# Farmadupe/vid_dup_finder_lib

Measured on AMD Instinct MI355X. Metric: hash-pairs/sec all-pairs Hamming (search(), tolerance 0.35) [+ frames/sec DCT-hash in 'summary.hash_summary'], higher is better.
Workload: dtype fp4 e2m1 ({0,1}) x fp4 -> f32 accumulate (exact half-integers < 2^11)

## Files before the change

vid_dup_finder_lib_amd/csrc/api.cpp:

```cpp
#include <algorithm>
#include <chrono>
#include <cmath>
#include <cstdio>
#include <cstdlib>
#include <cstring>
#include <memory>
#include <numeric>

#include "host_sort.h"
#include "vdf_ctx.h"

namespace {
thread_local std::string g_create_error;
inline double now_ms() { return std::chrono::duration<double, std::milli>(std::chrono::steady_clock::now().time_since_epoch()).count(); }
}

vdf_ctx::~vdf_ctx()
{
    if (!subs.empty() || !workers.empty()) vdf_impl::destroy_multi(this);
    if (copy_pool) vdf_impl::destroy_copy_pool(this);
    for (auto &kv : axis_tables) {
        kv.second->start.release(); kv.second->size.release(); kv.second->w.release();
        delete kv.second;
    }
    for (auto &kv : mfma_tables) {
        kv.second->operand.release(); kv.second->bias.release(); kv.second->meta.release();
        delete kv.second;
    }
    for (auto &kv : box_tables) {
        kv.second->blob.release(); kv.second->entries.release();
        delete kv.second;
    }
    DevBuf *all[] = {&row_lo, &row_hi, &tile_lo, &tile_hi, &tile_first, &tile_count, &tile_offset, &counters,
                     &hits, &perm, &matched, &exp_cols, &exp_rows, &pop_cols, &pop_rows, &cand, &group_cmin, &group_offset, &group_blocks, &up_hashes,
                     &up_dur, &up_ref_hashes, &up_ref_dur, &small, &frames, &frames2, &out_hashes, &out_hashes2, &out_dc,
                     &out_dc2, &cos_table, &crops, &crop_desc, &crop_tables, &crop_desc2, &crop_tables2, &crop_work, &sort_scratch, &sort_scratch_pub, &hits2, &hit_bitmaps, &bitmap_gather,
                     &out_zero, &out_zero2, &up_zero, &variant_hashes, &align_plan, &align_scratch, &align_up};
    for (DevBuf *b : all) b->release();
    for (PinBuf &b : pin) b.release();
    for (PinBuf &b : pin_out) b.release();
    pin_small.release();
    pin_ctrl.release();
    pin_crops.release();
    pin_desc.release();
    host_hits.buf.release();
    if (ev0) (void)hipEventDestroy(ev0);
    if (ev1) (void)hipEventDestroy(ev1);
    if (ev_mid) (void)hipEventDestroy(ev_mid);
    if (ev_wait) (void)hipEventDestroy(ev_wait);
    for (hipEvent_t e : ev_copy) if (e) (void)hipEventDestroy(e);
    for (hipEvent_t e : ev_done) if (e) (void)hipEventDestroy(e);
    if (copy_stream) (void)hipStreamDestroy(copy_stream);
    if (stream) (void)hipStreamDestroy(stream);
}

namespace vdf_impl {

void set_create_error(const std::string &msg) { g_create_error = msg; }

int fail(vdf_ctx *ctx, int code, const std::string &msg)
{
    if (ctx) ctx->err = msg;
    return code;
}

int fail_hip(vdf_ctx *ctx, hipError_t e, const char *what)
{
    std::string msg = std::string(what) + ": " + hipGetErrorString(e);
    (void)hipGetLastError();
    return fail(ctx, e == hipErrorOutOfMemory ? VDF_E_OOM : VDF_E_HIP, msg);
}

bool is_sorted_u32(const uint32_t *d, size_t n)
{
    for (size_t i = 1; i < n; i++)
        if (d[i] < d[i - 1]) return false;
    return true;
}

constexpr size_t kPinSmallBytes = 4u << 20;
constexpr uint64_t kDeviceSortHits = 1u << 17;
constexpr uint32_t kRefsMinWorkgroups = 2048;
constexpr uint64_t kSpecSortHits = 1u << 14;
constexpr uint64_t kFilterHits = 1u << 16;

int search_core(vdf_ctx *ctx, int mode, const uint64_t *d_col_hashes, const uint32_t *d_col_dur, size_t n_cols,
                const uint64_t *d_row_hashes, const uint32_t *d_row_dur, const uint32_t *d_row_perm, size_t n_rows,
                uint32_t tol_int, uint32_t shard_index, uint32_t shard_count, uint32_t row_begin, uint32_t row_end,
                const uint32_t *d_matched, uint32_t row_index_base, vdf_hit *hits, uint64_t capacity,
                uint64_t *n_hits_out, uint32_t *overflow_row_out, hipStream_t stream, bool replay_only, vdf_ctx::HostHits *staging,
                ShardExchange *fx)
{
    *n_hits_out = 0;
    *overflow_row_out = 0xFFFFFFFFu;
    if (n_rows == 0 || n_cols == 0) return VDF_OK;
    if (n_rows >= 0xFFFFFFFFull || n_cols >= 0xFFFFFFFFull) return fail(ctx, VDF_E_INVAL, "more than 2^32-1 hashes");
    if (shard_count == 0 || shard_index >= shard_count) return fail(ctx, VDF_E_INVAL, "bad shard index/count");
    VDF_HIP(ctx, hipSetDevice(ctx->device));
    const double t_enter = now_ms();

    vdf::SearchLaunch L{};
    const bool mfma = ctx->search_backend == 1;
    L.tile_rows = mfma ? (mode == 1 ? ctx->mfma_refs_rows : ctx->mfma_self_rows) : ctx->tile_rows;
    L.chunk_cols = mfma ? ctx->mfma_chunk_cols : ctx->chunk_cols;
    L.n_row_tiles = (uint32_t)((n_rows + L.tile_rows - 1) / L.tile_rows);
    if (mfma && L.chunk_cols == 0) {
        L.chunk_cols = 65536;
        while (L.chunk_cols > 4096 && (uint64_t)L.n_row_tiles * ((n_cols + L.chunk_cols - 1) / L.chunk_cols) < ctx->mfma_min_wgs) L.chunk_cols /= 2;
    }
    while ((uint64_t)L.n_row_tiles * ((n_cols + L.chunk_cols - 1) / L.chunk_cols) >= 0x40000000ull && L.chunk_cols < (1u << 22))
        L.chunk_cols *= 2;
    const size_t padded_rows = (size_t)L.n_row_tiles * L.tile_rows;
    VDF_HIP(ctx, ctx->row_lo.reserve(padded_rows * 4));
    VDF_HIP(ctx, ctx->row_hi.reserve(padded_rows * 4));
    VDF_HIP(ctx, ctx->tile_lo.reserve((size_t)L.n_row_tiles * 4));
    VDF_HIP(ctx, ctx->tile_hi.reserve((size_t)L.n_row_tiles * 4));
    VDF_HIP(ctx, ctx->tile_first.reserve((size_t)L.n_row_tiles * 4));
    VDF_HIP(ctx, ctx->tile_count.reserve((size_t)L.n_row_tiles * 4));
    VDF_HIP(ctx, ctx->tile_offset.reserve(((size_t)L.n_row_tiles + 1) * 4));
    VDF_HIP(ctx, ctx->counters.reserve(64));
    const uint64_t dev_cap = std::max<uint64_t>(capacity, 1);
    VDF_HIP(ctx, ctx->hits.reserve(dev_cap * sizeof(vdf_hit)));

    L.row_hashes = reinterpret_cast<const uint32_t *>(d_row_hashes);
    L.row_perm = d_row_perm;
    L.n_rows = (uint32_t)n_rows;
    L.row_index_base = row_index_base;
    L.col_hashes = reinterpret_cast<const uint32_t *>(d_col_hashes);
    L.n_cols = (uint32_t)n_cols;
    L.row_lo = ctx->row_lo.as<uint32_t>();
    L.row_hi = ctx->row_hi.as<uint32_t>();
    L.tile_lo = ctx->tile_lo.as<uint32_t>();
    L.tile_hi = ctx->tile_hi.as<uint32_t>();
    L.tile_first = ctx->tile_first.as<uint32_t>();
    L.tile_count = ctx->tile_count.as<uint32_t>();
    L.tile_offset = ctx->tile_offset.as<uint32_t>();
    L.tol = tol_int;
    L.matched = d_matched;
    L.self_mode = (mode == 0);
    L.shard_index = shard_index;
    L.shard_count = shard_count;
    L.hits = ctx->hits.as<vdf_hit>();
    L.capacity = capacity;
    L.counters = ctx->counters.as<unsigned long long>();
    L.overflow_row = reinterpret_cast<uint32_t *>(ctx->counters.as<unsigned long long>() + 4);

    L.prune_step = 16;
    if (ctx->mfma_prune_step >= 0) {
        L.prune_step = ctx->mfma_prune_step;
    } else {
        for (int st = 6; st <= 14; st++) {
            const double bits = 64.0 * (st + 1);
            if (bits / 2 - 2.0 * std::sqrt(bits) >= (double)tol_int + 1) { L.prune_step = st; break; }
        }
    }
    if (mfma) L.prune_step = L.prune_step <= 6 ? 6 : L.prune_step <= 8 ? 8 : L.prune_step <= 10 ? 10 : L.prune_step <= 14 ? L.prune_step : 16;
    else L.prune_step = L.prune_step <= 6 ? 6 : L.prune_step <= 10 ? 10 : L.prune_step <= 12 ? 12 : 16;
    if (mfma) {
        L.group_size = std::min<uint32_t>(ctx->mfma_group, L.n_row_tiles);
        L.n_groups = (L.n_row_tiles + L.group_size - 1) / L.group_size;
        if (L.n_groups > 1024) return fail(ctx, VDF_E_INVAL, "too many row-tile groups");
        VDF_HIP(ctx, ctx->group_cmin.reserve((size_t)L.n_groups * 4));
        VDF_HIP(ctx, ctx->group_offset.reserve(((size_t)L.n_groups + 1) * 4));
        VDF_HIP(ctx, ctx->group_blocks.reserve((size_t)L.n_groups * 4));
        L.group_blocks = ctx->group_blocks.as<uint32_t>();
        L.group_cmin = ctx->group_cmin.as<uint32_t>();
        L.group_offset = ctx->group_offset.as<uint32_t>();
        const uint32_t k_steps = (uint32_t)(L.prune_step < 15 ? L.prune_step + 1 : 16);
        const uint32_t col_pad = (uint32_t)((n_cols + vdf::kMfmaRowPad - 1) / vdf::kMfmaRowPad * vdf::kMfmaRowPad) + vdf::kMfmaColPad;
        VDF_HIP(ctx, ctx->exp_cols.reserve((size_t)col_pad * 512));
        VDF_HIP(ctx, ctx->pop_cols.reserve((size_t)col_pad * 12));
        const ExpOwner want_owner{d_col_hashes, n_cols, k_steps, ctx->exp_cols.p};
        const bool reuse = ctx->pinned_db == d_col_hashes && ctx->pinned_n == n_cols && ctx->exp_owner == want_owner;
        if (!reuse) {
            ctx->exp_owner = ExpOwner{};
            VDF_HIP(ctx, vdf::launch_expand_fp4(L.col_hashes, (uint32_t)n_cols, col_pad, ctx->exp_cols.p, k_steps,
                                                ctx->pop_cols.as<float>(), stream));
            ctx->exp_owner = want_owner;
        }
        L.col_exp = ctx->exp_cols.p;
        L.col_pop3 = ctx->pop_cols.as<float>();
        L.col_pad = col_pad;
        if (d_row_hashes == d_col_hashes) {
            L.row_exp = ctx->exp_cols.p;
            L.row_pop3 = L.col_pop3;
            L.row_pad = col_pad;
        } else {
            const uint32_t row_pad = (uint32_t)((padded_rows + 127) / 128 * 128);
            VDF_HIP(ctx, ctx->exp_rows.reserve((size_t)row_pad * 512));
            VDF_HIP(ctx, ctx->pop_rows.reserve((size_t)row_pad * 12));
            VDF_HIP(ctx, vdf::launch_expand_fp4(L.row_hashes, (uint32_t)n_rows, row_pad, ctx->exp_rows.p, k_steps,
                                                ctx->pop_rows.as<float>(), stream));
            L.row_exp = ctx->exp_rows.p;
            L.row_pop3 = ctx->pop_rows.as<float>();
            L.row_pad = row_pad;
        }
    }
    const unsigned long long init[8] = {0, 0, 0, 0, 0xFFFFFFFFull, 0, 0, 0};
    const bool pin_ok = ctx->pin_small.reserve(kPinSmallBytes) && ctx->pin_small.pinned;
    uint64_t spec = std::min<uint64_t>(capacity, std::max<uint64_t>(ctx->hits_guess + ctx->hits_guess / 4 + 1024, 8192));
    if (!pin_ok || spec * sizeof(vdf_hit) > kPinSmallBytes) spec = 0;
    const bool spec_sort = spec && ctx->hits_guess >= kSpecSortHits;
    if (spec_sort) VDF_HIP(ctx, hipMemsetAsync(ctx->hits.p, 0xFF, (size_t)spec * sizeof(vdf_hit), stream));
    const bool adapt_refs = mode == 1 && mfma && ctx->mfma_chunk_cols == 0;
    if (adapt_refs && ctx->refs_hint_cols == n_cols && ctx->refs_hint_rows == n_rows && ctx->refs_hint_chunk) L.chunk_cols = ctx->refs_hint_chunk;
    if (!ctx->pin_ctrl.reserve(256)) return fail(ctx, VDF_E_OOM, "pinned staging");
    unsigned long long *pre = ctx->pin_ctrl.as<unsigned long long>() + 8;
    uint32_t total_tiles = 0;
    unsigned long long unsorted = 0, admitted = 0;
    for (int pass = 0;; pass++) {
        VDF_HIP(ctx, hipMemcpyAsync(ctx->counters.p, init, sizeof init, hipMemcpyHostToDevice, stream));
        VDF_HIP(ctx, vdf::launch_windows_tiles(mode, d_col_dur, (uint32_t)n_cols, d_row_dur, d_row_perm, (uint32_t)n_rows,
                                               row_begin, row_end, shard_index, shard_count, L, stream));
        VDF_HIP(ctx, hipMemcpyAsync(pre, L.counters, 64, hipMemcpyDeviceToHost, stream));
        VDF_HIP(ctx, hipMemcpyAsync(pre + 8, mfma ? L.group_offset + L.n_groups : L.tile_offset + L.n_row_tiles, 4,
                                    hipMemcpyDeviceToHost, stream));
        VDF_HIP(ctx, hipMemcpyAsync(pre + 9, L.tile_offset + L.n_row_tiles, 4, hipMemcpyDeviceToHost, stream));
        VDF_HIP(ctx, hipStreamSynchronize(stream));
        total_tiles = *reinterpret_cast<const uint32_t *>(pre + 8);
        const uint32_t busy_tiles = *reinterpret_cast<const uint32_t *>(pre + 9);
        unsorted = pre[5];
        admitted = pre[2];
        if (!adapt_refs || pass > 0 || unsorted || busy_tiles == 0 || busy_tiles >= kRefsMinWorkgroups || L.chunk_cols <= 4096) break;
        uint64_t est = busy_tiles;
        while (L.chunk_cols > 4096 && est < kRefsMinWorkgroups) { L.chunk_cols /= 2; est *= 2; }
    }
    if (adapt_refs) { ctx->refs_hint_cols = n_cols; ctx->refs_hint_rows = n_rows; ctx->refs_hint_chunk = L.chunk_cols; }
    if (unsorted) return fail(ctx, VDF_E_INVAL, "durations are not ascending: pass the arrays in Search::sort order");
    if (total_tiles >= 0x7FFFFFFFu) return fail(ctx, VDF_E_INVAL, "tile count exceeds the grid limit");
    if (mfma) {
        const uint64_t want = ((uint64_t)((double)admitted * 6e-6) + (uint64_t)total_tiles * 8 * 8 + std::max<uint64_t>(capacity, 1ull << 20)) * ctx->cand_scale;
        L.cand_capacity = (uint32_t)std::min<uint64_t>(want, 0x40000000ull);
        if (ctx->cand_capacity_override)
            L.cand_capacity = (uint32_t)std::min<uint64_t>((uint64_t)ctx->cand_capacity_override * ctx->cand_scale, 0x40000000ull);
        const void *before = ctx->cand.p;
        VDF_HIP(ctx, ctx->cand.reserve((size_t)L.cand_capacity * 16));
        if (ctx->cand.p != before) ctx->cand_dirty = SIZE_MAX;
        const size_t slots = ctx->cand.cap / 16;
        const size_t fill = (ctx->cand_dirty == SIZE_MAX ? slots : std::min<size_t>(slots, ctx->cand_dirty)) * 16;
        if (fill) VDF_HIP(ctx, hipMemsetAsync(ctx->cand.p, 0xFF, fill, stream));
        ctx->cand_dirty = L.cand_capacity;
        L.cand = ctx->cand.p;
        L.cand_head = ctx->counters.as<unsigned long long>() + 6;
    }

    ctx->timing.prep_ms += (float)(now_ms() - t_enter);
    VDF_HIP(ctx, hipEventRecord(ctx->ev0, stream));
    if (mfma) {
        VDF_HIP(ctx, vdf::launch_hamming_tiles_mfma2(L, total_tiles, stream));
        VDF_HIP(ctx, hipEventRecord(ctx->ev_mid, stream));
        if (total_tiles) VDF_HIP(ctx, vdf::launch_resolve_candidates(L, stream));
    } else {
        VDF_HIP(ctx, vdf::launch_hamming_tiles(L, total_tiles, stream));
        VDF_HIP(ctx, hipEventRecord(ctx->ev_mid, stream));
    }
    VDF_HIP(ctx, hipEventRecord(ctx->ev1, stream));
    if (!ctx->pin_ctrl.reserve(256)) return fail(ctx, VDF_E_OOM, "pinned staging");
    unsigned long long *fin = ctx->pin_ctrl.as<unsigned long long>();
    VDF_HIP(ctx, hipMemcpyAsync(fin, ctx->counters.p, 64, hipMemcpyDeviceToHost, stream));
    unsigned row_bits = 1;
    while (row_bits < 32 && ((uint64_t)row_index_base + n_rows) >> row_bits) row_bits++;
    unsigned col_bits = 1;
    while (col_bits < 32 && ((uint64_t)n_cols >> col_bits)) col_bits++;
    if (spec_sort) {
        VDF_HIP(ctx, ctx->sort_scratch.reserve(vdf::sort_hits_scratch_bytes((size_t)spec)));
        VDF_HIP(ctx, vdf::launch_sort_hits(ctx->hits.as<vdf_hit>(), (size_t)spec, row_bits, ctx->sort_scratch.p, ctx->sort_scratch.cap, stream, col_bits));
    }
    if (spec) VDF_HIP(ctx, hipMemcpyAsync(ctx->pin_small.p, ctx->hits.p, (size_t)spec * sizeof(vdf_hit), hipMemcpyDeviceToHost, stream));
    VDF_HIP(ctx, hipStreamSynchronize(stream));
    const double t_synced = now_ms();
    float ms = 0.f, ms_stream = 0.f;
    VDF_HIP(ctx, hipEventElapsedTime(&ms, ctx->ev0, ctx->ev1));
    VDF_HIP(ctx, hipEventElapsedTime(&ms_stream, ctx->ev0, ctx->ev_mid));
    ctx->timing.stream_ms += ms_stream;
    ctx->timing.resolve_ms += ms - ms_stream;
    if (mfma) { ctx->timing.suspects += fin[6]; ctx->timing.suspect_capacity = L.cand_capacity; }

    if (mfma) ctx->cand_dirty = (size_t)std::min<uint64_t>(fin[6], L.cand_capacity);
    const uint64_t produced = fin[0];
    uint64_t stored = std::min<uint64_t>(produced, capacity);
    ctx->hits_guess = stored;
    uint64_t n_out = produced;
    vdf_hit *d_list = ctx->hits.as<vdf_hit>();
    uint64_t have = std::min(stored, spec);
    bool filter = false;
    if (replay_only && mode == 0 && !ctx->no_hit_filter) {
        bool complete = produced <= capacity && (uint32_t)fin[4] == 0xFFFFFFFFu;
        uint64_t total = produced;
        if (fx) {
            const int r = fx->agree(shard_index, ctx, &complete, &total);
            if (r) return r;
        } else if (shard_count != 1) {
            complete = false;
        }
        filter = complete && total >= kFilterHits;
    }
    if (filter) {
        const size_t words = ((size_t)n_cols + 31) / 32;
        VDF_HIP(ctx, ctx->hits2.reserve((size_t)std::max<uint64_t>(stored, 1) * sizeof(vdf_hit)));
        VDF_HIP(ctx, ctx->hit_bitmaps.reserve(2 * words * 4 + 16));
        uint32_t *bm = ctx->hit_bitmaps.as<uint32_t>();
        VDF_HIP(ctx, vdf::launch_filter_mark_incoming(d_list, stored, (uint32_t)n_cols, bm, stream));
        if (fx) { const int r = fx->or_bitmap(shard_index, ctx, bm, words, stream); if (r < 0) return r; if (r == vdf_impl::kExchangeOff) filter = false; }
        if (filter) {
            VDF_HIP(ctx, vdf::launch_filter_mark_covered(d_list, stored, (uint32_t)n_cols, bm, stream));
            if (fx) { const int r = fx->or_bitmap(shard_index, ctx, bm + words, words, stream); if (r < 0) return r; if (r == vdf_impl::kExchangeOff) filter = false; }
        }
    }
    if (filter) {
        uint32_t *bm = ctx->hit_bitmaps.as<uint32_t>();
        VDF_HIP(ctx, vdf::launch_filter_compact(d_list, stored, (uint32_t)n_cols, bm, ctx->hits2.as<vdf_hit>(), L.counters + 7, stream));
        VDF_HIP(ctx, hipMemcpyAsync(fin + 7, L.counters + 7, 8, hipMemcpyDeviceToHost, stream));
        VDF_HIP(ctx, hipStreamSynchronize(stream));
        d_list = ctx->hits2.as<vdf_hit>();
        stored = fin[7];
        n_out = stored;
        have = 0;
        ctx->timing.hits_filtered += produced - stored;
    }
    if (stored) {
        if (staging) {
            const size_t need = std::max<size_t>((size_t)stored, 1u << 16);
            if (staging->size() < need && !staging->resize(need + need / 4)) return fail(ctx, VDF_E_OOM, "hit staging");
            hits = staging->data();
        }
        if (have) std::memcpy(hits, ctx->pin_small.p, (size_t)have * sizeof(vdf_hit));
        if (stored > have) {
            const bool dev_sort = stored >= (d_list == ctx->hits.as<vdf_hit>() ? kDeviceSortHits : kDeviceSortHits / 16);
            if (dev_sort) {
                VDF_HIP(ctx, ctx->sort_scratch.reserve(vdf::sort_hits_scratch_bytes((size_t)stored)));
                VDF_HIP(ctx, vdf::launch_sort_hits(d_list, (size_t)stored, row_bits, ctx->sort_scratch.p, ctx->sort_scratch.cap, stream, col_bits));
                VDF_HIP(ctx, hipMemcpyAsync(hits, d_list, (size_t)stored * sizeof(vdf_hit), hipMemcpyDeviceToHost, stream));
            } else {
                VDF_HIP(ctx, hipMemcpyAsync(hits + have, d_list + have, (size_t)(stored - have) * sizeof(vdf_hit), hipMemcpyDeviceToHost, stream));
            }
            VDF_HIP(ctx, hipStreamSynchronize(stream));
            if (!dev_sort) sort_hits(hits, (size_t)stored);
        } else if (!spec_sort) {
            sort_hits(hits, (size_t)stored);
        }
    }
    ctx->timing.download_ms += (float)(now_ms() - t_synced);
    *n_hits_out = n_out;
    *overflow_row_out = (uint32_t)fin[4];
    ctx->stats.pairs += fin[2];
    ctx->stats.pairs_computed += fin[1];
    ctx->stats.n_hits += produced;
    ctx->stats.n_tiles += total_tiles;
    ctx->stats.n_launches += 1;
    ctx->stats.kernel_ms += ms;
    ctx->stats.pairs_early_exit += fin[3];
    ctx->stats.early_exit_bits = L.prune_step < 15 ? 64u * (uint32_t)(L.prune_step + 1) : 0u;
    return VDF_OK;
}

int upload(vdf_ctx *ctx, DevBuf &buf, const void *src, size_t bytes, hipStream_t stream)
{
    VDF_HIP(ctx, buf.reserve(std::max<size_t>(bytes, 16)));
    if (bytes) VDF_HIP(ctx, hipMemcpyAsync(buf.p, src, bytes, hipMemcpyHostToDevice, stream));
    return VDF_OK;
}

std::mutex &link_mutex(int device)
{
    static std::mutex m[64];
    return m[(unsigned)device % 64u];
}

int wait_event(vdf_ctx *ctx, hipEvent_t ev)
{
    if (!ctx->spin_wait) {
        const auto until = std::chrono::steady_clock::now() + std::chrono::microseconds(50);
        do {
            const hipError_t q = hipEventQuery(ev);
            if (q == hipSuccess) return VDF_OK;
            if (q != hipErrorNotReady) return fail_hip(ctx, q, "hipEventQuery");
        } while (std::chrono::steady_clock::now() < until);
    }
    VDF_HIP(ctx, hipEventSynchronize(ev));
    return VDF_OK;
}

DeviceAxisTable *axis_table(vdf_ctx *ctx, uint32_t in_size, hipStream_t stream, int *rc)
{
    auto it = ctx->axis_tables.find(in_size);
    if (it != ctx->axis_tables.end()) { *rc = VDF_OK; return it->second; }
    DeviceAxisTable *t = new DeviceAxisTable();
    if (!vdf::build_axis_table(in_size, VDF_DCT_SIZE, t->host)) {
        delete t;
        *rc = fail(ctx, VDF_E_BAD_DIMS, "cannot build resize table");
        return nullptr;
    }
    int r = upload(ctx, t->start, t->host.start.data(), t->host.start.size() * 4, stream);
    if (r == VDF_OK) r = upload(ctx, t->size, t->host.size.data(), t->host.size.size() * 4, stream);
    if (r == VDF_OK) r = upload(ctx, t->w, t->host.w.data(), t->host.w.size() * 2, stream);
    if (r == VDF_OK && hipStreamSynchronize(stream) != hipSuccess) r = fail(ctx, VDF_E_HIP, "table upload failed");
    if (r != VDF_OK) {
        t->start.release(); t->size.release(); t->w.release();
        delete t;
        *rc = r;
        return nullptr;
    }
    ctx->axis_tables[in_size] = t;
    *rc = VDF_OK;
    return t;
}

DeviceMfmaTable *mfma_table(vdf_ctx *ctx, uint32_t in_size, int layout, hipStream_t stream, int *rc)
{
    const uint64_t key = (uint64_t)in_size * 4 + (uint64_t)layout;
    auto it = ctx->mfma_tables.find(key);
    if (it != ctx->mfma_tables.end()) { *rc = VDF_OK; return it->second; }
    DeviceMfmaTable *t = new DeviceMfmaTable();
    if (!vdf::build_mfma_axis_table(in_size, layout, t->host)) {
        delete t;
        *rc = fail(ctx, VDF_E_BAD_DIMS, "cannot build resize table");
        return nullptr;
    }
    int r = VDF_OK;
    if (t->host.ok) {
        r = upload(ctx, t->operand, t->host.operand.data(), t->host.operand.size(), stream);
        if (r == VDF_OK) r = upload(ctx, t->bias, t->host.bias.data(), t->host.bias.size() * 4, stream);
        if (r == VDF_OK && !t->host.band_meta.empty())
            r = upload(ctx, t->meta, t->host.band_meta.data(), t->host.band_meta.size() * 4, stream);
        if (r == VDF_OK && hipStreamSynchronize(stream) != hipSuccess) r = fail(ctx, VDF_E_HIP, "table upload failed");
    }
    if (r != VDF_OK) {
        t->operand.release(); t->bias.release(); t->meta.release();
        delete t;
        *rc = r;
        return nullptr;
    }
    ctx->mfma_tables[key] = t;
    *rc = VDF_OK;
    return t;
}

BoxTableSet *box_table_set(vdf_ctx *ctx, uint32_t w, uint32_t h, hipStream_t stream, int *rc)
{
    const uint64_t key = ((uint64_t)w << 32) | h;
    auto it = ctx->box_tables.find(key);
    if (it != ctx->box_tables.end()) { *rc = VDF_OK; return it->second; }
    BoxTableSet *set = new BoxTableSet();
    set->one_tile = w <= 64 && h <= 64;
    const size_t n_idx = (size_t)w + h + 2;
    std::vector<vdf::CropTableEntry> entries(n_idx, vdf::CropTableEntry{nullptr, nullptr, 0, 0});
    std::vector<size_t> offset(n_idx, 0);
    std::vector<uint8_t> blob;
    bool usable = true;
    for (size_t idx = 0; idx < n_idx && usable; idx++) {
        const bool vertical = idx > w;
        const uint32_t size = (uint32_t)(vertical ? idx - w - 1 : idx);
        offset[idx] = blob.size();
        if (size == 0) {
            if (set->one_tile) blob.resize(blob.size() + vdf::kSmallBoxTableStride, 0);
            continue;
        }
        vdf::MfmaAxisTable t;
        if (!vdf::build_mfma_axis_table(size, vertical ? vdf::kMfmaLayoutVertical : vdf::kMfmaLayoutHorizontal, t) || !t.ok) { usable = false; break; }
        const size_t at = blob.size();
        blob.resize(at + t.operand.size() + 128, 0);
        std::memcpy(blob.data() + at, t.operand.data(), t.operand.size());
        std::memcpy(blob.data() + at + t.operand.size(), t.bias.data(), 64);
        const int32_t tail[2] = {t.precision, t.n_tiles};
        std::memcpy(blob.data() + at + t.operand.size() + 64, tail, sizeof tail);
        entries[idx].n_tiles = t.n_tiles;
        entries[idx].precision = t.precision;
        if (set->one_tile && blob.size() - at != vdf::kSmallBoxTableStride) usable = false;
    }
    int r = VDF_OK;
    if (usable) {
        r = upload(ctx, set->blob, blob.data(), blob.size(), stream);
        if (r == VDF_OK) {
            for (size_t idx = 0; idx < n_idx; idx++) {
                if (!entries[idx].n_tiles) continue;
                entries[idx].operand = set->blob.as<uint8_t>() + offset[idx];
                entries[idx].bias = reinterpret_cast<const int32_t *>(set->blob.as<uint8_t>() + offset[idx] + (size_t)entries[idx].n_tiles * 2048);
            }
            r = upload(ctx, set->entries, entries.data(), entries.size() * sizeof(vdf::CropTableEntry), stream);
        }
        if (r == VDF_OK && hipStreamSynchronize(stream) != hipSuccess) r = fail(ctx, VDF_E_HIP, "table upload failed");
    }
    if (r != VDF_OK) {
        set->blob.release(); set->entries.release();
        delete set;
        *rc = r;
        return nullptr;
    }
    set->usable = usable;
    ctx->box_tables[key] = set;
    *rc = VDF_OK;
    return set;
}

vdf::ResizeAxisTable dev_view(const DeviceAxisTable *t)
{
    vdf::ResizeAxisTable v{};
    if (t) {
        v.start = t->start.as<int32_t>();
        v.size = t->size.as<int32_t>();
        v.w = t->w.as<int16_t>();
        v.window = t->host.window;
        v.precision = t->host.precision;
    }
    return v;
}

int ensure_cos_table(vdf_ctx *ctx, hipStream_t stream)
{
    if (ctx->cos_table.p) return VDF_OK;
    double tab[16 * 16 + 17];
    for (int k = 0; k < 16; k++)
        for (int n = 0; n < 16; n++) tab[k * 16 + n] = std::cos(M_PI * (double)k * ((double)n + 0.5) / 16.0);
    int at = 256;
    auto twiddle = [&](int i, int fft_len) {
        const double angle_constant = M_PI * -2.0 / (double)fft_len;
        const double angle = angle_constant * (double)i;
        tab[at++] = std::cos(angle);
        tab[at++] = -std::sin(angle);
    };
    for (int i = 0; i < 4; i++) twiddle(2 * i + 1, 64);
    for (int i = 0; i < 2; i++) twiddle(2 * i + 1, 32);
    twiddle(1, 16);
    tab[at++] = M_SQRT1_2;
    tab[at++] = 0.0; tab[at++] = 0.0;
    int rc = upload(ctx, ctx->cos_table, tab, sizeof tab, stream);
    if (rc) return rc;
    VDF_HIP(ctx, hipStreamSynchronize(stream));
    return VDF_OK;
}

using vdf::kMaxClipsPerLaunch;

struct HashJob {
    const uint8_t *d_frames;
    size_t n_clips;
    uint32_t w, h;
    size_t frame_stride, clip_stride;
    uint64_t *d_out;
    uint32_t *d_dc;
    hipStream_t stream;
    uint64_t *d_zero = nullptr;
    vdf::HashCall call() const { return vdf::HashCall{d_frames, w, h, frame_stride, clip_stride, n_clips}; }
    const uint8_t *buf_end() const { return d_frames + (n_clips - 1) * clip_stride + (VDF_DCT_SIZE - 1) * frame_stride + (size_t)w * h; }
    HashJob clips(size_t c0, size_t n) const
    {
        return HashJob{d_frames + c0 * clip_stride, n, w, h, frame_stride, clip_stride, d_out + c0 * VDF_HASH_WORDS, d_dc ? d_dc + c0 : nullptr, stream,
                       d_zero ? d_zero + c0 * VDF_HASH_WORDS : nullptr};
    }
};

template <class One> int checked_launches(vdf_ctx *ctx, const HashJob &j, uint32_t frames_per_clip, One one)
// ... 433 lines not shown
                      uint64_t *d_zero)
{
    VDF_HIP(ctx, hipSetDevice(ctx->device));
    int rc = ensure_cos_table(ctx, stream);
    if (rc) return rc;
    const size_t n = plan.descs.size(), nd = n * sizeof(vdf::MixedClipDesc), off = (nd + 63) & ~size_t(63);
    const size_t max_entries = 2 * ((size_t)plan.max_w + plan.max_h + 2);
    if (!ctx->pin_desc.reserve(off + max_entries * sizeof(vdf::CropTableEntry))) return fail(ctx, VDF_E_OOM, "host staging for the clip descriptors");
    vdf::MixedClipDesc *dsc = ctx->pin_desc.as<vdf::MixedClipDesc>();
    vdf::CropTableEntry *ent = reinterpret_cast<vdf::CropTableEntry *>(ctx->pin_desc.as<char>() + off);
    LaunchTables plain(plan.max_w, plan.max_h, vdf::kMfmaLayoutHorizontal, vdf::kMfmaLayoutVertical), wide(plan.max_w, plan.max_h, vdf::kMfmaLayoutHorizontal, vdf::kMfmaLayoutVerticalWide);
    for (const vdf::MixedLaunch &l : plan.launches) {
        LaunchTables &tabs = l.part == vdf::MixedPart::kWideLines ? wide : plain;
        for (size_t i = l.first; i < l.first + l.count; i++) {
            vdf::MixedClipDesc d = plan.descs[i];
            const int32_t ih = tabs.entry(ctx, d.bw, false, stream, &rc), iv = ih < 0 ? -1 : tabs.entry(ctx, d.bh, true, stream, &rc);
            if (iv < 0) return rc ? rc : fail(ctx, VDF_E_BAD_DIMS, "box size whose coefficients do not fit the i8 split (clip " + std::to_string(d.out_index) + ")");
            d.h_table = (uint32_t)ih; d.v_table = (uint32_t)iv;
            dsc[i] = d;
        }
    }
    const size_t n_plain = plain.used.size(), n_entries = n_plain + wide.used.size();
    if (n_entries > max_entries) return fail(ctx, VDF_E_INVAL, "table index of a mixed call outgrew its staging");
    for (size_t i = 0; i < n_plain; i++) ent[i] = plain.crop_entry(i);
    for (size_t i = n_plain; i < n_entries; i++) ent[i] = wide.crop_entry(i - n_plain);
    for (const vdf::MixedLaunch &l : plan.launches)
        for (size_t i = l.first; i < l.first + l.count; i++) {
            if (l.part == vdf::MixedPart::kWideLines) { dsc[i].h_table += (uint32_t)n_plain; dsc[i].v_table += (uint32_t)n_plain; }
            if (dsc[i].h_table >= n_entries || dsc[i].v_table >= n_entries || dsc[i].out_index >= n) return fail(ctx, VDF_E_INVAL, "descriptor names a table or an output that is not there");
        }
    const size_t n_frames_part = n - plan.n_small;
    VDF_HIP(ctx, ctx->small.reserve(std::max<size_t>(n_frames_part, 1) * 4096));
    if ((rc = upload(ctx, ctx->crop_desc2, dsc, nd, stream))) return rc;
    if ((rc = upload(ctx, ctx->crop_tables2, ent, n_entries * sizeof(vdf::CropTableEntry), stream))) return rc;
    VDF_HIP(ctx, hipEventRecord(ctx->ev_mid, stream));
    const vdf::MixedClipDesc *d_desc = ctx->crop_desc2.as<vdf::MixedClipDesc>();
    const vdf::CropTableEntry *d_tab = ctx->crop_tables2.as<vdf::CropTableEntry>();
    const uint8_t *buf_end = d_buf + buf_bytes;
    uint8_t *small = ctx->small.as<uint8_t>();
    hipError_t e = hipSuccess;
    for (const vdf::MixedLaunch &l : plan.launches) {
        if (e != hipSuccess) break;
        if (l.part == vdf::MixedPart::kSmall) {
            e = vdf::launch_mixed_small(d_buf, buf_end, d_desc + l.first, l.count, d_tab, ctx->cos_table.as<double>(), d_out, d_dc, stream, d_zero);
        } else {
            uint8_t *slot0 = small + (l.first - plan.n_small) * 4096;
            e = vdf::launch_mixed_frames(d_buf, buf_end, d_desc + l.first, l.count, d_tab, l.part == vdf::MixedPart::kWideLines, slot0, stream);
            if (e == hipSuccess) e = vdf::launch_dct_hash_indexed(slot0, d_desc + l.first, l.count, ctx->cos_table.as<double>(), d_out, d_dc, stream, d_zero);
        }
    }
    const hipError_t ew = hipEventSynchronize(ctx->ev_mid);
    if (e != hipSuccess) return fail_hip(ctx, e, "mixed hash launch");
    VDF_HIP(ctx, ew);
    return VDF_OK;
}

int hash_clips_locked(vdf_ctx *ctx, const uint8_t *d_buf, size_t buf_bytes, const vdf_clip *clips, size_t n_clips, uint32_t frames_per_clip,
                      uint64_t *d_out, uint32_t *d_dc, hipStream_t stream, uint64_t *d_zero)
{
    if (n_clips && !clips) return fail(ctx, VDF_E_INVAL, "null pointer");
    if (n_clips > 0xFFFFFFFFull) return fail(ctx, VDF_E_INVAL, "more than 2^32 - 1 clips in one call");
    const vdf::MixedClip *mc = reinterpret_cast<const vdf::MixedClip *>(clips);
    const vdf::MixedCheck chk = vdf::check_mixed(mc, n_clips, frames_per_clip, buf_bytes);
    if (chk.error != vdf::MixedError::kNone) return mixed_check_failed(ctx, chk);
    if (n_clips == 0) return VDF_OK;
    if (!d_buf || !d_out) return fail(ctx, VDF_E_INVAL, "null pointer");
    const vdf::MixedPlan plan = vdf::plan_mixed(mc, n_clips, hash_knobs(ctx));
    if (plan.kind == vdf::MixedPlan::kUniform) {
        std::vector<uint32_t> crops;
        if (plan.cropped) {
            crops.resize(n_clips * 4);
            for (size_t i = 0; i < n_clips; i++) std::memcpy(&crops[4 * i], mc[i].crop, 16);
        }
        const HashJob all{d_buf + plan.offset0, n_clips, mc[0].w, mc[0].h, (size_t)mc[0].frame_stride, (size_t)plan.clip_stride, d_out, d_dc, stream, d_zero};
        return checked_launches(ctx, all, frames_per_clip,
                                [&](size_t c0, size_t n) { return hash_cropped_launch(ctx, all.clips(c0, n), plan.cropped ? crops.data() + 4 * c0 : nullptr); });
    }
    return hash_mixed_launch(ctx, d_buf, buf_bytes, plan, d_out, d_dc, stream, d_zero);
}

int letterbox_small(vdf_ctx *ctx, const HashJob &j, uint32_t frames_per_clip, const vdf::LetterboxPlan &plan, const BoxTableSet *set, uint32_t *out_crops,
                    uint32_t *d_crops)
{
    const size_t n_fused = j.n_clips - plan.n_tail;
    if (n_fused)
        VDF_HIP(ctx, vdf::launch_letterbox_hash_small(j.d_frames, n_fused, j.w, j.h, j.frame_stride, j.clip_stride, set->blob.p, ctx->cos_table.as<double>(),
                                                      j.d_out, j.d_dc, d_crops, ctx->hash_wgs_per_cu_set ? ctx->hash_wgs_per_cu : 0, j.stream));
    if (plan.n_tail) {
        const HashJob tail = j.clips(n_fused, plan.n_tail);
        VDF_HIP(ctx, ctx->crop_work.reserve(vdf::letterbox_work_bytes(tail.n_clips, frames_per_clip)));
        VDF_HIP(ctx, vdf::launch_letterbox(tail.d_frames, tail.n_clips, frames_per_clip, j.w, j.h, j.frame_stride, j.clip_stride, d_crops + 4 * n_fused,
                                           ctx->crop_work.as<uint32_t>(), j.stream, ctx->lb_side_strips));
        VDF_HIP(ctx, vdf::launch_resize_dct_cropped_small_boxes(tail.d_frames, tail.n_clips, j.w, j.h, j.frame_stride, j.clip_stride, j.buf_end(), d_crops + 4 * n_fused,
                                                                set->entries.as<vdf::CropTableEntry>(), ctx->cos_table.as<double>(), tail.d_out, tail.d_dc, j.stream));
    }
    if (out_crops) {
        if (!ctx->pin_crops.reserve(j.n_clips * 16)) return fail(ctx, VDF_E_OOM, "host staging for the crop boxes");
        VDF_HIP(ctx, hipMemcpyAsync(ctx->pin_crops.p, d_crops, j.n_clips * 16, hipMemcpyDeviceToHost, j.stream));
        VDF_HIP(ctx, hipEventRecord(ctx->ev_mid, j.stream));
        VDF_HIP(ctx, hipEventSynchronize(ctx->ev_mid));
        std::memcpy(out_crops, ctx->pin_crops.p, j.n_clips * 16);
    }
    return VDF_OK;
}

int letterbox_launch(vdf_ctx *ctx, const HashJob &j, uint32_t frames_per_clip, uint32_t *out_crops, uint32_t *d_out_crops)
{
    VDF_HIP(ctx, hipSetDevice(ctx->device));
    uint32_t *d_crops = d_out_crops;
    if (!d_crops) {
        VDF_HIP(ctx, ctx->crops.reserve(j.n_clips * 16));
        d_crops = ctx->crops.as<uint32_t>();
    }
    const vdf::LetterboxPlan plan = vdf::plan_letterbox(j.call(), hash_knobs(ctx));
    if (plan.small_frames) {
        int rc = ensure_cos_table(ctx, j.stream);
        if (rc) return rc;
        const BoxTableSet *set = box_table_set(ctx, j.w, j.h, j.stream, &rc);
        if (rc) return rc;
        if (set->usable) return letterbox_small(ctx, j, frames_per_clip, plan, set, out_crops, d_crops);
    }
    VDF_HIP(ctx, ctx->crop_work.reserve(vdf::letterbox_work_bytes(j.n_clips, frames_per_clip)));
    VDF_HIP(ctx, vdf::launch_letterbox(j.d_frames, j.n_clips, frames_per_clip, j.w, j.h, j.frame_stride, j.clip_stride, d_crops, ctx->crop_work.as<uint32_t>(),
                                       j.stream, ctx->lb_side_strips));
    if (!ctx->pin_crops.reserve(j.n_clips * 16)) return fail(ctx, VDF_E_OOM, "host staging for the crop boxes");
    uint32_t *crops = ctx->pin_crops.as<uint32_t>();
    VDF_HIP(ctx, hipMemcpyAsync(crops, d_crops, j.n_clips * 16, hipMemcpyDeviceToHost, j.stream));
    VDF_HIP(ctx, hipEventRecord(ctx->ev_wait, j.stream));
    if (int rcw = wait_event(ctx, ctx->ev_wait)) return rcw;
    if (out_crops) std::memcpy(out_crops, crops, j.n_clips * 16);
    return hash_cropped_launch(ctx, j, crops);
}

int letterbox_hash_device_locked(vdf_ctx *ctx, const uint8_t *d_frames, size_t n_clips, uint32_t frames_per_clip,
                                 uint32_t w, uint32_t h, size_t frame_stride, size_t clip_stride, uint64_t *d_out,
                                 uint32_t *d_dc, uint32_t *out_crops, hipStream_t stream, uint32_t *d_out_crops)
{
    const HashJob all{d_frames, n_clips, w, h, frame_stride, clip_stride, d_out, d_dc, stream};
    return checked_launches(ctx, all, frames_per_clip, [&](size_t c0, size_t n) {
        return letterbox_launch(ctx, all.clips(c0, n), frames_per_clip, out_crops ? out_crops + 4 * c0 : nullptr, d_out_crops ? d_out_crops + 4 * c0 : nullptr);
    });
}

static int letterbox_clips_plan(vdf_ctx *ctx, const void *d_buf, size_t buf_bytes, const vdf_clip *clips, size_t n_clips, uint32_t frames_per_clip, const void *out,
                                vdf::LetterboxMixedPlan *plan)
{
    if (n_clips && !clips) return fail(ctx, VDF_E_INVAL, "null pointer");
    if (n_clips > 0xFFFFFFFFull) return fail(ctx, VDF_E_INVAL, "more than 2^32 - 1 clips in one call");
    const vdf::MixedClip *mc = reinterpret_cast<const vdf::MixedClip *>(clips);
    const vdf::MixedCheck chk = vdf::check_mixed(mc, n_clips, frames_per_clip, buf_bytes);
    if (chk.error != vdf::MixedError::kNone) return mixed_check_failed(ctx, chk);
    *plan = vdf::plan_letterbox_mixed(mc, n_clips, hash_knobs(ctx));
    if (plan->kind == vdf::LetterboxMixedPlan::kCropGiven) return mixed_check_failed(ctx, vdf::MixedCheck{vdf::MixedError::kCropGiven, plan->bad_clip});
    if (n_clips && (!d_buf || !out)) return fail(ctx, VDF_E_INVAL, "null pointer");
    return VDF_OK;
}

static int letterbox_clips_detect(vdf_ctx *ctx, const uint8_t *d_buf, const vdf::LetterboxMixedPlan &plan, size_t n_clips, uint32_t *d_crops, hipStream_t stream)
{
    VDF_HIP(ctx, hipSetDevice(ctx->device));
    const size_t nd = plan.descs.size() * sizeof(vdf::LetterboxProbeDesc);
    if (plan.descs.size() != n_clips) return fail(ctx, VDF_E_INVAL, "letterbox plan does not cover the call");
    if (!ctx->pin_desc.reserve(nd)) return fail(ctx, VDF_E_OOM, "host staging for the clip descriptors");
    std::memcpy(ctx->pin_desc.p, plan.descs.data(), nd);
    if (int rc = upload(ctx, ctx->crop_desc, ctx->pin_desc.p, nd, stream)) return rc;
    VDF_HIP(ctx, hipEventRecord(ctx->ev_mid, stream));
    VDF_HIP(ctx, ctx->crop_work.reserve(plan.work_bytes));
    const hipError_t e = vdf::launch_letterbox_mixed(d_buf, ctx->crop_desc.as<vdf::LetterboxProbeDesc>(), plan.launches.data(), plan.launches.size(), n_clips, d_crops,
                                                     ctx->crop_work.as<uint32_t>(), stream);
    const hipError_t ew = hipEventSynchronize(ctx->ev_mid);
    if (e != hipSuccess) return fail_hip(ctx, e, "mixed letterbox launch");
    VDF_HIP(ctx, ew);
    return VDF_OK;
}

int cropdetect_clips_locked(vdf_ctx *ctx, const uint8_t *d_buf, size_t buf_bytes, const vdf_clip *clips, size_t n_clips, uint32_t frames_per_clip,
                            uint32_t *d_crops, hipStream_t stream)
{
    vdf::LetterboxMixedPlan plan;
    if (int rc = letterbox_clips_plan(ctx, d_buf, buf_bytes, clips, n_clips, frames_per_clip, d_crops, &plan)) return rc;
    if (n_clips == 0) return VDF_OK;
    if (plan.kind == vdf::LetterboxMixedPlan::kUniform) {
        VDF_HIP(ctx, hipSetDevice(ctx->device));
        const uint8_t *base = d_buf + plan.offset0;
        VDF_HIP(ctx, ctx->crop_work.reserve(vdf::letterbox_work_bytes(std::min(kMaxClipsPerLaunch, n_clips), frames_per_clip)));
        for (size_t c0 = 0; c0 < n_clips; c0 += kMaxClipsPerLaunch)
            VDF_HIP(ctx, vdf::launch_letterbox(base + c0 * plan.clip_stride, std::min(kMaxClipsPerLaunch, n_clips - c0), frames_per_clip, clips[0].w, clips[0].h,
                                               (size_t)clips[0].frame_stride, (size_t)plan.clip_stride, d_crops + 4 * c0, ctx->crop_work.as<uint32_t>(), stream,
                                               ctx->lb_side_strips));
        return VDF_OK;
    }
    return letterbox_clips_detect(ctx, d_buf, plan, n_clips, d_crops, stream);
}

int letterbox_clips_locked(vdf_ctx *ctx, const uint8_t *d_buf, size_t buf_bytes, const vdf_clip *clips, size_t n_clips, uint32_t frames_per_clip,
                           uint64_t *d_out, uint32_t *d_dc, uint32_t *out_crops, hipStream_t stream)
{
    vdf::LetterboxMixedPlan plan;
    if (int rc = letterbox_clips_plan(ctx, d_buf, buf_bytes, clips, n_clips, frames_per_clip, d_out, &plan)) return rc;
    if (n_clips == 0) return VDF_OK;
    if (plan.kind == vdf::LetterboxMixedPlan::kUniform)
        return letterbox_hash_device_locked(ctx, d_buf + plan.offset0, n_clips, frames_per_clip, clips[0].w, clips[0].h, (size_t)clips[0].frame_stride,
                                            (size_t)plan.clip_stride, d_out, d_dc, out_crops, stream);
    VDF_HIP(ctx, hipSetDevice(ctx->device));
    VDF_HIP(ctx, ctx->crops.reserve(n_clips * 16));
    uint32_t *d_crops = ctx->crops.as<uint32_t>();
    if (int rc = letterbox_clips_detect(ctx, d_buf, plan, n_clips, d_crops, stream)) return rc;
    if (!ctx->pin_crops.reserve(n_clips * 16)) return fail(ctx, VDF_E_OOM, "host staging for the crop boxes");
    const uint32_t *crops = ctx->pin_crops.as<uint32_t>();
    VDF_HIP(ctx, hipMemcpyAsync(ctx->pin_crops.p, d_crops, n_clips * 16, hipMemcpyDeviceToHost, stream));
    VDF_HIP(ctx, hipEventRecord(ctx->ev_wait, stream));
    if (int rcw = wait_event(ctx, ctx->ev_wait)) return rcw;
    if (out_crops) std::memcpy(out_crops, crops, n_clips * 16);
    std::vector<vdf_clip> boxed(clips, clips + n_clips);
    for (size_t i = 0; i < n_clips; i++) {
        boxed[i].crop_left = crops[4 * i]; boxed[i].crop_right = crops[4 * i + 1];
        boxed[i].crop_top = crops[4 * i + 2]; boxed[i].crop_bottom = crops[4 * i + 3];
    }
    return hash_clips_locked(ctx, d_buf, buf_bytes, boxed.data(), n_clips, frames_per_clip, d_out, d_dc, stream);
}


int search_refs_device_locked(vdf_ctx *ctx, const uint64_t *d_cand_hashes, const uint32_t *d_cand_durations,
                                     size_t n_cand, const uint64_t *d_ref_hashes, const uint32_t *d_ref_durations,
                                     size_t n_ref, uint32_t tol_int, uint32_t ref_index_base, vdf_hit *hits,
                                     uint64_t capacity, uint64_t *n_hits, hipStream_t s, vdf_ctx::HostHits *staging)
{
    ctx->stats = vdf_search_stats{};
    ctx->timing = vdf_search_timing{};
    *n_hits = 0;
    if (n_ref == 0 || n_cand == 0) return VDF_OK;
    VDF_HIP(ctx, hipSetDevice(ctx->device));
    const size_t sbytes = vdf::sort_order_scratch_bytes((uint32_t)n_ref, false);
    VDF_HIP(ctx, ctx->sort_scratch.reserve(sbytes));
    VDF_HIP(ctx, ctx->perm.reserve(std::max<size_t>(n_ref * 4, 16)));
    VDF_HIP(ctx, vdf::launch_sort_order(d_ref_durations, nullptr, (uint32_t)n_ref, ctx->perm.as<uint32_t>(), ctx->sort_scratch.p,
                                        ctx->sort_scratch.cap, s));
    int rc = VDF_OK;
    for (int attempt = 0;; attempt++) {
        uint32_t overflow_row = 0;
        ctx->stats = vdf_search_stats{};
        rc = search_core(ctx, 1, d_cand_hashes, d_cand_durations, n_cand, d_ref_hashes, d_ref_durations,
                         ctx->perm.as<uint32_t>(), n_ref, tol_int, 0, 1, 0, 0xFFFFFFFFu, nullptr, ref_index_base, hits,
                         capacity, n_hits, &overflow_row, s, false, staging);
        if (rc) { ctx->cand_scale = 1; return rc; }
        if (*n_hits > capacity) { ctx->cand_scale = 1; return fail(ctx, VDF_E_OVERFLOW, "hit buffer too small; *n_hits holds the required size"); }
        if (overflow_row == 0xFFFFFFFFu) break;
        if (attempt >= 12) { ctx->cand_scale = 1; return fail(ctx, VDF_E_OVERFLOW, "suspect queue overflow"); }
        ctx->cand_scale *= 4;
    }
    ctx->cand_scale = 1;
    return VDF_OK;
}

int create_single(int device_id, vdf_ctx **out, std::string *err)
{
    *out = nullptr;
    int count = 0;
    hipError_t e = hipGetDeviceCount(&count);
    if (e != hipSuccess || count <= 0) {
        *err = std::string("no usable HIP device: ") + (e != hipSuccess ? hipGetErrorString(e) : "count = 0");
        (void)hipGetLastError();
        return VDF_E_HIP;
    }
    if (device_id < 0 || device_id >= count) { *err = "device id out of range"; return VDF_E_INVAL; }
    vdf_ctx *ctx = new (std::nothrow) vdf_ctx();
    if (!ctx) return VDF_E_OOM;
    ctx->device = device_id;
    ctx->spin_wait = std::getenv("VDF_SPIN_WAIT") != nullptr;
    ctx->no_link_turns = std::getenv("VDF_NO_LINK_TURNS") != nullptr;
    const unsigned wait_flags = hipEventDisableTiming | (ctx->spin_wait ? 0u : (unsigned)hipEventBlockingSync);
    bool ok = hipSetDevice(device_id) == hipSuccess &&
              hipStreamCreateWithFlags(&ctx->stream, hipStreamNonBlocking) == hipSuccess &&
              hipEventCreate(&ctx->ev0) == hipSuccess && hipEventCreate(&ctx->ev1) == hipSuccess &&
              hipEventCreate(&ctx->ev_mid) == hipSuccess && hipEventCreateWithFlags(&ctx->ev_wait, wait_flags) == hipSuccess;
    for (int i = 0; ok && i < 2; i++)
        ok = hipEventCreateWithFlags(&ctx->ev_copy[i], wait_flags) == hipSuccess &&
             hipEventCreateWithFlags(&ctx->ev_done[i], wait_flags) == hipSuccess;
    if (!ok) {
        *err = std::string("context setup failed: ") + hipGetErrorString(hipGetLastError());
        delete ctx;
        return VDF_E_HIP;
    }
    if (const char *s = std::getenv("VDF_ROWS_PER_LANE")) {
        int r = std::atoi(s);
        if (r == 1 || r == 2 || r == 4) ctx->tile_rows = 256u * (uint32_t)r;
    }
    if (const char *s = std::getenv("VDF_RESIZE_MODE")) {
        int m = std::atoi(s);
        if (m >= 0 && m <= 6 && m != 2) ctx->resize_mode = m;
    }
    if (const char *s = std::getenv("VDF_SEARCH_BACKEND")) {
        if (!std::strcmp(s, "valu")) ctx->search_backend = 0;
        else if (!std::strcmp(s, "mfma")) ctx->search_backend = 1;
    }
    if (const char *s = std::getenv("VDF_MFMA_CHUNK_COLS")) {
        long c = std::atol(s);
        if (c >= 32 && c <= (1 << 22)) ctx->mfma_chunk_cols = (uint32_t)c;
    }
    if (const char *s = std::getenv("VDF_CAND_CAPACITY")) { const long v = std::atol(s); if (v >= 8 && v <= 0x40000000l) ctx->cand_capacity_override = (uint32_t)v; }
    if (const char *s = std::getenv("VDF_MFMA_SELF_ROWS")) { const int v = std::atoi(s); if (v == 256 || v == 512) ctx->mfma_self_rows = (uint32_t)v; }
    if (const char *s = std::getenv("VDF_MFMA_REFS_ROWS")) { const int v = std::atoi(s); if (v == 256 || v == 512) ctx->mfma_refs_rows = (uint32_t)v; }
    if (const char *s = std::getenv("VDF_MFMA_PRUNE_STEP")) ctx->mfma_prune_step = std::atoi(s);
    if (const char *s = std::getenv("VDF_MFMA_MIN_WGS")) { const long v = std::atol(s); if (v >= 1 && v <= (1 << 24)) ctx->mfma_min_wgs = (uint32_t)v; }
    if (const char *s = std::getenv("VDF_MFMA_GROUP")) {
        long c = std::atol(s);
        if (c >= 1 && c <= (1 << 20)) ctx->mfma_group = (uint32_t)c;
    }
    if (const char *s = std::getenv("VDF_NO_HIT_FILTER")) ctx->no_hit_filter = std::atoi(s) != 0;
    if (std::getenv("VDF_NO_WAVESTREAM")) ctx->wavestream_knob = -1;
    else if (const char *s = std::getenv("VDF_WAVESTREAM_NW")) { const int v = std::atoi(s); if (v >= 3 && v <= 8) ctx->wavestream_knob = v; }
    ctx->no_rowcrop = std::getenv("VDF_NO_ROWCROP") != nullptr;
    ctx->rowcrop_all = std::getenv("VDF_ROWCROP_ALL") != nullptr;
    ctx->no_boxstream = std::getenv("VDF_NO_BOXSTREAM") != nullptr;
    ctx->no_smallcrop = std::getenv("VDF_NO_SMALLCROP") != nullptr;
    ctx->no_device_path_order = std::getenv("VDF_NO_DEVICE_PATH_ORDER") != nullptr;
    ctx->lb_host_plan = std::getenv("VDF_LB_HOST_PLAN") != nullptr;
    ctx->no_lb_fused = std::getenv("VDF_NO_LB_FUSED") != nullptr;
    if (std::getenv("VDF_LB_NC16")) ctx->lb_side_strips = 16;
    if (const char *s = std::getenv("VDF_COPY_THREADS")) { const int v = std::atoi(s); if (v >= 1 && v <= 64) ctx->copy_threads = v; }
    if (const char *s = std::getenv("VDF_HOST_CHUNK_MB")) { const long v = std::atol(s); if (v >= 1 && v <= 1024) ctx->host_chunk_bytes = (size_t)v << 20; }
    if (const char *s = std::getenv("VDF_HOST_DIRECT")) ctx->host_direct = std::atoi(s) != 0;
    if (const char *s = std::getenv("VDF_HASH_NO_PERSISTENT")) ctx->hash_no_persistent = std::atoi(s) != 0;
    if (const char *s = std::getenv("VDF_HASH_WGS_PER_CU")) {
        int v = std::atoi(s);
        if (v >= 1 && v <= 8) { ctx->hash_wgs_per_cu = v; ctx->hash_wgs_per_cu_set = true; }
    }
    if (const char *s = std::getenv("VDF_CHUNK_COLS")) {
        long c = std::atol(s);
        if (c >= 64 && c <= (1 << 20)) ctx->chunk_cols = (uint32_t)c;
    }
    *out = ctx;
    return VDF_OK;
}

int search_self_resident(vdf_ctx *ctx, size_t n, uint32_t tol_int, vdf_groups *out)
{
    const int G = device_count(ctx);
    uint64_t capacity = ctx->hit_capacity;
    std::vector<uint8_t> matched(n, 0);
    std::vector<uint32_t> bitmap;
    bool use_bitmap = false;
    std::vector<vdf_hit> merged;
    uint32_t row_begin = 0;
    uint64_t span = n;
    ctx->stats = vdf_search_stats{};
    const double t_call = now_ms();
    double replay_ms = 0.0;
    for (int k = 0; k < G; k++) { device_ctx(ctx, k)->stats = vdf_search_stats{}; device_ctx(ctx, k)->timing = vdf_search_timing{}; }
    while (row_begin < n) {
        const uint32_t row_end = (uint32_t)std::min<uint64_t>((uint64_t)row_begin + span, n);
        std::unique_ptr<ShardExchange> fx(make_local_exchange(ctx));
        int rc = for_each_device(ctx, [&](int k, vdf_ctx *d) {
            const int r = search_core(d, 0, d->up_hashes.as<uint64_t>(), d->up_dur.as<uint32_t>(), n, d->up_hashes.as<uint64_t>(),
                                      d->up_dur.as<uint32_t>(), nullptr, n, tol_int, (uint32_t)k, (uint32_t)G, row_begin, row_end,
                                      use_bitmap ? d->matched.as<uint32_t>() : nullptr, 0, nullptr, capacity,
                                      &d->r_n_hits, &d->r_overflow, d->stream, true, &d->host_hits, fx.get());
            if (r && fx && !d->err_secondary) fx->abort(r, "device " + std::to_string(d->device) + ": " + d->err);
            return r;
        });
        if (rc) { vdf_groups_free(out); return rc; }
        uint32_t overflow_row = 0xFFFFFFFFu;
        for (int k = 0; k < G; k++) overflow_row = std::min(overflow_row, device_ctx(ctx, k)->r_overflow);
        const uint32_t complete_end = std::min(overflow_row, row_end);
        const vdf_hit *hp;
        uint64_t nh;
        if (G == 1) {
            hp = device_ctx(ctx, 0)->host_hits.data();
            nh = std::min(device_ctx(ctx, 0)->r_n_hits, capacity);
        } else {
            merged.clear();
            for (int k = 0; k < G; k++) {
                const vdf_ctx *d = device_ctx(ctx, k);
                const vdf_hit *b = d->host_hits.data(), *e = b + std::min(d->r_n_hits, capacity);
                e = std::lower_bound(b, e, vdf_hit{complete_end, 0u}, hit_less);
                const size_t mid = merged.size();
                merged.insert(merged.end(), b, e);
                std::inplace_merge(merged.begin(), merged.begin() + (ptrdiff_t)mid, merged.end(), hit_less);
            }
            hp = merged.data();
            nh = merged.size();
        }
        const uint64_t old_members = out->n_groups ? out->offsets[out->n_groups] : 0;
        const double t_replay = now_ms();
        rc = vdf_replay_self(n, hp, nh, row_begin, complete_end, matched.data(), out);
        replay_ms += now_ms() - t_replay;
        if (rc) { vdf_groups_free(out); return fail(ctx, rc, "replay failed"); }
        if (overflow_row == 0xFFFFFFFFu) {
            row_begin = row_end;
            span = std::min<uint64_t>(n, span * 4);
        } else {
            const uint64_t progress = complete_end - row_begin;
            if (progress == 0) {
                span = 1;
                if (capacity < n) capacity = n;
                for (int k = 0; k < G; k++) device_ctx(ctx, k)->cand_scale = std::min<uint64_t>(device_ctx(ctx, k)->cand_scale * 4, 1ull << 24);
            } else {
                span = std::max<uint64_t>(progress * 2, device_ctx(ctx, 0)->tile_rows);
            }
            row_begin = complete_end;
        }
        if (row_begin < n) {
            if (!use_bitmap) {
                bitmap.assign((n + 31) / 32, 0u);
                for (size_t i = 0; i < n; i++)
                    if (matched[i]) bitmap[i >> 5] |= 1u << (i & 31);
                use_bitmap = true;
            } else {
                const uint64_t new_members = out->n_groups ? out->offsets[out->n_groups] : 0;
                for (uint64_t q = old_members; q < new_members; q++) {
                    const uint64_t i = out->members[q];
                    bitmap[i >> 5] |= 1u << (i & 31);
                }
            }
            rc = for_each_device(ctx, [&](int, vdf_ctx *d) {
                int r = upload(d, d->matched, bitmap.data(), bitmap.size() * 4, d->stream);
                if (r) return r;
                VDF_HIP(d, hipStreamSynchronize(d->stream));
                return (int)VDF_OK;
            });
            if (rc) { vdf_groups_free(out); return rc; }
        }
    }
    ctx->dev_stats.assign((size_t)G, vdf_search_stats{});
    vdf_search_stats agg{};
    for (int k = 0; k < G; k++) {
        device_ctx(ctx, k)->cand_scale = 1;
        const vdf_search_stats &st = device_ctx(ctx, k)->stats;
        ctx->dev_stats[(size_t)k] = st;
        agg.pairs += st.pairs; agg.pairs_computed += st.pairs_computed; agg.n_hits += st.n_hits; agg.n_tiles += st.n_tiles;
        agg.pairs_early_exit += st.pairs_early_exit;
        agg.n_launches = std::max(agg.n_launches, st.n_launches);
        agg.kernel_ms = std::max(agg.kernel_ms, st.kernel_ms);
        agg.early_exit_bits = st.early_exit_bits;
    }
    ctx->stats = agg;
    const double t_fin = now_ms();
    const int rc_fin = vdf_groups_finish_self(out);
    vdf_search_timing tm{};
    for (int k = 0; k < G; k++) {
        const vdf_search_timing &q = device_ctx(ctx, k)->timing;
        tm.prep_ms = std::max(tm.prep_ms, q.prep_ms); tm.stream_ms = std::max(tm.stream_ms, q.stream_ms);
        tm.resolve_ms = std::max(tm.resolve_ms, q.resolve_ms); tm.download_ms = std::max(tm.download_ms, q.download_ms);
        tm.suspects += q.suspects; tm.suspect_capacity = std::max(tm.suspect_capacity, q.suspect_capacity);
        tm.hits_filtered += q.hits_filtered;
    }
    tm.replay_ms = (float)(replay_ms + now_ms() - t_fin);
    tm.total_ms = (float)(now_ms() - t_call);
    ctx->timing = tm;
    ctx->dev_timing.assign((size_t)G, vdf_search_timing{});
    for (int k = 0; k < G; k++) ctx->dev_timing[(size_t)k] = device_ctx(ctx, k)->timing;
    return rc_fin;
}

int search_refs_resident(vdf_ctx *ctx, size_t n_cand, const std::vector<size_t> &ref_cnt, const std::vector<size_t> &ref_base,
                         uint32_t tol_int, vdf_groups *out)
{
    const int G = device_count(ctx);
    const uint64_t capacity0 = ctx->hit_capacity;
    const double t_call = now_ms();
    int rc = for_each_device(ctx, [&](int k, vdf_ctx *d) {
        d->r_n_hits = 0;
        d->stats = vdf_search_stats{};
        d->timing = vdf_search_timing{};
        if (ref_cnt[(size_t)k] == 0) return (int)VDF_OK;
        uint64_t capacity = capacity0;
        for (int attempt = 0; attempt < 6; attempt++) {
            int r = search_refs_device_locked(d, d->up_hashes.as<uint64_t>(), d->up_dur.as<uint32_t>(), n_cand,
                                              d->up_ref_hashes.as<uint64_t>(), d->up_ref_dur.as<uint32_t>(),
                                              ref_cnt[(size_t)k], tol_int, (uint32_t)ref_base[(size_t)k], nullptr,
                                              capacity, &d->r_n_hits, d->stream, &d->host_hits);
            if (r == VDF_E_OVERFLOW && d->r_n_hits > capacity) { capacity = d->r_n_hits; continue; }
            return r;
        }
        return (int)VDF_E_OVERFLOW;
    });
    if (rc) return rc;
    ctx->dev_stats.assign((size_t)G, vdf_search_stats{});
    vdf_search_stats agg{};
    for (int k = 0; k < G; k++) {
        const vdf_search_stats &st = device_ctx(ctx, k)->stats;
        ctx->dev_stats[(size_t)k] = st;
        agg.pairs += st.pairs; agg.pairs_computed += st.pairs_computed; agg.n_hits += st.n_hits; agg.n_tiles += st.n_tiles;
        agg.pairs_early_exit += st.pairs_early_exit;
        agg.n_launches = std::max(agg.n_launches, st.n_launches);
        agg.kernel_ms = std::max(agg.kernel_ms, st.kernel_ms);
        agg.early_exit_bits = st.early_exit_bits;
    }
    ctx->stats = agg;
    vdf_search_timing tm{};
    for (int k = 0; k < G; k++) {
        const vdf_search_timing &q = device_ctx(ctx, k)->timing;
        tm.prep_ms = std::max(tm.prep_ms, q.prep_ms); tm.stream_ms = std::max(tm.stream_ms, q.stream_ms);
        tm.resolve_ms = std::max(tm.resolve_ms, q.resolve_ms); tm.download_ms = std::max(tm.download_ms, q.download_ms);
        tm.suspects += q.suspects; tm.suspect_capacity = std::max(tm.suspect_capacity, q.suspect_capacity);
        tm.hits_filtered += q.hits_filtered;
    }
    ctx->dev_timing.assign((size_t)G, vdf_search_timing{});
    for (int k = 0; k < G; k++) ctx->dev_timing[(size_t)k] = device_ctx(ctx, k)->timing;
    const double t_group = now_ms();
    int rcg;
    if (G == 1) {
        rcg = vdf_groups_from_ref_hits(device_ctx(ctx, 0)->host_hits.data(), device_ctx(ctx, 0)->r_n_hits, out);
    } else {
        std::vector<vdf_hit> all;
        for (int k = 0; k < G; k++) {
            const vdf_ctx *d = device_ctx(ctx, k);
            all.insert(all.end(), d->host_hits.data(), d->host_hits.data() + d->r_n_hits);
        }
        rcg = vdf_groups_from_ref_hits(all.data(), all.size(), out);
    }
    tm.replay_ms = (float)(now_ms() - t_group);
    tm.total_ms = (float)(now_ms() - t_call);
    ctx->timing = tm;
    return rcg;
}

int align_checks(vdf_ctx *ctx, const void *a_hashes, const uint32_t *a_first, size_t n_a, const void *b_hashes, const uint32_t *b_first, size_t n_b,
                 const void *a_first_ptr, const void *b_first_ptr, uint32_t min_run, const void *out, size_t capacity, const size_t *n_out)
{
    const bool self = b_hashes == nullptr;
    if (!n_out || (n_a && (!a_hashes || !a_first_ptr)) || (!self && n_b && !b_first_ptr) || (capacity && !out)) return fail(ctx, VDF_E_INVAL, "null pointer");
    if (min_run == 0) return fail(ctx, VDF_E_INVAL, "min_run of zero");
    const uint32_t *firsts[2] = {a_first, self ? nullptr : b_first};
    const size_t counts[2] = {n_a, n_b};
    for (int side = 0; side < 2; side++)
        for (size_t v = 0; firsts[side] && v < counts[side]; v++)
            if (firsts[side][v + 1] >= firsts[side][v] && firsts[side][v + 1] - firsts[side][v] > vdf::kAlignMaxWindows)
                return fail(ctx, VDF_E_INVAL, std::string("video ") + std::to_string(v) + (side ? " of B" : " of A") + " has more than 2^20 windows");
    for (int side = 0; side < 2; side++)
        for (size_t v = 0; firsts[side] && v < counts[side]; v++)
            if (firsts[side][v + 1] < firsts[side][v])
                return fail(ctx, VDF_E_INVAL, std::string("the first array") + (side ? " of B" : " of A") + " decreases at video " + std::to_string(v));
    if (n_a > 0xFFFFFFFFull || n_b > 0xFFFFFFFFull || vdf::align_pair_count(n_a, self ? n_a : n_b, self) > vdf::kAlignMaxPairs)
        return fail(ctx, VDF_E_INVAL, "more than 2^24 pairs of videos in one call");
    return VDF_OK;
}

void align_pair_host(const uint64_t *A, uint32_t Na, const uint8_t *skip_a, const uint64_t *B, uint32_t Nb, const uint8_t *skip_b, uint32_t tol,
                     uint32_t min_run, vdf_alignment *best)
{
    uint32_t best_score = 0;
    best->offset = 0; best->start_a = 0; best->n_windows = 0; best->dist_sum = 0;
    for (int64_t d = -((int64_t)Na - 1); d <= (int64_t)Nb - 1; d++) {
        const int64_t ka0 = std::max<int64_t>(0, -d), ka1 = std::min<int64_t>(Na, (int64_t)Nb - d);
        uint32_t len = 0, sum = 0;
        for (int64_t ka = ka0; ka <= ka1; ka++) {
            bool match = false;
            uint32_t dist = 0;
            if (ka < ka1 && !(skip_a && skip_a[ka]) && !(skip_b && skip_b[ka + d])) {
                const uint64_t *x = A + 16 * ka, *y = B + 16 * (ka + d);
                for (int w = 0; w < VDF_HASH_WORDS; w++) dist += (uint32_t)__builtin_popcountll(x[w] ^ y[w]);
                match = dist <= tol;
            }
            if (match) { len++; sum += dist; continue; }
            if (len >= min_run) {
                const uint32_t score = len * (tol + 1) - sum, start = (uint32_t)(ka - len);
                if (vdf::align_better(score, (int32_t)d, start, best_score, best->offset, best->start_a)) {
                    best_score = score; best->offset = (int32_t)d; best->start_a = start; best->n_windows = len; best->dist_sum = sum;
                }
            }
            len = 0; sum = 0;
        }
    }
}

int align_locked(vdf_ctx *ctx, const uint64_t *d_a_hashes, const uint32_t *d_a_first, const uint32_t *h_first_a, size_t n_a, const uint8_t *d_a_skip,
                 const uint64_t *d_b_hashes, const uint32_t *d_b_first, const uint32_t *h_first_b, size_t n_b, const uint8_t *d_b_skip, bool self,
                 uint32_t tol_int, uint32_t min_run, vdf_alignment *out, size_t capacity, size_t *n_out, hipStream_t s)
{
    vdf::AlignCursor cur;
    vdf::AlignChunk ch;
    size_t found = 0;
    while (vdf::align_next_chunk(h_first_a, n_a, h_first_b, n_b, self, cur, ch)) {
        const size_t n_pairs = ch.pairs.size(), n_units = ch.n_units();
        const size_t pair_bytes = n_pairs * sizeof(vdf::AlignPair), off_bytes = (n_pairs + 1) * sizeof(uint32_t);
        VDF_HIP(ctx, ctx->align_plan.reserve(pair_bytes + off_bytes));
        VDF_HIP(ctx, ctx->align_scratch.reserve(vdf::align_scratch_bytes(n_pairs, n_units)));
        char *plan = ctx->align_plan.as<char>();
        VDF_HIP(ctx, hipMemcpyAsync(plan, ch.pairs.data(), pair_bytes, hipMemcpyHostToDevice, s));
        VDF_HIP(ctx, hipMemcpyAsync(plan + pair_bytes, ch.unit_offset.data(), off_bytes, hipMemcpyHostToDevice, s));
        vdf_alignment *d_dense = nullptr;
        uint32_t *d_total = nullptr;
        vdf::AlignLaunch L{};
        L.a_hashes = reinterpret_cast<const uint32_t *>(d_a_hashes); L.a_first = d_a_first; L.a_skip = d_a_skip;
        L.b_hashes = reinterpret_cast<const uint32_t *>(d_b_hashes); L.b_first = d_b_first; L.b_skip = d_b_skip;
        L.pairs = reinterpret_cast<const vdf::AlignPair *>(plan);
        L.unit_offset = reinterpret_cast<const uint32_t *>(plan + pair_bytes);
        L.n_pairs = (uint32_t)n_pairs; L.n_units = (uint32_t)n_units;
        L.tol = std::min<uint32_t>(tol_int, 1024u); L.min_run = min_run;
        L.scratch = ctx->align_scratch.p; L.dense_out = &d_dense; L.total_out = &d_total;
        VDF_HIP(ctx, vdf::launch_align_chunk(L, s));
        uint32_t total = 0;
        VDF_HIP(ctx, hipMemcpyAsync(&total, d_total, sizeof(total), hipMemcpyDeviceToHost, s));
        VDF_HIP(ctx, hipStreamSynchronize(s));
        const size_t room = capacity > found ? capacity - found : 0, take = std::min<size_t>(total, room);
        if (take) {
            VDF_HIP(ctx, hipMemcpyAsync(out + found, d_dense, take * sizeof(vdf_alignment), hipMemcpyDeviceToHost, s));
            VDF_HIP(ctx, hipStreamSynchronize(s));
        }
        found += total;
    }
    *n_out = found;
    return VDF_OK;
}

}

using namespace vdf_impl;

extern "C" {
// ... 739 lines not shown
```

vid_dup_finder_lib_amd/csrc/hamming.hip:

```cpp
#include <algorithm>

#include "vdf_internal.h"

namespace vdf {

constexpr uint32_t kMaxBlocksPerLaunch = 4u << 20;

typedef const __attribute__((address_space(4))) uint32_t *const_u32_ptr;

__device__ __forceinline__ uint32_t sat_u32(double x)
{
    if (!(x == x)) return 0u;
    if (x <= 0.0) return 0u;
    if (x >= 4294967295.0) return 0xFFFFFFFFu;
    return (uint32_t)x;
}

__device__ __forceinline__ uint32_t partition_point_lt(const uint32_t *__restrict__ d, uint32_t n, uint32_t v)
{
    uint32_t lo = 0, hi = n;
    while (lo < hi) {
        uint32_t mid = lo + ((hi - lo) >> 1);
        if (d[mid] < v) lo = mid + 1; else hi = mid;
    }
    return lo;
}
__device__ __forceinline__ uint32_t partition_point_le(const uint32_t *__restrict__ d, uint32_t n, uint32_t v)
{
    uint32_t lo = 0, hi = n;
    while (lo < hi) {
        uint32_t mid = lo + ((hi - lo) >> 1);
        if (d[mid] <= v) lo = mid + 1; else hi = mid;
    }
    return lo;
}

__device__ __forceinline__ uint32_t wave_min(uint32_t v)
{
#pragma unroll
    for (int o = 32; o > 0; o >>= 1) v = min(v, (uint32_t)__shfl_xor((int)v, o, 64));
    return v;
}
__device__ __forceinline__ uint32_t wave_max(uint32_t v)
{
#pragma unroll
    for (int o = 32; o > 0; o >>= 1) v = max(v, (uint32_t)__shfl_xor((int)v, o, 64));
    return v;
}

__device__ __forceinline__ void wave_append_hits(bool hit, uint32_t row, uint32_t col, vdf_hit *__restrict__ hits,
                                                 unsigned long long capacity, unsigned long long *__restrict__ counters,
                                                 uint32_t *__restrict__ overflow_row)
{
    const unsigned long long bal = __builtin_amdgcn_ballot_w64(hit);
    if (bal == 0ull) return;
    const int leader = __builtin_ctzll(bal);
    unsigned long long base = 0;
    if ((int)(threadIdx.x & 63) == leader) base = atomicAdd(&counters[0], (unsigned long long)__builtin_popcountll(bal));
    base = ((unsigned long long)(uint32_t)__shfl((int)(base >> 32), leader, 64) << 32) | (uint32_t)__shfl((int)(uint32_t)base, leader, 64);
    if (hit) {
        const unsigned long long at = base + __builtin_amdgcn_mbcnt_hi((uint32_t)(bal >> 32), __builtin_amdgcn_mbcnt_lo((uint32_t)bal, 0u));
        if (at < capacity) {
            vdf_hit hp; hp.row = row; hp.col = col;
            hits[at] = hp;
        } else {
            atomicMin(overflow_row, row);
        }
    }
}

__global__ __launch_bounds__(256) void windows_tiles_kernel(
    int mode, const uint32_t *__restrict__ col_dur, uint32_t n_cols, const uint32_t *__restrict__ row_dur,
    const uint32_t *__restrict__ row_perm, uint32_t n_rows, uint32_t row_begin, uint32_t row_end, uint32_t shard_index,
    uint32_t shard_count, uint32_t tile_rows, uint32_t chunk_cols, uint32_t *__restrict__ row_lo,
    uint32_t *__restrict__ row_hi, uint32_t *__restrict__ tile_lo, uint32_t *__restrict__ tile_hi,
    uint32_t *__restrict__ tile_first, uint32_t *__restrict__ tile_count, unsigned long long *__restrict__ counters)
{
    __shared__ uint32_t s_min[4], s_max[4];
    __shared__ unsigned long long s_pairs[4];
    const uint32_t t = blockIdx.x;
    const bool mine = (t % shard_count) == shard_index;
    uint32_t mn = 0xFFFFFFFFu, mx = 0u;
    unsigned long long pairs = 0;
    for (uint32_t q = threadIdx.x; q < tile_rows; q += 256) {
        const uint32_t p = t * tile_rows + q;
        uint32_t lo = 0, hi = 0;
        if (mine && p < n_rows && p >= row_begin && p < row_end) {
            const uint32_t r = row_perm ? row_perm[p] : p;
            const double d = (double)row_dur[r];
            if (mode == 0) {
                lo = p + 1;
                hi = partition_point_le(col_dur, n_cols, sat_u32(d * 1.1));
            } else {
                lo = partition_point_lt(col_dur, n_cols, sat_u32(d * 0.95));
                hi = partition_point_le(col_dur, n_cols, sat_u32(d * 1.05));
            }
            if (hi <= lo) { lo = 0; hi = 0; }
        }
        row_lo[p] = lo;
        row_hi[p] = hi;
        if (hi > lo) {
            mn = min(mn, lo);
            mx = max(mx, hi);
            pairs += hi - lo;
        }
    }
    mn = wave_min(mn);
    mx = wave_max(mx);
#pragma unroll
    for (int o = 32; o > 0; o >>= 1) pairs += __shfl_xor(pairs, o, 64);
    const int wave = threadIdx.x >> 6;
    if ((threadIdx.x & 63) == 0) { s_min[wave] = mn; s_max[wave] = mx; s_pairs[wave] = pairs; }
    __syncthreads();
    if (threadIdx.x == 0) {
        mn = min(min(s_min[0], s_min[1]), min(s_min[2], s_min[3]));
        mx = max(max(s_max[0], s_max[1]), max(s_max[2], s_max[3]));
        pairs = s_pairs[0] + s_pairs[1] + s_pairs[2] + s_pairs[3];
        uint32_t cnt = 0, first = 0;
        if (mx > mn) {
            first = mn / chunk_cols;
            cnt = (mx + chunk_cols - 1) / chunk_cols - first;
        } else {
            mn = 0; mx = 0;
        }
        tile_lo[t] = mn;
        tile_hi[t] = mx;
        tile_first[t] = first;
        tile_count[t] = cnt;
        if (pairs) atomicAdd(&counters[2], pairs);
    }
}

__global__ __launch_bounds__(256) void check_sorted_kernel(const uint32_t *__restrict__ d, uint32_t n,
                                                           unsigned long long *__restrict__ counters)
{
    bool bad = false;
    for (size_t i = (size_t)blockIdx.x * 256 + threadIdx.x; i + 1 < n; i += (size_t)gridDim.x * 256) bad |= d[i] > d[i + 1];
    if (__builtin_amdgcn_ballot_w64(bad) != 0ull && (threadIdx.x & 63) == 0) counters[5] = 1ull;
}

__global__ __launch_bounds__(1024) void scan_tiles_kernel(const uint32_t *__restrict__ tile_count, uint32_t n,
                                                          uint32_t *__restrict__ tile_offset)
{
    __shared__ uint32_t s_part[1024];
    const uint32_t tid = threadIdx.x;
    const uint32_t per = (n + 1023) / 1024;
    const uint32_t b = min(tid * per, n), e = min(b + per, n);
    uint32_t sum = 0;
    for (uint32_t i = b; i < e; i++) sum += tile_count[i];
    s_part[tid] = sum;
    __syncthreads();
    for (uint32_t o = 1; o < 1024; o <<= 1) {
        uint32_t v = (tid >= o) ? s_part[tid - o] : 0u;
        __syncthreads();
        s_part[tid] += v;
        __syncthreads();
    }
    uint32_t run = s_part[tid] - sum;
    for (uint32_t i = b; i < e; i++) { tile_offset[i] = run; run += tile_count[i]; }
    if (tid == 1023) tile_offset[n] = s_part[1023];
}

__global__ __launch_bounds__(256) void group_tiles_kernel(const uint32_t *__restrict__ tile_first,
                                                          const uint32_t *__restrict__ tile_count, uint32_t n_row_tiles,
                                                          uint32_t group_size, uint32_t shard_count,
                                                          uint32_t *__restrict__ group_cmin,
                                                          uint32_t *__restrict__ group_blocks)
{
    __shared__ uint32_t s_min[4], s_max[4];
    const uint32_t g = blockIdx.x;
    uint32_t cmin = 0xFFFFFFFFu, cmax = 0;
    const uint32_t t1 = min((g + 1) * group_size, n_row_tiles);
    for (uint32_t t = g * group_size + threadIdx.x; t < t1; t += 256) {
        if (tile_count[t]) {
            cmin = min(cmin, tile_first[t]);
            cmax = max(cmax, tile_first[t] + tile_count[t]);
        }
    }
    cmin = wave_min(cmin);
    cmax = wave_max(cmax);
    if ((threadIdx.x & 63) == 0) { s_min[threadIdx.x >> 6] = cmin; s_max[threadIdx.x >> 6] = cmax; }
    __syncthreads();
    if (threadIdx.x == 0) {
        cmin = min(min(s_min[0], s_min[1]), min(s_min[2], s_min[3]));
        cmax = max(max(s_max[0], s_max[1]), max(s_max[2], s_max[3]));
        if (cmax <= cmin) { cmin = 0; cmax = 0; }
        group_cmin[g] = cmin;
        const uint32_t n_chunks = cmax - cmin;
        group_blocks[g] = n_chunks * ((group_size + shard_count - 1) / shard_count);
    }
}

__global__ void group_scan_kernel(const uint32_t *__restrict__ group_blocks, uint32_t n_groups,
                                  uint32_t *__restrict__ group_offset)
{
    if (threadIdx.x == 0 && blockIdx.x == 0) {
        uint32_t run = 0;
        for (uint32_t g = 0; g < n_groups; g++) { group_offset[g] = run; run += group_blocks[g]; }
        group_offset[n_groups] = run;
    }
}

template <int R, int CHKW>
__global__ __launch_bounds__(256) void hamming_tile_kernel(
    const uint32_t *__restrict__ row_hashes, const uint32_t *__restrict__ row_perm, uint32_t n_rows,
    uint32_t row_index_base, const uint32_t *__restrict__ col_hashes, const uint32_t *__restrict__ row_lo,
    const uint32_t *__restrict__ row_hi, const uint32_t *__restrict__ tile_lo, const uint32_t *__restrict__ tile_hi,
    const uint32_t *__restrict__ tile_first, const uint32_t *__restrict__ tile_offset, uint32_t n_row_tiles,
    uint32_t chunk_cols, uint32_t tol, const uint32_t *__restrict__ matched, int self_mode,
    vdf_hit *__restrict__ hits, unsigned long long capacity, unsigned long long *__restrict__ counters,
    uint32_t *__restrict__ overflow_row, uint32_t block_base)
{
    constexpr uint32_t TILE_ROWS = 256 * R;
    const uint32_t lane = threadIdx.x & 63, wave = threadIdx.x >> 6;
    const uint32_t bid = blockIdx.x + block_base;

    const_u32_ptr off = (const_u32_ptr)(uintptr_t)tile_offset;
    uint32_t tl = 0, th = n_row_tiles;
    while (th - tl > 1) {
        const uint32_t mid = (tl + th) >> 1;
        if (off[mid] <= bid) tl = mid; else th = mid;
    }
    const uint32_t t = tl;
    const uint32_t chunk = ((const_u32_ptr)(uintptr_t)tile_first)[t] + (bid - off[t]);
    const uint32_t t_lo = ((const_u32_ptr)(uintptr_t)tile_lo)[t];
    const uint32_t t_hi = ((const_u32_ptr)(uintptr_t)tile_hi)[t];
    const uint32_t c_begin = max(chunk * chunk_cols, t_lo);
    const uint32_t c_end = min((chunk + 1) * chunk_cols, t_hi);
    if (c_begin >= c_end) return;

    uint32_t rw[R][32];
    uint32_t rlo[R], rhi[R], rid[R];
#pragma unroll
    for (int k = 0; k < R; k++) {
        const uint32_t p = t * TILE_ROWS + wave * (64 * R) + k * 64 + lane;
        uint32_t lo = row_lo[p], hi = row_hi[p];
        uint32_t src = p;
        if (p < n_rows) {
            if (row_perm) src = row_perm[p];
            const uint4 *rp = reinterpret_cast<const uint4 *>(row_hashes + (size_t)src * 32);
#pragma unroll
            for (int q = 0; q < 8; q++) {
                const uint4 v = rp[q];
                rw[k][4 * q + 0] = v.x; rw[k][4 * q + 1] = v.y; rw[k][4 * q + 2] = v.z; rw[k][4 * q + 3] = v.w;
            }
            if (self_mode && matched && ((matched[src >> 5] >> (src & 31)) & 1u)) { lo = 0; hi = 0; }
        } else {
#pragma unroll
            for (int q = 0; q < 32; q++) rw[k][q] = 0u;
            lo = 0; hi = 0;
        }
        rlo[k] = lo; rhi[k] = hi; rid[k] = row_index_base + src;
    }

    const_u32_ptr cols = (const_u32_ptr)(uintptr_t)col_hashes;
    uint32_t n_early = 0;
    for (uint32_t c = c_begin; c < c_end; ++c) {
        const_u32_ptr cp = cols + (size_t)c * 32;
        uint32_t d[R];
#pragma unroll
        for (int k = 0; k < R; k++) d[k] = 0u;
#pragma unroll
        for (int w = 0; w < (CHKW < 32 ? CHKW : 32); ++w) {
            const uint32_t cw = cp[w];
#pragma unroll
            for (int k = 0; k < R; k++) d[k] += __builtin_popcount(rw[k][w] ^ cw);
        }
        uint32_t m = d[0];
#pragma unroll
        for (int k = 1; k < R; k++) m = min(m, d[k]);
        if (CHKW < 32) {
            if (__builtin_amdgcn_ballot_w64(m <= tol) == 0ull) { n_early += 1; continue; }
#pragma unroll
            for (int w = CHKW; w < 32; ++w) {
                const uint32_t cw = cp[w];
#pragma unroll
                for (int k = 0; k < R; k++) d[k] += __builtin_popcount(rw[k][w] ^ cw);
            }
            m = d[0];
#pragma unroll
            for (int k = 1; k < R; k++) m = min(m, d[k]);
        }
        if (__builtin_amdgcn_ballot_w64(m <= tol) != 0ull) {
            bool col_ok = true;
            if (matched) col_ok = ((((const_u32_ptr)(uintptr_t)matched)[c >> 5] >> (c & 31)) & 1u) == 0u;
            if (col_ok) {
#pragma unroll
                for (int k = 0; k < R; k++)
                    wave_append_hits(d[k] <= tol && c >= rlo[k] && c < rhi[k], rid[k], c, hits, capacity, counters, overflow_row);
            }
        }
    }
    if (threadIdx.x == 0) atomicAdd(&counters[1], (unsigned long long)(c_end - c_begin) * TILE_ROWS);
    if (CHKW < 32 && lane == 0 && n_early) atomicAdd(&counters[3], (unsigned long long)n_early * (64u * R));
}

typedef int v8i __attribute__((ext_vector_type(8)));
typedef int v4i __attribute__((ext_vector_type(4)));
typedef float v16f __attribute__((ext_vector_type(16)));

__global__ __launch_bounds__(256) void expand_fp4_kernel(const uint32_t *__restrict__ packed, uint32_t n,
                                                        uint32_t n_pad, uint4 *__restrict__ expanded,
                                                        uint32_t k_steps, float *__restrict__ pop,
                                                        float *__restrict__ popk, float *__restrict__ popkT)
{
    for (size_t idx = (size_t)blockIdx.x * 256 + threadIdx.x; idx < (size_t)n_pad * 32;
         idx += (size_t)gridDim.x * 256) {
    const uint32_t hsh = (uint32_t)(idx >> 5), dw = (uint32_t)idx & 31u;
    uint4 out = {0u, 0u, 0u, 0u};
    uint32_t w = 0;
    if (hsh < n) {
        w = packed[idx];
        uint32_t o[4];
#pragma unroll
        for (int j = 0; j < 4; j++) {
            uint32_t x = (w >> (8 * j)) & 0xFFu;
            x = (x | (x << 12)) & 0x000F000Fu;
            x = (x | (x << 6)) & 0x03030303u;
            x = (x | (x << 3)) & 0x11111111u;
            o[j] = x << 1;
        }
        out = make_uint4(o[0], o[1], o[2], o[3]);
    }
    expanded[idx] = out;
    if (pop) {
        uint32_t pc = (uint32_t)__builtin_popcount(w), pk = (dw & 15u) < k_steps ? pc : 0u;
#pragma unroll
        for (int o = 16; o > 0; o >>= 1) { pc += (uint32_t)__shfl_xor((int)pc, o, 32); pk += (uint32_t)__shfl_xor((int)pk, o, 32); }
        if (dw == 0) {
            pop[hsh] = (float)pc;
            popk[hsh] = (float)pk;
            popkT[(size_t)(hsh >> 7) * 128 + (hsh & 31u) * 4 + ((hsh >> 5) & 3u)] = (float)pk;
        }
    }
    }
}

template <int N>
struct IntC { static constexpr int value = N; };
template <int I, int N, class F>
__device__ __forceinline__ void static_for(F &&f)
{
    if constexpr (I < N) {
        f(IntC<I>{});
        static_for<I + 1, N>(f);
    }
}

struct CandEntry {
    uint32_t row_base;
    uint32_t col;
    uint32_t mask;
    uint32_t pad;
};

__global__ __launch_bounds__(256) void resolve_candidates_kernel(
    const CandEntry *__restrict__ cand, const unsigned long long *__restrict__ cand_head, uint32_t cand_capacity,
    const uint32_t *__restrict__ row_hashes, const uint32_t *__restrict__ row_perm, uint32_t n_rows, uint32_t row_index_base,
    const uint32_t *__restrict__ col_hashes, uint32_t n_cols, const uint32_t *__restrict__ row_lo,
    const uint32_t *__restrict__ row_hi, uint32_t tol, const uint32_t *__restrict__ matched, int self_mode,
    vdf_hit *__restrict__ hits, unsigned long long capacity, unsigned long long *__restrict__ counters,
    uint32_t *__restrict__ overflow_row)
{
    const uint32_t n = (uint32_t)min(*cand_head, (unsigned long long)cand_capacity);
    const uint32_t lane = threadIdx.x & 63, wave = threadIdx.x >> 6;
    constexpr uint32_t kStage = 512;
    __shared__ vdf_hit s_stage[4][kStage];
    uint32_t staged = 0;
    auto flush = [&]() {
        if (staged == 0) return;
        __builtin_amdgcn_fence(__ATOMIC_ACQ_REL, "wavefront");
        __builtin_amdgcn_wave_barrier();
        unsigned long long base = 0;
        if (lane == 0) base = atomicAdd(&counters[0], (unsigned long long)staged);
        base = ((unsigned long long)(uint32_t)__builtin_amdgcn_readfirstlane((int)(base >> 32)) << 32) |
               (uint32_t)__builtin_amdgcn_readfirstlane((int)(uint32_t)base);
        for (uint32_t k = lane; k < staged; k += 64) {
            const vdf_hit hp = s_stage[wave][k];
            if (base + k < capacity) hits[base + k] = hp;
            else atomicMin(overflow_row, hp.row);
        }
        __builtin_amdgcn_fence(__ATOMIC_ACQ_REL, "wavefront");
        __builtin_amdgcn_wave_barrier();
        staged = 0;
    };
    for (uint32_t e0 = blockIdx.x * 256 + (threadIdx.x & ~63u); e0 < n; e0 += gridDim.x * 256) {
        const uint32_t e = e0 + lane;
        CandEntry ce;
        ce.row_base = 0xFFFFFFFFu; ce.col = 0; ce.mask = 0; ce.pad = 0;
        if (e < n) ce = cand[e];
        uint32_t m = ce.mask;
        if (ce.row_base == 0xFFFFFFFFu || ce.col >= n_cols) m = 0;
        if (m && matched && ((matched[ce.col >> 5] >> (ce.col & 31)) & 1u)) m = 0;
        uint4 cw[8];
        if (m) {
            const uint4 *cp = reinterpret_cast<const uint4 *>(col_hashes + (size_t)ce.col * 32);
#pragma unroll
            for (int q = 0; q < 8; q++) cw[q] = cp[q];
        }
        while (__builtin_amdgcn_ballot_w64(m != 0u) != 0ull) {
            bool hit = false;
            uint32_t src = 0;
            if (m) {
                const uint32_t r = (uint32_t)__builtin_ctz(m);
                m &= m - 1;
                const uint32_t p = ce.row_base + (r & 3) + 8 * (r >> 2);
                if (p < n_rows) {
                    const uint32_t lo = row_lo[p], hi = row_hi[p];
                    if (ce.col >= lo && ce.col < hi) {
                        src = row_perm ? row_perm[p] : p;
                        if (!(self_mode && matched && ((matched[src >> 5] >> (src & 31)) & 1u))) {
                            const uint4 *rp = reinterpret_cast<const uint4 *>(row_hashes + (size_t)src * 32);
                            uint32_t d = 0;
#pragma unroll
                            for (int q = 0; q < 8; q++) {
                                const uint4 v = rp[q];
                                d += __builtin_popcount(v.x ^ cw[q].x) + __builtin_popcount(v.y ^ cw[q].y) +
                                     __builtin_popcount(v.z ^ cw[q].z) + __builtin_popcount(v.w ^ cw[q].w);
                            }
                            hit = d <= tol;
                        }
                    }
                }
            }
            const unsigned long long bal = __builtin_amdgcn_ballot_w64(hit);
            if (bal == 0ull) continue;
            const uint32_t cnt = (uint32_t)__builtin_popcountll(bal);
            if (staged + cnt > kStage) flush();
            if (hit) {
                vdf_hit hp; hp.row = row_index_base + src; hp.col = ce.col;
                s_stage[wave][staged + __builtin_amdgcn_mbcnt_hi((uint32_t)(bal >> 32), __builtin_amdgcn_mbcnt_lo((uint32_t)bal, 0u))] = hp;
            }
            staged += cnt;
        }
    }
    flush();
}

template <int CHK, int WAVES>
__global__ __launch_bounds__(64 * WAVES, 2) void hamming_mfma2_kernel(
    const uint4 *__restrict__ row_exp, const uint32_t *__restrict__ row_perm, uint32_t n_rows,
    uint32_t row_index_base, const uint4 *__restrict__ col_exp, const uint32_t *__restrict__ row_lo,
    const uint32_t *__restrict__ row_hi, const uint32_t *__restrict__ tile_lo, const uint32_t *__restrict__ tile_hi,
    const uint32_t *__restrict__ tile_first, const uint32_t *__restrict__ tile_count,
    const uint32_t *__restrict__ group_offset, const uint32_t *__restrict__ group_cmin, uint32_t n_groups,
    uint32_t group_size, uint32_t shard_index, uint32_t shard_count, uint32_t n_row_tiles, uint32_t chunk_cols,
    uint32_t tol, const uint32_t *__restrict__ matched, int self_mode, vdf_hit *__restrict__ hits,
    unsigned long long capacity, unsigned long long *__restrict__ counters, uint32_t *__restrict__ overflow_row,
    uint32_t block_base, const float *__restrict__ row_pop3, uint32_t row_pad, const float *__restrict__ col_pop3,
    uint32_t col_pad, CandEntry *__restrict__ cand, uint32_t cand_capacity, unsigned long long *__restrict__ cand_head)
{
    constexpr int K = CHK < 15 ? CHK + 1 : 16;
    constexpr bool kRowcLds = K > 13;
    constexpr uint32_t kSub = WAVES >= 8 ? 4 : 2;
    constexpr uint32_t kColStep = 32 * kSub;
    constexpr int NBLK = 2 * (int)kSub;
    constexpr int NM = NBLK * K;
    constexpr int P = (K == 16 && WAVES >= 8) ? 2 : 4, NB = P + 1;
    constexpr uint32_t kTileRows = 64 * WAVES;
    constexpr int kDmaPerWave = (int)(kColStep * 32 / (64 * WAVES));
    constexpr int kDmaEvery = NM / kDmaPerWave;
    static_assert(kDmaEvery >= 2, "stage too short for its DMA pieces");
    constexpr int kTestAt = 2;
    static_assert(K >= kTestAt + 4, "block too short to hide the previous block's test");
    const uint32_t bid = blockIdx.x + block_base;
    __shared__ __attribute__((aligned(16))) uint4 s_b0[kColStep * 32];
    __shared__ __attribute__((aligned(16))) uint4 s_b1[kColStep * 32];
    const uint32_t tid = threadIdx.x, lane = tid & 63, g = lane >> 5, c31 = lane & 31;
    const uint32_t wave = (uint32_t)__builtin_amdgcn_readfirstlane((int)(tid >> 6));

    const_u32_ptr goff = (const_u32_ptr)(uintptr_t)group_offset;
    uint32_t gl = 0, gh = n_groups;
    while (gh - gl > 1) {
        const uint32_t mid = (gl + gh) >> 1;
        if (goff[mid] <= bid) gl = mid; else gh = mid;
    }
    const uint32_t idx = bid - goff[gl];
    const uint32_t per_group = (group_size + shard_count - 1) / shard_count;
    const uint32_t g0 = gl * group_size;
    const uint32_t t0 = g0 + (shard_index + shard_count - g0 % shard_count) % shard_count;
    const uint32_t t = t0 + (idx % per_group) * shard_count;
    const uint32_t chunk = ((const_u32_ptr)(uintptr_t)group_cmin)[gl] + idx / per_group;
    if (t >= n_row_tiles || t >= g0 + group_size) return;
    {
        const uint32_t f = ((const_u32_ptr)(uintptr_t)tile_first)[t], cnt = ((const_u32_ptr)(uintptr_t)tile_count)[t];
        if (chunk < f || chunk >= f + cnt) return;
    }
    const uint32_t t_lo = ((const_u32_ptr)(uintptr_t)tile_lo)[t];
    const uint32_t t_hi = ((const_u32_ptr)(uintptr_t)tile_hi)[t];
    const uint32_t c_begin = max(chunk * chunk_cols, t_lo);
    const uint32_t c_end = min((chunk + 1) * chunk_cols, t_hi);
    if (c_begin >= c_end) return;

    const float tol_f = (float)min(tol, 1024u);
    const float *row_popk = row_pop3 + row_pad;
    const float *col_popkT = col_pop3 + 2 * (size_t)col_pad;
    const uint32_t row0 = t * kTileRows + wave * 64;
    v4i a[2][K];
    const float4 *s_rc = nullptr;
    v16f rowc[2];
    uint32_t live[2];
#pragma unroll
    for (int rt = 0; rt < 2; rt++) {
        live[rt] = 0;
        const uint32_t p = row0 + 32 * rt + c31;
        uint32_t src = p;
        if (p < n_rows && row_perm) src = row_perm[p];
        const uint4 *rp = row_exp + (size_t)src * 32 + 16 * g;
#pragma unroll
        for (int s = 0; s < K; s++) {
            const uint4 v = rp[s];
            a[rt][s] = (v4i){(int)v.x, (int)v.y, (int)v.z, (int)v.w};
        }
#pragma unroll
        for (int r = 0; r < 16; r++) {
            const uint32_t pr = row0 + 32 * rt + (r & 3) + 8 * (r >> 2) + 4 * g;
            const uint32_t sr = (pr < n_rows && row_perm) ? row_perm[pr] : pr;
            rowc[rt][r] = -0.5f * row_popk[sr];
            if (row_hi[pr] > row_lo[pr]) live[rt] |= 1u << r;
        }
    }
    if constexpr (kRowcLds) {
        __shared__ __attribute__((aligned(16))) float4 s_rowc[WAVES * 2 * 2 * 4];
        float4 *mine = s_rowc + ((size_t)wave * 2 * 2 + g) * 4;
        if (c31 == 0) {
#pragma unroll
            for (int rt = 0; rt < 2; rt++)
#pragma unroll
                for (int q = 0; q < 4; q++)
                    mine[rt * 2 * 4 + q] = float4{rowc[rt][4 * q], rowc[rt][4 * q + 1], rowc[rt][4 * q + 2], rowc[rt][4 * q + 3]};
        }
        s_rc = mine;
    }
    const uint32_t cb0 = c_begin & ~(kColStep - 1);
    constexpr uint32_t kColsPerRound = 2 * WAVES;
    constexpr int kOffsets = 32 / kColsPerRound;
    static_assert(kOffsets >= 1 && (kOffsets & (kOffsets - 1)) == 0, "piece addressing");
    const uint32_t c0 = 2 * wave + g;
    uint32_t lane_off[kOffsets];
#pragma unroll
    for (int j = 0; j < kOffsets; j++) lane_off[j] = c0 * 512u + ((((lane & 31) ^ c0) << 4) ^ (16u * kColsPerRound * j));
    auto stage_rsrc = [&](uint32_t cb) __attribute__((always_inline)) {
        return __builtin_amdgcn_make_buffer_rsrc(
            const_cast<char *>(reinterpret_cast<const char *>(col_exp) + (size_t)cb * 512), 0, kColStep * 512u, 0x00020000);
    };
    auto load_piece = [&](__amdgpu_buffer_rsrc_t rs, uint4 *dst, int i) __attribute__((always_inline)) {
        auto *lds = (__attribute__((address_space(3))) void *)&dst[64 * WAVES * i + 64 * wave];
        const int voff = (int)lane_off[i & (kOffsets - 1)], soff = (int)(512u * kColsPerRound * (uint32_t)i);
        __builtin_amdgcn_raw_ptr_buffer_load_lds(rs, lds, 16, voff, soff, 0, 0);
    };
    auto load_thr = [&](uint32_t cb, float (&out)[kSub]) __attribute__((always_inline)) {
        const float *q = col_popkT + (size_t)(cb >> 7) * 128 + c31 * 4 + ((cb >> 5) & 3u);
        if constexpr (kSub == 4) {
            const float4 v = *reinterpret_cast<const float4 *>(q);
            out[0] = v.x; out[1] = v.y; out[2] = v.z; out[3] = v.w;
        } else {
            const float2 v = *reinterpret_cast<const float2 *>(q);
            out[0] = v.x; out[1] = v.y;
        }
    };

    v16f acc[2] = {v16f{}, v16f{}};
    if constexpr (kRowcLds) acc[0] = rowc[0];
    uint32_t n_early = 0;
    float thr[kSub], thr_next[kSub];

    constexpr uint32_t kCandChunk = 8, kCandChunkMax = 512;
    uint32_t q_chunk = kCandChunk, q_taken = 0;
    unsigned long long q_next = 0, q_end = 0;
    auto emit = [&](const v16f &c, float thrv, uint32_t live_rows, uint32_t rows_first, uint32_t col_first) __attribute__((always_inline)) {
        uint32_t mask = 0;
#pragma unroll
        for (int r = 0; r < 16; r++) mask |= (c[r] >= thrv) ? (1u << r) : 0u;
        mask &= live_rows;
        const uint32_t j = col_first + c31;
        if (j < c_begin || j >= c_end) mask = 0;
        const unsigned long long bal = __builtin_amdgcn_ballot_w64(mask != 0u);
        if (bal == 0ull) return;
        const uint32_t need = (uint32_t)__builtin_popcountll(bal);
        if (q_next + need > q_end) {
            if (q_taken >= 2) q_chunk = min(2u * q_chunk, kCandChunkMax);
            q_taken++;
            const uint32_t take = max((need + kCandChunk - 1) / kCandChunk * kCandChunk, q_chunk);
            unsigned long long base = 0;
            if (lane == 0) base = atomicAdd(cand_head, (unsigned long long)take);
            q_next = ((unsigned long long)(uint32_t)__builtin_amdgcn_readfirstlane((int)(base >> 32)) << 32) |
                     (uint32_t)__builtin_amdgcn_readfirstlane((int)(uint32_t)base);
            q_end = q_next + take;
        }
        const unsigned long long slot = q_next + __builtin_amdgcn_mbcnt_hi((uint32_t)(bal >> 32), __builtin_amdgcn_mbcnt_lo((uint32_t)bal, 0u));
        if (mask != 0u) {
            if (slot < cand_capacity) {
                CandEntry ce; ce.row_base = rows_first + 4 * g; ce.col = j; ce.mask = mask; ce.pad = 0;
                *reinterpret_cast<uint4 *>(&cand[slot]) = *reinterpret_cast<const uint4 *>(&ce);
            } else {
                const uint32_t p = rows_first + 4 * g + (uint32_t)(__builtin_ctz(mask) & 3) + 8 * (uint32_t)(__builtin_ctz(mask) >> 2);
                if (p < n_rows) atomicMin(overflow_row, row_index_base + (row_perm ? row_perm[p] : p));
            }
        }
        q_next += need;
    };

    auto run_stage = [&](uint32_t cb, const uint4 *cur, uint4 *nxt) __attribute__((always_inline)) {
        const uint32_t cb_next = cb + kColStep < c_end ? cb + kColStep : cb;
        const __amdgpu_buffer_rsrc_t rs_next = stage_rsrc(cb_next);
        load_thr(cb_next, thr_next);
        uint32_t flags = 0;
        uint4 fq[NB];
        auto frag = [&](int i) __attribute__((always_inline)) {
            const uint32_t sub = (uint32_t)((i / K) >> 1), s = (uint32_t)(i % K);
            return cur[((32u * sub + c31) << 5) | ((s + 16u * g) ^ c31)];
        };
#pragma unroll
        for (int i = 0; i < P; i++) fq[i] = frag(i);
        __builtin_amdgcn_sched_barrier(0);
        float m0 = 0.f, m1 = 0.f, m2 = 0.f, m3 = 0.f, m4 = 0.f, m5 = 0.f;
        static_for<0, NM>([&](auto ic) __attribute__((always_inline)) {
            constexpr int i = decltype(ic)::value;
            constexpr int blk = i / K, s = i % K, rt = blk & 1;
            const uint4 bv = fq[i % NB];
            const v8i b = {(int)bv.x, (int)bv.y, (int)bv.z, (int)bv.w, 0, 0, 0, 0};
            const v8i ar = {a[rt][s].x, a[rt][s].y, a[rt][s].z, a[rt][s].w, 0, 0, 0, 0};
            if constexpr (s == 0 && !kRowcLds) acc[rt] = __builtin_amdgcn_mfma_scale_f32_32x32x64_f8f6f4(ar, b, rowc[rt], 4, 4, 0, 0, 0, 0);
            else acc[rt] = __builtin_amdgcn_mfma_scale_f32_32x32x64_f8f6f4(ar, b, acc[rt], 4, 4, 0, 0, 0, 0);
            if constexpr (i + P < NM) fq[(i + P) % NB] = frag(i + P);
            if constexpr ((i % kDmaEvery) == 1 && (i / kDmaEvery) < kDmaPerWave) load_piece(rs_next, nxt, i / kDmaEvery);
            if constexpr (blk >= 1) {
                const v16f &c = acc[rt ^ 1];
                if constexpr (s == kTestAt) {
                    m0 = fmaxf(fmaxf(c[0], c[1]), c[2]); m1 = fmaxf(fmaxf(c[3], c[4]), c[5]); m2 = fmaxf(fmaxf(c[6], c[7]), c[8]);
                } else if constexpr (s == kTestAt + 1) {
                    m3 = fmaxf(fmaxf(c[9], c[10]), c[11]); m4 = fmaxf(fmaxf(c[12], c[13]), c[14]);
                } else if constexpr (s == kTestAt + 2) {
                    m5 = fmaxf(fmaxf(m0, m1), m2); m3 = fmaxf(fmaxf(m3, m4), c[15]);
                } else if constexpr (s == kTestAt + 3) {
                    if (__builtin_amdgcn_ballot_w64(fmaxf(m5, m3) >= thr[(blk - 1) >> 1]) != 0ull) {
                        flags |= 1u << (blk - 1);
                        emit(c, thr[(blk - 1) >> 1], live[rt ^ 1], row0 + 32u * (uint32_t)(rt ^ 1), cb + 32u * (uint32_t)((blk - 1) >> 1));
                    }
                }
            }
            if constexpr (kRowcLds && s >= kTestAt + 4 && s < kTestAt + 8) {
                constexpr int q = s - (kTestAt + 4);
                const float4 v = s_rc[((rt ^ 1) * 2) * 4 + q];
                acc[rt ^ 1][4 * q + 0] = v.x; acc[rt ^ 1][4 * q + 1] = v.y; acc[rt ^ 1][4 * q + 2] = v.z; acc[rt ^ 1][4 * q + 3] = v.w;
            }
            __builtin_amdgcn_sched_barrier(0);
        });
        {
            const v16f &c = acc[(NBLK - 1) & 1];
            m0 = fmaxf(fmaxf(c[0], c[1]), c[2]); m1 = fmaxf(fmaxf(c[3], c[4]), c[5]); m2 = fmaxf(fmaxf(c[6], c[7]), c[8]);
            m3 = fmaxf(fmaxf(c[9], c[10]), c[11]); m4 = fmaxf(fmaxf(c[12], c[13]), c[14]);
            const float pm = fmaxf(fmaxf(fmaxf(m0, m1), m2), fmaxf(fmaxf(m3, m4), c[15]));
            if (__builtin_amdgcn_ballot_w64(pm >= thr[kSub - 1]) != 0ull) {
                flags |= 1u << (NBLK - 1);
                emit(c, thr[kSub - 1], live[(NBLK - 1) & 1], row0 + 32u * (uint32_t)((NBLK - 1) & 1), cb + 32u * (kSub - 1));
            }
        }
        uint32_t valid = 0;
#pragma unroll
        for (uint32_t sub = 0; sub < kSub; sub++)
            if (cb + 32u * sub < c_end) valid |= 3u << (2 * sub);
        flags &= valid;
        n_early += (uint32_t)__builtin_popcount(valid & ~flags);
        asm volatile("s_waitcnt vmcnt(0)" ::: "memory");
        __syncthreads();
#pragma unroll
        for (uint32_t sub = 0; sub < kSub; sub++) thr[sub] = 0.5f * (thr_next[sub] - tol_f);
    };

#pragma unroll
    for (int i = 0; i < kDmaPerWave; i++) load_piece(stage_rsrc(cb0), s_b0, i);
    load_thr(cb0, thr_next);
#pragma unroll
    for (int rt = 0; rt < 2; rt++)
#pragma unroll
        for (int s = 0; s < K; s++) asm volatile("" ::"v"(a[rt][s]));
    asm volatile("s_waitcnt vmcnt(0)" ::: "memory");
    __syncthreads();
#pragma unroll
    for (uint32_t sub = 0; sub < kSub; sub++) thr[sub] = 0.5f * (thr_next[sub] - tol_f);
    for (uint32_t cb = cb0; cb < c_end; cb += 2 * kColStep) {
        run_stage(cb, s_b0, s_b1);
        if (cb + kColStep >= c_end) break;
        run_stage(cb + kColStep, s_b1, s_b0);
    }
    if (tid == 0) atomicAdd(&counters[1], (unsigned long long)(c_end - c_begin) * kTileRows);
    if (CHK < 15 && lane == 0 && n_early) atomicAdd(&counters[3], (unsigned long long)n_early * (32u * 32u));
}

__global__ __launch_bounds__(256) void hits_mark_incoming_kernel(const vdf_hit *__restrict__ hits, unsigned long long n,
                                                                 uint32_t *__restrict__ has_in)
{
    for (size_t i = (size_t)blockIdx.x * 256 + threadIdx.x; i < n; i += (size_t)gridDim.x * 256) {
        const uint32_t j = hits[i].col;
        if (!((has_in[j >> 5] >> (j & 31)) & 1u)) atomicOr(&has_in[j >> 5], 1u << (j & 31));
    }
}

__global__ __launch_bounds__(256) void hits_mark_covered_kernel(const vdf_hit *__restrict__ hits, unsigned long long n,
                                                                const uint32_t *__restrict__ has_in, uint32_t *__restrict__ covered)
{
    for (size_t i = (size_t)blockIdx.x * 256 + threadIdx.x; i < n; i += (size_t)gridDim.x * 256) {
        const vdf_hit h = hits[i];
        if (!((has_in[h.row >> 5] >> (h.row & 31)) & 1u) && !((covered[h.col >> 5] >> (h.col & 31)) & 1u))
            atomicOr(&covered[h.col >> 5], 1u << (h.col & 31));
    }
}

__global__ __launch_bounds__(256) void hits_compact_kernel(const vdf_hit *__restrict__ hits, unsigned long long n,
                                                           const uint32_t *__restrict__ covered, vdf_hit *__restrict__ out,
                                                           unsigned long long *__restrict__ counter)
{
    const size_t n_round = (n + 63) & ~(size_t)63;
    for (size_t i = (size_t)blockIdx.x * 256 + threadIdx.x; i < n_round; i += (size_t)gridDim.x * 256) {
        vdf_hit h{0u, 0u};
        bool keep = false;
        if (i < n) {
            h = hits[i];
            keep = !((covered[h.row >> 5] >> (h.row & 31)) & 1u);
        }
        const unsigned long long bal = __builtin_amdgcn_ballot_w64(keep);
        if (bal == 0ull) continue;
        const int leader = __builtin_ctzll(bal);
        unsigned long long base = 0;
        if ((int)(threadIdx.x & 63) == leader) base = atomicAdd(counter, (unsigned long long)__builtin_popcountll(bal));
        base = ((unsigned long long)(uint32_t)__shfl((int)(base >> 32), leader, 64) << 32) | (uint32_t)__shfl((int)(uint32_t)base, leader, 64);
        if (keep) out[base + __builtin_amdgcn_mbcnt_hi((uint32_t)(bal >> 32), __builtin_amdgcn_mbcnt_lo((uint32_t)bal, 0u))] = h;
    }
}

__global__ __launch_bounds__(256) void bitmap_or_kernel(uint32_t *__restrict__ dst, const uint32_t *__restrict__ srcs, size_t n_words,
                                                        uint32_t n_srcs)
{
    for (size_t w = (size_t)blockIdx.x * 256 + threadIdx.x; w < n_words; w += (size_t)gridDim.x * 256) {
        uint32_t v = dst[w];
        for (uint32_t r = 0; r < n_srcs; r++) v |= srcs[(size_t)r * n_words + w];
        dst[w] = v;
    }
}

hipError_t launch_bitmap_or(uint32_t *dst, const uint32_t *srcs, size_t n_words, uint32_t n_srcs, hipStream_t stream)
{
    if (n_words == 0 || n_srcs == 0) return hipSuccess;
    const uint32_t grid = (uint32_t)std::min<size_t>((n_words + 255) / 256, 4096);
    hipLaunchKernelGGL(bitmap_or_kernel, dim3(grid), dim3(256), 0, stream, dst, srcs, n_words, n_srcs);
    return hipGetLastError();
}

static inline uint32_t filter_grid(unsigned long long n_hits) { return (uint32_t)std::min<unsigned long long>(std::max<unsigned long long>((n_hits + 255) / 256, 1ull), 8192ull); }

hipError_t launch_filter_mark_incoming(const vdf_hit *hits, unsigned long long n_hits, uint32_t n_entries, uint32_t *bitmaps, hipStream_t stream)
{
    const size_t words = ((size_t)n_entries + 31) / 32;
    hipError_t e = hipMemsetAsync(bitmaps, 0, 2 * words * 4, stream);
    if (e != hipSuccess) return e;
    if (n_hits) hipLaunchKernelGGL(hits_mark_incoming_kernel, dim3(filter_grid(n_hits)), dim3(256), 0, stream, hits, n_hits, bitmaps);
    return hipGetLastError();
}

hipError_t launch_filter_mark_covered(const vdf_hit *hits, unsigned long long n_hits, uint32_t n_entries, uint32_t *bitmaps, hipStream_t stream)
{
    const size_t words = ((size_t)n_entries + 31) / 32;
    if (n_hits) hipLaunchKernelGGL(hits_mark_covered_kernel, dim3(filter_grid(n_hits)), dim3(256), 0, stream, hits, n_hits, bitmaps, bitmaps + words);
    return hipGetLastError();
}

hipError_t launch_filter_compact(const vdf_hit *hits, unsigned long long n_hits, uint32_t n_entries, const uint32_t *bitmaps, vdf_hit *out,
                                 unsigned long long *counter, hipStream_t stream)
{
    const size_t words = ((size_t)n_entries + 31) / 32;
    hipError_t e = hipMemsetAsync(counter, 0, 8, stream);
    if (e != hipSuccess) return e;
    if (n_hits) hipLaunchKernelGGL(hits_compact_kernel, dim3(filter_grid(n_hits)), dim3(256), 0, stream, hits, n_hits, bitmaps + words, out, counter);
    return hipGetLastError();
}

hipError_t launch_windows_tiles(int mode, const uint32_t *col_dur, uint32_t n_cols, const uint32_t *row_dur,
                                const uint32_t *row_perm, uint32_t n_rows, uint32_t row_begin, uint32_t row_end,
                                uint32_t shard_index, uint32_t shard_count, const SearchLaunch &L, hipStream_t stream)
{
    if (L.n_row_tiles == 0) return hipSuccess;
    hipLaunchKernelGGL(check_sorted_kernel, dim3(std::min<uint32_t>((n_cols + 255) / 256, 2048u)), dim3(256), 0, stream, col_dur,
                       n_cols, L.counters);
    hipLaunchKernelGGL(windows_tiles_kernel, dim3(L.n_row_tiles), dim3(256), 0, stream, mode, col_dur, n_cols, row_dur,
                       row_perm, n_rows, row_begin, row_end, shard_index, shard_count, (uint32_t)L.tile_rows,
                       L.chunk_cols, L.row_lo, L.row_hi, L.tile_lo, L.tile_hi, L.tile_first, L.tile_count, L.counters);
    hipLaunchKernelGGL(scan_tiles_kernel, dim3(1), dim3(1024), 0, stream, L.tile_count, L.n_row_tiles, L.tile_offset);
    if (L.n_groups) {
        hipLaunchKernelGGL(group_tiles_kernel, dim3(L.n_groups), dim3(256), 0, stream, L.tile_first, L.tile_count,
                           L.n_row_tiles, L.group_size, L.shard_count, L.group_cmin, L.group_blocks);
        hipLaunchKernelGGL(group_scan_kernel, dim3(1), dim3(64), 0, stream, L.group_blocks, L.n_groups, L.group_offset);
    }
    return hipGetLastError();
}

hipError_t launch_hamming_tiles(const SearchLaunch &L, uint32_t total_tiles, hipStream_t stream)
{
    if (total_tiles == 0) return hipSuccess;
#define VDF_LAUNCH(RR, CW)                                                                                          \
    hipLaunchKernelGGL((hamming_tile_kernel<RR, CW>), dim3(nb), dim3(256), 0, stream, L.row_hashes, L.row_perm,      \
                       L.n_rows, L.row_index_base, L.col_hashes, L.row_lo, L.row_hi, L.tile_lo, L.tile_hi,          \
                       L.tile_first, L.tile_offset, L.n_row_tiles, L.chunk_cols, L.tol, L.matched, L.self_mode,     \
                       L.hits, L.capacity, L.counters, L.overflow_row, base)
#define VDF_LAUNCH_R(RR)                                                                                            \
    switch (L.prune_step) {       \
    case 6: VDF_LAUNCH(RR, 14); break;                                                                              \
    case 8: case 10: VDF_LAUNCH(RR, 22); break;                                                                     \
    case 11: case 12: VDF_LAUNCH(RR, 26); break;                                                                    \
    default: VDF_LAUNCH(RR, 32); break;                                                                             \
    }
    for (uint32_t base = 0; base < total_tiles; base += kMaxBlocksPerLaunch) {
        const uint32_t nb = std::min(kMaxBlocksPerLaunch, total_tiles - base);
        switch (L.tile_rows / 256) {
        case 1: VDF_LAUNCH_R(1); break;
        case 2: VDF_LAUNCH_R(2); break;
        case 4: VDF_LAUNCH_R(4); break;
        default: return hipErrorInvalidValue;
        }
        hipError_t e = hipGetLastError();
        if (e != hipSuccess) return e;
    }
#undef VDF_LAUNCH_R
#undef VDF_LAUNCH
    return hipSuccess;
}

__global__ __launch_bounds__(256) void group_max_distance_kernel(const uint32_t *__restrict__ hashes,
                                                                 const unsigned long long *__restrict__ offsets,
                                                                 const unsigned long long *__restrict__ members,
                                                                 const uint32_t *__restrict__ ref_hashes,
                                                                 const long long *__restrict__ ref_index,
                                                                 uint32_t *__restrict__ out)
{
    __shared__ uint32_t s_max[4];
    const uint32_t g = blockIdx.x;
    const unsigned long long a = offsets[g], b = offsets[g + 1];
    const bool has_ref = ref_hashes != nullptr && ref_index != nullptr && ref_index[g] >= 0;
    const uint32_t k = (uint32_t)(b - a) + (has_ref ? 1u : 0u);
    auto member_ptr = [&](uint32_t idx) -> const uint32_t * {
        return idx < (uint32_t)(b - a) ? hashes + (size_t)members[a + idx] * 32 : ref_hashes + (size_t)ref_index[g] * 32;
    };
    uint32_t best = 0;
    for (uint32_t i = 0; i + 1 < k; i++) {
        const_u32_ptr hi = (const_u32_ptr)(uintptr_t)member_ptr(i);
        for (uint32_t j = i + 1 + threadIdx.x; j < k; j += 256) {
            const uint4 *hj = reinterpret_cast<const uint4 *>(member_ptr(j));
            uint32_t d = 0;
#pragma unroll
            for (int q = 0; q < 8; q++) {
                const uint4 v = hj[q];
                d += __builtin_popcount(v.x ^ hi[4 * q]) + __builtin_popcount(v.y ^ hi[4 * q + 1]) +
                     __builtin_popcount(v.z ^ hi[4 * q + 2]) + __builtin_popcount(v.w ^ hi[4 * q + 3]);
            }
            best = max(best, d);
        }
    }
    best = wave_max(best);
    if ((threadIdx.x & 63) == 0) s_max[threadIdx.x >> 6] = best;
    __syncthreads();
    if (threadIdx.x == 0) out[g] = max(max(s_max[0], s_max[1]), max(s_max[2], s_max[3]));
}

hipError_t launch_group_max_distance(const uint32_t *hashes, const unsigned long long *offsets,
                                     const unsigned long long *members, const uint32_t *ref_hashes,
                                     const long long *ref_index, uint32_t n_groups, uint32_t *out, hipStream_t stream)
{
    if (n_groups == 0) return hipSuccess;
    hipLaunchKernelGGL(group_max_distance_kernel, dim3(n_groups), dim3(256), 0, stream, hashes, offsets, members,
                       ref_hashes, ref_index, out);
    return hipGetLastError();
}

hipError_t launch_expand_fp4(const uint32_t *packed, uint32_t n, uint32_t n_pad, void *expanded, uint32_t k_steps,
                             float *pop3 , hipStream_t stream)
{
    if (n_pad == 0) return hipSuccess;
    if (pop3 && (n_pad % 128u)) return hipErrorInvalidValue;
    const size_t total = (size_t)n_pad * 32;
    hipLaunchKernelGGL(expand_fp4_kernel, dim3((uint32_t)std::min<size_t>((total + 255) / 256, kMaxBlocksPerLaunch)), dim3(256), 0, stream, packed, n, n_pad,
                       reinterpret_cast<uint4 *>(expanded), k_steps, pop3, pop3 ? pop3 + n_pad : nullptr,
                       pop3 ? pop3 + 2 * (size_t)n_pad : nullptr);
    return hipGetLastError();
}

hipError_t launch_hamming_tiles_mfma2(const SearchLaunch &L, uint32_t total_tiles, hipStream_t stream)
{
    if (total_tiles == 0) return hipSuccess;
    if (L.tile_rows != 512 && L.tile_rows != 256) return hipErrorInvalidValue;
    for (uint32_t base = 0; base < total_tiles; base += kMaxBlocksPerLaunch) {
        const uint32_t nb = std::min(kMaxBlocksPerLaunch, total_tiles - base);
#define VDF_MFMA2_LAUNCH(CK, WV)                                                                                    \
    hipLaunchKernelGGL((hamming_mfma2_kernel<CK, WV>), dim3(nb), dim3(64 * WV), 0, stream,                           \
                       reinterpret_cast<const uint4 *>(L.row_exp), L.row_perm, L.n_rows, L.row_index_base,           \
                       reinterpret_cast<const uint4 *>(L.col_exp), L.row_lo, L.row_hi, L.tile_lo, L.tile_hi,         \
                       L.tile_first, L.tile_count, L.group_offset, L.group_cmin, L.n_groups, L.group_size,           \
                       L.shard_index, L.shard_count, L.n_row_tiles, L.chunk_cols, L.tol, L.matched, L.self_mode,     \
                       L.hits, L.capacity, L.counters, L.overflow_row, base, L.row_pop3, L.row_pad, L.col_pop3, L.col_pad,                   \
                       reinterpret_cast<CandEntry *>(L.cand), L.cand_capacity, L.cand_head)
#define VDF_MFMA2_STEPS(WV)                                                                                         \
    switch (L.prune_step) {                                    \
    case 0: case 1: case 2: case 3: case 4: case 5: case 6: VDF_MFMA2_LAUNCH(6, WV); break;                          \
    case 7: case 8: VDF_MFMA2_LAUNCH(8, WV); break;                                                                  \
    case 9: case 10: VDF_MFMA2_LAUNCH(10, WV); break;                                                                \
    case 11: VDF_MFMA2_LAUNCH(11, WV); break;                                                                        \
    case 12: VDF_MFMA2_LAUNCH(12, WV); break;                                                                        \
    case 13: VDF_MFMA2_LAUNCH(13, WV); break;                                                                        \
    case 14: VDF_MFMA2_LAUNCH(14, WV); break;                                                                        \
    default: VDF_MFMA2_LAUNCH(16, WV); break;                                                                        \
    }
        if (L.tile_rows == 512) { VDF_MFMA2_STEPS(8) } else { VDF_MFMA2_STEPS(4) }
#undef VDF_MFMA2_STEPS
#undef VDF_MFMA2_LAUNCH
        hipError_t e = hipGetLastError();
        if (e != hipSuccess) return e;
    }
    return hipSuccess;
}

hipError_t launch_resolve_candidates(const SearchLaunch &L, hipStream_t stream)
{
    hipLaunchKernelGGL(resolve_candidates_kernel, dim3(1024), dim3(256), 0, stream, reinterpret_cast<const CandEntry *>(L.cand),
                       L.cand_head, L.cand_capacity, L.row_hashes, L.row_perm, L.n_rows, L.row_index_base, L.col_hashes, L.n_cols,
                       L.row_lo, L.row_hi, L.tol, L.matched, L.self_mode, L.hits, L.capacity, L.counters, L.overflow_row);
    return hipGetLastError();
}

}
```

vid_dup_finder_lib_amd/csrc/vdf_ctx.h:

```cpp
#pragma once
#include <condition_variable>
#include <functional>
#include <map>
#include <mutex>
#include <string>
#include <thread>
#include <vector>

#include "resize_tables.h"
#include <atomic>

#include "vdf_internal.h"

inline std::atomic<long long> g_live_device_bytes{0};
inline std::atomic<long long> g_live_pinned_bytes{0};

struct DevBuf {
    void *p = nullptr;
    size_t cap = 0;
    hipError_t reserve(size_t bytes)
    {
        if (bytes <= cap) return hipSuccess;
        release();
        size_t want = bytes + bytes / 8 + 256;
        hipError_t e = hipMalloc(&p, want);
        if (e != hipSuccess) { p = nullptr; return e; }
        cap = want;
        g_live_device_bytes += (long long)cap;
        return hipSuccess;
    }
    void release()
    {
        if (p) { (void)hipFree(p); g_live_device_bytes -= (long long)cap; }
        p = nullptr;
        cap = 0;
    }
    template <class T> T *as() const { return reinterpret_cast<T *>(p); }
};

struct PinBuf {
    void *p = nullptr;
    size_t cap = 0;
    bool pinned = false;
    bool reserve(size_t bytes)
    {
        if (bytes <= cap) return true;
        release();
        if (hipHostMalloc(&p, bytes, hipHostMallocDefault) == hipSuccess) {
            pinned = true;
            g_live_pinned_bytes += (long long)bytes;
        } else {
            (void)hipGetLastError();
            p = std::malloc(bytes);
            pinned = false;
            if (!p) return false;
        }
        cap = bytes;
        return true;
    }
    void release()
    {
        if (p) { if (pinned) { (void)hipHostFree(p); g_live_pinned_bytes -= (long long)cap; } else std::free(p); }
        p = nullptr; cap = 0; pinned = false;
    }
    template <class T> T *as() const { return reinterpret_cast<T *>(p); }
};

struct DeviceAxisTable {
    DevBuf start, size, w;
    vdf::HostAxisTable host;
};

struct DeviceMfmaTable {
    DevBuf operand, bias, meta;
    vdf::MfmaAxisTable host;
};

struct BoxTableSet {
    DevBuf blob, entries;
    bool usable = false;
    bool one_tile = false;
};

namespace vdf_impl {
struct Worker;
struct RcclState;
struct CopyPool;

struct ShardExchange {
    virtual ~ShardExchange() = default;
    virtual int agree(uint32_t shard, vdf_ctx *d, bool *all_complete, uint64_t *total_hits) = 0;
    virtual int or_bitmap(uint32_t shard, vdf_ctx *d, uint32_t *d_bitmap, size_t n_words, hipStream_t stream) = 0;
    virtual void abort(int rc, const std::string &msg) { (void)rc; (void)msg; }
};
constexpr int kExchangeOff = 1;
}

struct ExpOwner {
    const void *hashes = nullptr;
    size_t n = 0;
    uint32_t k_steps = 0;
    const void *buffer = nullptr;
    bool operator==(const ExpOwner &o) const { return hashes == o.hashes && n == o.n && k_steps == o.k_steps && buffer == o.buffer && hashes; }
};

struct vdf_ctx {
    int device = 0;
    hipStream_t stream = nullptr;
    hipStream_t copy_stream = nullptr;
    bool one_stream = false;
    hipEvent_t ev0 = nullptr, ev1 = nullptr;
    hipEvent_t ev_copy[2] = {nullptr, nullptr}, ev_done[2] = {nullptr, nullptr};
    std::mutex mu;
    std::string err;
    uint64_t hit_capacity = 1ull << 24;
    vdf_search_stats stats{};
    vdf_search_timing timing{};
    hipEvent_t ev_mid = nullptr;
    hipEvent_t ev_wait = nullptr;
    bool spin_wait = false;
    bool no_link_turns = false;
    uint32_t tile_rows = 256 * vdf::kDefaultRowsPerLane;
    uint32_t chunk_cols = vdf::kDefaultChunkCols;
    DevBuf row_lo, row_hi, tile_lo, tile_hi, tile_first, tile_count, tile_offset, counters, hits, perm, matched;
    DevBuf up_hashes, up_dur, up_ref_hashes, up_ref_dur;
    DevBuf hits2, hit_bitmaps;
    DevBuf bitmap_gather;
    DevBuf sort_scratch;
    DevBuf sort_scratch_pub;
    DevBuf align_plan, align_scratch, align_up;
    DevBuf out_zero, out_zero2, up_zero, variant_hashes;
    DevBuf small, frames, frames2, out_hashes, out_hashes2, out_dc, out_dc2, cos_table, crops, crop_desc, crop_tables, crop_desc2, crop_tables2, crop_work;
    PinBuf pin[2], pin_out[2];
    PinBuf pin_ctrl;
    PinBuf pin_crops, pin_desc;
    const void *pinned_db = nullptr;
    size_t pinned_n = 0;
    ExpOwner exp_owner;
    size_t refs_hint_cols = 0, refs_hint_rows = 0;
    uint32_t refs_hint_chunk = 0;
    bool no_hit_filter = false;
    uint64_t hits_guess = 0;
    PinBuf pin_small;
    std::map<uint32_t, DeviceAxisTable *> axis_tables;
    std::map<uint64_t, DeviceMfmaTable *> mfma_tables;
    std::map<uint64_t, BoxTableSet *> box_tables;
    std::map<uint32_t, bool> axis_symmetric;
    bool no_device_path_order = false;
    bool lb_host_plan = false;
    bool no_lb_fused = false;
    int hash_no_persistent = 0, hash_wgs_per_cu = 3;
    bool hash_wgs_per_cu_set = false;
    uint32_t mfma_chunk_cols = 0, mfma_group = 8192;
    DevBuf group_cmin, group_offset, group_blocks;
    uint32_t mfma_min_wgs = 8192;
    uint64_t cand_scale = 1;
    uint32_t cand_capacity_override = 0;
    uint32_t mfma_self_rows = 512;
    uint32_t mfma_refs_rows = 256;
    int mfma_prune_step = -1;
    int search_backend = 1;
    DevBuf exp_cols, exp_rows, pop_cols, pop_rows, cand;
    size_t cand_dirty = SIZE_MAX;
    int wavestream_knob = 0;
    bool no_rowcrop = false, rowcrop_all = false, no_boxstream = false;
    bool no_smallcrop = false;
    int lb_side_strips = 0;
    int copy_threads = 0;
    size_t host_chunk_bytes = 32u << 20;
    bool host_direct = true;
    bool force_rccl = false;
    bool test_exchange_fail = false;
    bool err_secondary = false;
    int resize_mode = 0;
    struct HostHits {
        PinBuf buf;
        size_t size() const { return buf.cap / sizeof(vdf_hit); }
        bool resize(size_t n) { return buf.reserve(n * sizeof(vdf_hit)); }
        vdf_hit *data() const { return buf.as<vdf_hit>(); }
    } host_hits;
    vdf_impl::CopyPool *copy_pool = nullptr;
    uint64_t r_n_hits = 0;
    uint32_t r_overflow = 0xFFFFFFFFu;
    int r_rc = 0;

    std::vector<vdf_ctx *> subs;
    std::vector<vdf_impl::Worker *> workers;
    vdf_impl::RcclState *rccl = nullptr;
    std::vector<vdf_search_stats> dev_stats;
    std::vector<vdf_search_timing> dev_timing;

    ~vdf_ctx();
};

namespace vdf_impl {

void set_create_error(const std::string &msg);
int fail(vdf_ctx *ctx, int code, const std::string &msg);
int fail_hip(vdf_ctx *ctx, hipError_t e, const char *what);

#define VDF_HIP(ctx, call)                                                      \
    do {                                                                        \
        hipError_t e__ = (call);                                                \
        if (e__ != hipSuccess) return vdf_impl::fail_hip((ctx), e__, #call);    \
    } while (0)

struct DeviceGuard {
    int saved = -1;
    DeviceGuard() { if (hipGetDevice(&saved) != hipSuccess) { saved = -1; (void)hipGetLastError(); } }
    ~DeviceGuard() { if (saved >= 0) (void)hipSetDevice(saved); }
    DeviceGuard(const DeviceGuard &) = delete;
    DeviceGuard &operator=(const DeviceGuard &) = delete;
};

inline bool hit_less(const vdf_hit &a, const vdf_hit &b) { return a.row != b.row ? a.row < b.row : a.col < b.col; }

int create_single(int device_id, vdf_ctx **out, std::string *err);
int upload(vdf_ctx *ctx, DevBuf &buf, const void *src, size_t bytes, hipStream_t stream);
int wait_event(vdf_ctx *ctx, hipEvent_t ev);
std::mutex &link_mutex(int device);
int search_core(vdf_ctx *ctx, int mode, const uint64_t *d_col_hashes, const uint32_t *d_col_dur, size_t n_cols,
                const uint64_t *d_row_hashes, const uint32_t *d_row_dur, const uint32_t *d_row_perm, size_t n_rows,
                uint32_t tol_int, uint32_t shard_index, uint32_t shard_count, uint32_t row_begin, uint32_t row_end,
                const uint32_t *d_matched, uint32_t row_index_base, vdf_hit *hits, uint64_t capacity,
                uint64_t *n_hits_out, uint32_t *overflow_row_out, hipStream_t stream, bool replay_only = false,
                vdf_ctx::HostHits *staging = nullptr,
                ShardExchange *fx = nullptr);
int search_refs_device_locked(vdf_ctx *ctx, const uint64_t *d_cand_hashes, const uint32_t *d_cand_durations,
                              size_t n_cand, const uint64_t *d_ref_hashes, const uint32_t *d_ref_durations, size_t n_ref,
                              uint32_t tol_int, uint32_t ref_index_base, vdf_hit *hits, uint64_t capacity,
                              uint64_t *n_hits, hipStream_t s, vdf_ctx::HostHits *staging = nullptr);
int hash_device_locked(vdf_ctx *ctx, const uint8_t *d_frames, size_t n_clips, uint32_t frames_per_clip, uint32_t w,
                       uint32_t h, size_t frame_stride, size_t clip_stride, uint64_t *d_out, uint32_t *d_dc,
                       hipStream_t stream, uint64_t *d_zero = nullptr);
int hash_host_locked(vdf_ctx *ctx, const uint8_t *frames, size_t n_clips, uint32_t w, uint32_t h, size_t frame_stride,
                     size_t clip_stride, int letterbox, uint64_t *out_hashes, uint32_t *out_crops, uint32_t *out_dontcare,
                     uint64_t *out_zero = nullptr);
int search_self_resident(vdf_ctx *ctx, size_t n, uint32_t tol_int, vdf_groups *out);
int search_refs_resident(vdf_ctx *ctx, size_t n_cand, const std::vector<size_t> &ref_cnt, const std::vector<size_t> &ref_base,
                         uint32_t tol_int, vdf_groups *out);
int letterbox_hash_device_locked(vdf_ctx *ctx, const uint8_t *d_frames, size_t n_clips, uint32_t frames_per_clip,
                                 uint32_t w, uint32_t h, size_t frame_stride, size_t clip_stride, uint64_t *d_out,
                                 uint32_t *d_dc, uint32_t *out_crops, hipStream_t stream, uint32_t *d_out_crops = nullptr);
int hash_clips_locked(vdf_ctx *ctx, const uint8_t *d_buf, size_t buf_bytes, const vdf_clip *clips, size_t n_clips, uint32_t frames_per_clip,
                      uint64_t *d_out, uint32_t *d_dc, hipStream_t stream, uint64_t *d_zero = nullptr);
int hash_clips_host_locked(vdf_ctx *ctx, const uint8_t *buf, size_t buf_bytes, const vdf_clip *clips, size_t n_clips, uint32_t frames_per_clip,
                           uint64_t *out_hashes, uint32_t *out_dontcare, int letterbox = 0, uint32_t *out_crops = nullptr,
                           uint64_t *out_zero = nullptr);
int letterbox_clips_locked(vdf_ctx *ctx, const uint8_t *d_buf, size_t buf_bytes, const vdf_clip *clips, size_t n_clips, uint32_t frames_per_clip,
                           uint64_t *d_out, uint32_t *d_dc, uint32_t *out_crops, hipStream_t stream);
int mixed_check_failed(vdf_ctx *ctx, const vdf::MixedCheck &c);
void destroy_copy_pool(vdf_ctx *ctx);
bool is_sorted_u32(const uint32_t *d, size_t n);

int for_each_device(vdf_ctx *ctx, const std::function<int(int, vdf_ctx *)> &f);
inline int device_count(const vdf_ctx *ctx) { return ctx->subs.empty() ? 1 : (int)ctx->subs.size(); }
inline vdf_ctx *device_ctx(vdf_ctx *ctx, int k) { return ctx->subs.empty() ? ctx : ctx->subs[k]; }
void destroy_multi(vdf_ctx *ctx);
ShardExchange *make_local_exchange(vdf_ctx *ctx);

}
```

vid_dup_finder_lib_amd/csrc/vdf_internal.h:

```cpp
#pragma once
#include <hip/hip_runtime.h>
#include <stdint.h>

#include "../../include/vdf.h"
#include "hash_variant.h"
#include "resize_dispatch.h"
#include "windows_plan.h"
#include "align_plan.h"

namespace vdf {

constexpr int kDefaultRowsPerLane = 2;
constexpr uint32_t kDefaultChunkCols = 2048;

struct SearchLaunch {
    const uint32_t *row_hashes;
    const uint32_t *row_perm;
    uint32_t n_rows;
    uint32_t row_index_base;
    const uint32_t *col_hashes;
    uint32_t n_cols;
    const void *row_exp, *col_exp;
    const float *row_pop3 = nullptr, *col_pop3 = nullptr;
    uint32_t row_pad = 0, col_pad = 0;
    void *cand = nullptr;
    uint32_t cand_capacity = 0;
    unsigned long long *cand_head = nullptr;
    uint32_t *row_lo, *row_hi;
    uint32_t *tile_lo, *tile_hi, *tile_first, *tile_count, *tile_offset;
    uint32_t *group_cmin, *group_offset, *group_blocks;
    int prune_step = 16;
    uint32_t shard_index = 0, shard_count = 1;
    uint32_t n_groups, group_size;
    uint32_t n_row_tiles;
    uint32_t tile_rows;
    uint32_t chunk_cols;
    uint32_t tol;
    const uint32_t *matched;
    int self_mode;
    vdf_hit *hits;
    unsigned long long capacity;
    unsigned long long *counters;
    uint32_t *overflow_row;
};

hipError_t launch_windows_tiles(int mode, const uint32_t *col_dur, uint32_t n_cols, const uint32_t *row_dur,
                                const uint32_t *row_perm, uint32_t n_rows, uint32_t row_begin, uint32_t row_end,
                                uint32_t shard_index, uint32_t shard_count, const SearchLaunch &L,
                                hipStream_t stream);
hipError_t launch_hamming_tiles(const SearchLaunch &L, uint32_t total_tiles, hipStream_t stream);
constexpr uint32_t kMfmaRowPad = 512, kMfmaColPad = 128;
hipError_t launch_expand_fp4(const uint32_t *packed, uint32_t n, uint32_t n_pad, void *expanded, uint32_t k_steps,
                             float *pop3, hipStream_t stream);
hipError_t launch_hamming_tiles_mfma2(const SearchLaunch &L, uint32_t total_tiles, hipStream_t stream);
hipError_t launch_resolve_candidates(const SearchLaunch &L, hipStream_t stream);
hipError_t launch_filter_mark_incoming(const vdf_hit *hits, unsigned long long n_hits, uint32_t n_entries, uint32_t *bitmaps, hipStream_t stream);
hipError_t launch_filter_mark_covered(const vdf_hit *hits, unsigned long long n_hits, uint32_t n_entries, uint32_t *bitmaps, hipStream_t stream);
hipError_t launch_filter_compact(const vdf_hit *hits, unsigned long long n_hits, uint32_t n_entries, const uint32_t *bitmaps, vdf_hit *out,
                                 unsigned long long *counter, hipStream_t stream);
hipError_t launch_bitmap_or(uint32_t *dst, const uint32_t *srcs, size_t n_words, uint32_t n_srcs, hipStream_t stream);
hipError_t launch_group_max_distance(const uint32_t *hashes, const unsigned long long *offsets,
                                     const unsigned long long *members, const uint32_t *ref_hashes,
                                     const long long *ref_index, uint32_t n_groups, uint32_t *out, hipStream_t stream);

struct ResizeAxisTable {
    const int32_t *start;
    const int32_t *size;
    const int16_t *w;
    int32_t window;
    int32_t precision;
};

hipError_t launch_resize_generic(const uint8_t *frames, size_t n_clips, uint32_t w, uint32_t h, size_t frame_stride,
                                 size_t clip_stride, ResizeAxisTable th, ResizeAxisTable tv, int need_h, int need_v,
                                 int32_t y_first, int32_t tmp_rows, uint8_t *small, hipStream_t stream);
struct MfmaResizeArgs {
    const void *bh, *av;
    const int32_t *bias_h, *bias_v;
    int32_t prec_h, prec_v, n_kt, n_rg;
    const int32_t *band_meta = nullptr;
    int32_t band_stride = 0;
    int32_t persistent_wgs_per_cu = 3;
};
hipError_t launch_resize_dct_fused(const uint8_t *frames, size_t n_clips, uint32_t w, uint32_t h, size_t frame_stride,
                                   size_t clip_stride, const uint8_t *buf_end, const MfmaResizeArgs &a, const HashPlan &plan,
                                   const double *cos_table, uint64_t *out_hashes, uint32_t *out_dontcare,
                                   hipStream_t stream, uint64_t *out_zero = nullptr);
hipError_t launch_resize_mfma_frames(const uint8_t *frames, size_t n_clips, uint32_t w, uint32_t h,
                                     size_t frame_stride, size_t clip_stride, const uint8_t *buf_end,
                                     const MfmaResizeArgs &a, uint8_t *small, hipStream_t stream);
struct CropStreamClip;
struct CropStreamTable;
hipError_t launch_resize_mfma_frames_stream(const uint8_t *frames, size_t n_clips, uint32_t w, uint32_t h,
                                            size_t frame_stride, size_t clip_stride, const MfmaResizeArgs &a, const HashPlan &plan,
                                            uint8_t *small, hipStream_t stream, const CropStreamClip *clips = nullptr,
                                            const CropStreamTable *tables = nullptr);
hipError_t launch_resize_mfma_frames_ksplit(const uint8_t *frames, size_t n_clips, uint32_t w, uint32_t h,
                                            size_t frame_stride, size_t clip_stride, const MfmaResizeArgs &a, const HashPlan &plan,
                                            uint8_t *small, hipStream_t stream, const CropStreamClip *clips = nullptr,
                                            const CropStreamTable *tables = nullptr);
struct CropClipDesc {
    uint32_t x0, y0, w, h;
    uint32_t h_table, v_table;
    uint32_t src_clip, pad;
};
struct CropTableEntry {
    const void *operand;
    const int32_t *bias;
    int32_t n_tiles, precision;
};
struct CropStreamClip {
    uint32_t x0, y0, w, h;
    uint32_t wp, nb, n_chunks, src_clip;
    uint32_t h_table, v_table, step_rows, step_x;
};
struct CropStreamTable {
    const void *operand;
    const int32_t *bias;
    const int32_t *meta;
    int32_t n_tiles, precision, band_stride, pad;
};
hipError_t launch_resize_mfma_cropped_stream(const uint8_t *frames, size_t n_clips, uint32_t pitch, uint32_t frame_rows,
                                             size_t frame_stride, size_t clip_stride, const CropStreamClip *clips,
                                             const CropStreamTable *tables, int cls, bool shift, uint8_t *small,
                                             hipStream_t stream);
hipError_t launch_resize_mfma_box_wavestream(const uint8_t *frames, size_t n_clips, uint32_t w, uint32_t h, size_t frame_stride,
                                             size_t clip_stride, const MfmaResizeArgs &a, uint32_t x0, uint32_t box_w, int waves,
                                             const CropStreamClip *clips, const CropStreamTable *tables, uint8_t *small, hipStream_t stream);
size_t letterbox_work_bytes(size_t n_clips, uint32_t frames_per_clip);
hipError_t launch_letterbox(const uint8_t *frames, size_t n_clips, uint32_t frames_per_clip, uint32_t w, uint32_t h,
                            size_t frame_stride, size_t clip_stride, uint32_t *crops, uint32_t *work, hipStream_t stream, int side_strips = 0);
hipError_t launch_resize_dct_cropped_small(const uint8_t *frames, size_t n_clips, uint32_t pitch, size_t frame_stride,
                                           size_t clip_stride, const uint8_t *buf_end, const CropClipDesc *desc,
                                           const CropTableEntry *tables, const double *cos_table, uint64_t *out_hashes,
                                           uint32_t *out_dontcare, hipStream_t stream, uint64_t *out_zero = nullptr);
hipError_t launch_resize_dct_cropped_small_boxes(const uint8_t *frames, size_t n_clips, uint32_t w, uint32_t h, size_t frame_stride,
                                                 size_t clip_stride, const uint8_t *buf_end, const uint32_t *boxes,
                                                 const CropTableEntry *tables, const double *cos_table, uint64_t *out_hashes,
                                                 uint32_t *out_dontcare, hipStream_t stream);
hipError_t launch_letterbox_mixed(const uint8_t *buf, const LetterboxProbeDesc *d_desc, const LetterboxMixedLaunch *launches, size_t n_launches, size_t n_clips,
                                  uint32_t *crops, uint32_t *work, hipStream_t stream);
constexpr uint32_t kSmallBoxTableStride = 2176;
hipError_t launch_letterbox_hash_small(const uint8_t *frames, size_t n_clips, uint32_t w, uint32_t h, size_t frame_stride, size_t clip_stride,
                                       const void *box_tables, const double *cos_table, uint64_t *out_hashes, uint32_t *out_dontcare,
                                       uint32_t *out_crops, int wgs_per_cu, hipStream_t stream);
hipError_t launch_resize_mfma_cropped(const uint8_t *frames, size_t n_clips, uint32_t pitch, size_t frame_stride,
                                      size_t clip_stride, const uint8_t *buf_end, const CropClipDesc *desc,
                                      const CropTableEntry *tables, uint8_t *small, bool wide, hipStream_t stream);
hipError_t launch_mixed_small(const uint8_t *buf, const uint8_t *buf_end, const MixedClipDesc *desc, size_t n_clips, const CropTableEntry *tables,
                              const double *cos_table, uint64_t *out_hashes, uint32_t *out_dontcare, hipStream_t stream, uint64_t *out_zero = nullptr);
hipError_t launch_mixed_frames(const uint8_t *buf, const uint8_t *buf_end, const MixedClipDesc *desc, size_t n_clips, const CropTableEntry *tables,
                               bool wide, uint8_t *small, hipStream_t stream);
hipError_t launch_dct_hash_indexed(const uint8_t *small, const MixedClipDesc *desc, size_t n_clips, const double *cos_table, uint64_t *out_hashes,
                                   uint32_t *out_dontcare, hipStream_t stream, uint64_t *out_zero = nullptr);
size_t sort_order_scratch_bytes(uint32_t n, bool with_rank);
hipError_t launch_sort_order(const uint32_t *dur, const uint32_t *rank, uint32_t n, uint32_t *perm_out, void *scratch,
                             size_t scratch_bytes, hipStream_t stream);
hipError_t launch_path_facts(const char *d_blob, const unsigned long long *d_off, const uint32_t *d_sel, uint32_t n, void *d_facts16, hipStream_t stream);
size_t path_order_scratch_bytes(uint32_t n);
hipError_t launch_path_duration_order(const char *d_blob, const unsigned long long *d_off, const uint32_t *d_sel, const uint32_t *d_dur, uint32_t n,
                                      uint32_t first_word, uint32_t n_words, uint32_t *order_out, void *scratch, size_t scratch_bytes,
                                      hipStream_t stream);
size_t sort_hits_scratch_bytes(size_t n);
hipError_t launch_sort_hits(vdf_hit *hits, size_t n, unsigned row_bits, void *scratch, size_t scratch_bytes, hipStream_t stream,
                            unsigned col_bits = 32);
hipError_t launch_gather_hashes(const uint64_t *hashes, const uint32_t *dur, const uint32_t *perm, uint32_t n, uint64_t *hashes_out,
                                uint32_t *dur_out, hipStream_t stream);
hipError_t launch_dct_hash(const uint8_t *small, size_t small_clip_stride, size_t small_frame_stride, size_t n_clips,
                           const double *cos_table, uint64_t *out_hashes, uint32_t *out_dontcare, hipStream_t stream, uint64_t *out_zero = nullptr);
hipError_t launch_hash_variants(const uint64_t *hashes, const uint64_t *zero, size_t n, const uint32_t *variants, uint32_t n_variants, uint64_t *out,
                                hipStream_t stream);
struct WindowsFrames {
    const uint8_t *base, *tail;
    size_t clip_stride, chunk_stride, frame_stride, tail_clip_stride;
    uint32_t main_frames, tail_first;
    bool dwords;
};
hipError_t launch_dct_hash_windows(const WindowsFrames &f, size_t n_clips, const WindowsPlan &plan, const double *cos_table, uint64_t *out_hashes,
                                   uint32_t *out_dontcare, hipStream_t stream);
struct AlignLaunch {
    const uint32_t *a_hashes, *a_first;
    const uint8_t *a_skip;
    const uint32_t *b_hashes, *b_first;
    const uint8_t *b_skip;
    const AlignPair *pairs;
    const uint32_t *unit_offset;
    uint32_t n_pairs, n_units;
    uint32_t tol, min_run;
    void *scratch;
    vdf_alignment **dense_out;
    uint32_t **total_out;
};
size_t align_scratch_bytes(size_t n_pairs, size_t n_units);
hipError_t launch_align_chunk(const AlignLaunch &L, hipStream_t stream);

}
```

Before: 4712 billion.

## Replace row-tile groups with balanced work items and a persistent ticketed MFMA kernel

Replaces the group-based grid (groups of row tiles times column chunks) with an explicit list of search items, each a row tile and a column span. Span size is capped from the total column work divided by resident workgroups times items per workgroup. The MFMA kernel now launches with as many workgroups as can be resident, queried through occupancy, and they pull items through an atomic ticket. This is meant to remove idle blocks and load imbalance from uneven duration windows, and it drops the two-pass adaptive chunk search for refs mode. The cost is extra count, scan and fill kernels plus the added item buffer.

```diff
diff --git a/vid_dup_finder_lib_amd/csrc/api.cpp b/vid_dup_finder_lib_amd/csrc/api.cpp
--- a/vid_dup_finder_lib_amd/csrc/api.cpp
+++ b/vid_dup_finder_lib_amd/csrc/api.cpp
@@ -32,7 +32,7 @@
         delete kv.second;
     }
     DevBuf *all[] = {&row_lo, &row_hi, &tile_lo, &tile_hi, &tile_first, &tile_count, &tile_offset, &counters,
-                     &hits, &perm, &matched, &exp_cols, &exp_rows, &pop_cols, &pop_rows, &cand, &group_cmin, &group_offset, &group_blocks, &up_hashes,
+                     &hits, &perm, &matched, &exp_cols, &exp_rows, &pop_cols, &pop_rows, &cand, &chunk_items, &chunk_offset, &items, &up_hashes,
                      &up_dur, &up_ref_hashes, &up_ref_dur, &small, &frames, &frames2, &out_hashes, &out_hashes2, &out_dc,
                      &out_dc2, &cos_table, &crops, &crop_desc, &crop_tables, &crop_desc2, &crop_tables2, &crop_work, &sort_scratch, &sort_scratch_pub, &hits2, &hit_bitmaps, &bitmap_gather,
                      &out_zero, &out_zero2, &up_zero, &variant_hashes, &align_plan, &align_scratch, &align_up};
@@ -80,7 +80,6 @@
 
 constexpr size_t kPinSmallBytes = 4u << 20;
 constexpr uint64_t kDeviceSortHits = 1u << 17;
-constexpr uint32_t kRefsMinWorkgroups = 2048;
 constexpr uint64_t kSpecSortHits = 1u << 14;
 constexpr uint64_t kFilterHits = 1u << 16;
 
@@ -104,12 +103,10 @@
     L.tile_rows = mfma ? (mode == 1 ? ctx->mfma_refs_rows : ctx->mfma_self_rows) : ctx->tile_rows;
     L.chunk_cols = mfma ? ctx->mfma_chunk_cols : ctx->chunk_cols;
     L.n_row_tiles = (uint32_t)((n_rows + L.tile_rows - 1) / L.tile_rows);
-    if (mfma && L.chunk_cols == 0) {
-        L.chunk_cols = 65536;
-        while (L.chunk_cols > 4096 && (uint64_t)L.n_row_tiles * ((n_cols + L.chunk_cols - 1) / L.chunk_cols) < ctx->mfma_min_wgs) L.chunk_cols /= 2;
-    }
-    while ((uint64_t)L.n_row_tiles * ((n_cols + L.chunk_cols - 1) / L.chunk_cols) >= 0x40000000ull && L.chunk_cols < (1u << 22))
+    if (mfma && L.chunk_cols == 0) L.chunk_cols = vdf::kItemMaxSpan;
+    while (!mfma && (uint64_t)L.n_row_tiles * ((n_cols + L.chunk_cols - 1) / L.chunk_cols) >= 0x40000000ull && L.chunk_cols < (1u << 22))
         L.chunk_cols *= 2;
+    while (mfma && (n_cols + L.chunk_cols - 1) / L.chunk_cols > (1u << 20) && L.chunk_cols < (1u << 22)) L.chunk_cols *= 2;
     const size_t padded_rows = (size_t)L.n_row_tiles * L.tile_rows;
     VDF_HIP(ctx, ctx->row_lo.reserve(padded_rows * 4));
     VDF_HIP(ctx, ctx->row_hi.reserve(padded_rows * 4));
@@ -118,7 +115,7 @@
     VDF_HIP(ctx, ctx->tile_first.reserve((size_t)L.n_row_tiles * 4));
     VDF_HIP(ctx, ctx->tile_count.reserve((size_t)L.n_row_tiles * 4));
     VDF_HIP(ctx, ctx->tile_offset.reserve(((size_t)L.n_row_tiles + 1) * 4));
-    VDF_HIP(ctx, ctx->counters.reserve(64));
+    VDF_HIP(ctx, ctx->counters.reserve(128));
     const uint64_t dev_cap = std::max<uint64_t>(capacity, 1);
     VDF_HIP(ctx, ctx->hits.reserve(dev_cap * sizeof(vdf_hit)));
 
@@ -157,15 +154,23 @@
     if (mfma) L.prune_step = L.prune_step <= 6 ? 6 : L.prune_step <= 8 ? 8 : L.prune_step <= 10 ? 10 : L.prune_step <= 14 ? L.prune_step : 16;
     else L.prune_step = L.prune_step <= 6 ? 6 : L.prune_step <= 10 ? 10 : L.prune_step <= 12 ? 12 : 16;
     if (mfma) {
-        L.group_size = std::min<uint32_t>(ctx->mfma_group, L.n_row_tiles);
-        L.n_groups = (L.n_row_tiles + L.group_size - 1) / L.group_size;
-        if (L.n_groups > 1024) return fail(ctx, VDF_E_INVAL, "too many row-tile groups");
-        VDF_HIP(ctx, ctx->group_cmin.reserve((size_t)L.n_groups * 4));
-        VDF_HIP(ctx, ctx->group_offset.reserve(((size_t)L.n_groups + 1) * 4));
-        VDF_HIP(ctx, ctx->group_blocks.reserve((size_t)L.n_groups * 4));
-        L.group_blocks = ctx->group_blocks.as<uint32_t>();
-        L.group_cmin = ctx->group_cmin.as<uint32_t>();
-        L.group_offset = ctx->group_offset.as<uint32_t>();
+        L.n_chunks = (uint32_t)((n_cols + L.chunk_cols - 1) / L.chunk_cols);
+        VDF_HIP(ctx, ctx->chunk_items.reserve((size_t)L.n_chunks * 4));
+        VDF_HIP(ctx, ctx->chunk_offset.reserve(((size_t)L.n_chunks + 1) * 4));
+        L.chunk_items = ctx->chunk_items.as<uint32_t>();
+        L.chunk_offset = ctx->chunk_offset.as<uint32_t>();
+        L.ticket = reinterpret_cast<uint32_t *>(ctx->counters.as<unsigned long long>() + 8);
+        L.items_per_wg = ctx->mfma_items_per_wg;
+        uint32_t &resident = ctx->mfma_resident[L.tile_rows * 32u + (uint32_t)L.prune_step];
+        if (resident == 0) {
+            int per_cu = 0, cus = 0;
+            VDF_HIP(ctx, vdf::mfma2_resident_per_cu(L.tile_rows, L.prune_step, &per_cu));
+            VDF_HIP(ctx, hipDeviceGetAttribute(&cus, hipDeviceAttributeMultiprocessorCount, ctx->device));
+            if (cus < 1) return fail(ctx, VDF_E_HIP, "no compute units");
+            resident = (uint32_t)per_cu * (uint32_t)cus;
+        }
+        L.resident_wgs = resident;
+        L.max_wgs = ctx->mfma_max_wgs;
         const uint32_t k_steps = (uint32_t)(L.prune_step < 15 ? L.prune_step + 1 : 16);
         const uint32_t col_pad = (uint32_t)((n_cols + vdf::kMfmaRowPad - 1) / vdf::kMfmaRowPad * vdf::kMfmaRowPad) + vdf::kMfmaColPad;
         VDF_HIP(ctx, ctx->exp_cols.reserve((size_t)col_pad * 512));
@@ -196,39 +201,31 @@
             L.row_pad = row_pad;
         }
     }
-    const unsigned long long init[8] = {0, 0, 0, 0, 0xFFFFFFFFull, 0, 0, 0};
+    const unsigned long long init[16] = {0, 0, 0, 0, 0xFFFFFFFFull, 0, 0, 0, 0, 0, 0, 0, 0, 0, 0, 0};
     const bool pin_ok = ctx->pin_small.reserve(kPinSmallBytes) && ctx->pin_small.pinned;
     uint64_t spec = std::min<uint64_t>(capacity, std::max<uint64_t>(ctx->hits_guess + ctx->hits_guess / 4 + 1024, 8192));
     if (!pin_ok || spec * sizeof(vdf_hit) > kPinSmallBytes) spec = 0;
     const bool spec_sort = spec && ctx->hits_guess >= kSpecSortHits;
     if (spec_sort) VDF_HIP(ctx, hipMemsetAsync(ctx->hits.p, 0xFF, (size_t)spec * sizeof(vdf_hit), stream));
-    const bool adapt_refs = mode == 1 && mfma && ctx->mfma_chunk_cols == 0;
-    if (adapt_refs && ctx->refs_hint_cols == n_cols && ctx->refs_hint_rows == n_rows && ctx->refs_hint_chunk) L.chunk_cols = ctx->refs_hint_chunk;
-    if (!ctx->pin_ctrl.reserve(256)) return fail(ctx, VDF_E_OOM, "pinned staging");
+    if (!ctx->pin_ctrl.reserve(512)) return fail(ctx, VDF_E_OOM, "pinned staging");
     unsigned long long *pre = ctx->pin_ctrl.as<unsigned long long>() + 8;
-    uint32_t total_tiles = 0;
-    unsigned long long unsorted = 0, admitted = 0;
-    for (int pass = 0;; pass++) {
-        VDF_HIP(ctx, hipMemcpyAsync(ctx->counters.p, init, sizeof init, hipMemcpyHostToDevice, stream));
-        VDF_HIP(ctx, vdf::launch_windows_tiles(mode, d_col_dur, (uint32_t)n_cols, d_row_dur, d_row_perm, (uint32_t)n_rows,
-                                               row_begin, row_end, shard_index, shard_count, L, stream));
-        VDF_HIP(ctx, hipMemcpyAsync(pre, L.counters, 64, hipMemcpyDeviceToHost, stream));
-        VDF_HIP(ctx, hipMemcpyAsync(pre + 8, mfma ? L.group_offset + L.n_groups : L.tile_offset + L.n_row_tiles, 4,
-                                    hipMemcpyDeviceToHost, stream));
-        VDF_HIP(ctx, hipMemcpyAsync(pre + 9, L.tile_offset + L.n_row_tiles, 4, hipMemcpyDeviceToHost, stream));
-        VDF_HIP(ctx, hipStreamSynchronize(stream));
-        total_tiles = *reinterpret_cast<const uint32_t *>(pre + 8);
-        const uint32_t busy_tiles = *reinterpret_cast<const uint32_t *>(pre + 9);
-        unsorted = pre[5];
-        admitted = pre[2];
-        if (!adapt_refs || pass > 0 || unsorted || busy_tiles == 0 || busy_tiles >= kRefsMinWorkgroups || L.chunk_cols <= 4096) break;
-        uint64_t est = busy_tiles;
-        while (L.chunk_cols > 4096 && est < kRefsMinWorkgroups) { L.chunk_cols /= 2; est *= 2; }
-    }
-    if (adapt_refs) { ctx->refs_hint_cols = n_cols; ctx->refs_hint_rows = n_rows; ctx->refs_hint_chunk = L.chunk_cols; }
+    VDF_HIP(ctx, hipMemcpyAsync(ctx->counters.p, init, sizeof init, hipMemcpyHostToDevice, stream));
+    VDF_HIP(ctx, vdf::launch_windows_tiles(mode, d_col_dur, (uint32_t)n_cols, d_row_dur, d_row_perm, (uint32_t)n_rows,
+                                           row_begin, row_end, shard_index, shard_count, L, stream));
+    VDF_HIP(ctx, hipMemcpyAsync(pre, L.counters, 128, hipMemcpyDeviceToHost, stream));
+    VDF_HIP(ctx, hipMemcpyAsync(pre + 16, mfma ? L.chunk_offset + L.n_chunks : L.tile_offset + L.n_row_tiles, 4,
+                                hipMemcpyDeviceToHost, stream));
+    VDF_HIP(ctx, hipStreamSynchronize(stream));
+    const uint32_t total_tiles = *reinterpret_cast<const uint32_t *>(pre + 16);
+    const unsigned long long unsorted = pre[5], admitted = pre[2];
     if (unsorted) return fail(ctx, VDF_E_INVAL, "durations are not ascending: pass the arrays in Search::sort order");
     if (total_tiles >= 0x7FFFFFFFu) return fail(ctx, VDF_E_INVAL, "tile count exceeds the grid limit");
     if (mfma) {
+        L.n_items = total_tiles;
+        VDF_HIP(ctx, ctx->items.reserve((size_t)std::max<uint32_t>(L.n_items, 1) * sizeof(vdf::SearchItem)));
+        L.items = ctx->items.as<vdf::SearchItem>();
+        VDF_HIP(ctx, vdf::launch_search_items_fill(L, stream));
+        L.span_cap = (uint32_t)pre[9];
         const uint64_t want = ((uint64_t)((double)admitted * 6e-6) + (uint64_t)total_tiles * 8 * 8 + std::max<uint64_t>(capacity, 1ull << 20)) * ctx->cand_scale;
         L.cand_capacity = (uint32_t)std::min<uint64_t>(want, 0x40000000ull);
         if (ctx->cand_capacity_override)
@@ -247,7 +244,7 @@
     ctx->timing.prep_ms += (float)(now_ms() - t_enter);
     VDF_HIP(ctx, hipEventRecord(ctx->ev0, stream));
     if (mfma) {
-        VDF_HIP(ctx, vdf::launch_hamming_tiles_mfma2(L, total_tiles, stream));
+        VDF_HIP(ctx, vdf::launch_hamming_tiles_mfma2(L, stream));
         VDF_HIP(ctx, hipEventRecord(ctx->ev_mid, stream));
         if (total_tiles) VDF_HIP(ctx, vdf::launch_resolve_candidates(L, stream));
     } else {
@@ -1287,11 +1284,8 @@
     if (const char *s = std::getenv("VDF_MFMA_SELF_ROWS")) { const int v = std::atoi(s); if (v == 256 || v == 512) ctx->mfma_self_rows = (uint32_t)v; }
     if (const char *s = std::getenv("VDF_MFMA_REFS_ROWS")) { const int v = std::atoi(s); if (v == 256 || v == 512) ctx->mfma_refs_rows = (uint32_t)v; }
     if (const char *s = std::getenv("VDF_MFMA_PRUNE_STEP")) ctx->mfma_prune_step = std::atoi(s);
-    if (const char *s = std::getenv("VDF_MFMA_MIN_WGS")) { const long v = std::atol(s); if (v >= 1 && v <= (1 << 24)) ctx->mfma_min_wgs = (uint32_t)v; }
-    if (const char *s = std::getenv("VDF_MFMA_GROUP")) {
-        long c = std::atol(s);
-        if (c >= 1 && c <= (1 << 20)) ctx->mfma_group = (uint32_t)c;
-    }
+    if (const char *s = std::getenv("VDF_MFMA_MAX_WGS")) { const long v = std::atol(s); if (v >= 1 && v <= (1 << 20)) ctx->mfma_max_wgs = (uint32_t)v; }
+    if (const char *s = std::getenv("VDF_MFMA_ITEMS_PER_WG")) { const long v = std::atol(s); if (v >= 1 && v <= (1 << 16)) ctx->mfma_items_per_wg = (uint32_t)v; }
     if (const char *s = std::getenv("VDF_NO_HIT_FILTER")) ctx->no_hit_filter = std::atoi(s) != 0;
     if (std::getenv("VDF_NO_WAVESTREAM")) ctx->wavestream_knob = -1;
     else if (const char *s = std::getenv("VDF_WAVESTREAM_NW")) { const int v = std::atoi(s); if (v >= 3 && v <= 8) ctx->wavestream_knob = v; }
diff --git a/vid_dup_finder_lib_amd/csrc/hamming.hip b/vid_dup_finder_lib_amd/csrc/hamming.hip
--- a/vid_dup_finder_lib_amd/csrc/hamming.hip
+++ b/vid_dup_finder_lib_amd/csrc/hamming.hip
@@ -161,43 +161,63 @@
     if (tid == 1023) tile_offset[n] = s_part[1023];
 }
 
-__global__ __launch_bounds__(256) void group_tiles_kernel(const uint32_t *__restrict__ tile_first,
-                                                          const uint32_t *__restrict__ tile_count, uint32_t n_row_tiles,
-                                                          uint32_t group_size, uint32_t shard_count,
-                                                          uint32_t *__restrict__ group_cmin,
-                                                          uint32_t *__restrict__ group_blocks)
-{
-    __shared__ uint32_t s_min[4], s_max[4];
-    const uint32_t g = blockIdx.x;
-    uint32_t cmin = 0xFFFFFFFFu, cmax = 0;
-    const uint32_t t1 = min((g + 1) * group_size, n_row_tiles);
-    for (uint32_t t = g * group_size + threadIdx.x; t < t1; t += 256) {
-        if (tile_count[t]) {
-            cmin = min(cmin, tile_first[t]);
-            cmax = max(cmax, tile_first[t] + tile_count[t]);
-        }
-    }
-    cmin = wave_min(cmin);
-    cmax = wave_max(cmax);
-    if ((threadIdx.x & 63) == 0) { s_min[threadIdx.x >> 6] = cmin; s_max[threadIdx.x >> 6] = cmax; }
+__global__ __launch_bounds__(256) void items_count_kernel(const uint32_t *__restrict__ tile_lo, const uint32_t *__restrict__ tile_hi,
+                                                          uint32_t n_row_tiles, uint32_t shard_index, uint32_t shard_count,
+                                                          uint32_t chunk_cols, uint32_t resident_wgs, uint32_t per_wg,
+                                                          uint32_t *__restrict__ chunk_items, unsigned long long *__restrict__ counters)
+{
+    __shared__ unsigned long long s_cols[4];
+    __shared__ uint32_t s_n[4];
+    const uint32_t c = blockIdx.x, wave = threadIdx.x >> 6;
+    unsigned long long cols = 0;
+    for (uint32_t t = shard_index + threadIdx.x * shard_count; t < n_row_tiles; t += 256 * shard_count) cols += tile_hi[t] - tile_lo[t];
+#pragma unroll
+    for (int o = 32; o > 0; o >>= 1) cols += __shfl_xor(cols, o, 64);
+    if ((threadIdx.x & 63) == 0) s_cols[wave] = cols;
+    __syncthreads();
+    const uint32_t cap = item_span_cap(s_cols[0] + s_cols[1] + s_cols[2] + s_cols[3], resident_wgs, per_wg);
+    uint32_t n = 0;
+    for (uint32_t t = shard_index + threadIdx.x * shard_count; t < n_row_tiles; t += 256 * shard_count)
+        n += items_in_chunk(tile_lo[t], tile_hi[t], chunk_cols, cap, c);
+#pragma unroll
+    for (int o = 32; o > 0; o >>= 1) n += (uint32_t)__shfl_xor((int)n, o, 64);
+    if ((threadIdx.x & 63) == 0) s_n[wave] = n;
     __syncthreads();
     if (threadIdx.x == 0) {
-        cmin = min(min(s_min[0], s_min[1]), min(s_min[2], s_min[3]));
-        cmax = max(max(s_max[0], s_max[1]), max(s_max[2], s_max[3]));
-        if (cmax <= cmin) { cmin = 0; cmax = 0; }
-        group_cmin[g] = cmin;
-        const uint32_t n_chunks = cmax - cmin;
-        group_blocks[g] = n_chunks * ((group_size + shard_count - 1) / shard_count);
-    }
-}
-
-__global__ void group_scan_kernel(const uint32_t *__restrict__ group_blocks, uint32_t n_groups,
-                                  uint32_t *__restrict__ group_offset)
-{
-    if (threadIdx.x == 0 && blockIdx.x == 0) {
-        uint32_t run = 0;
-        for (uint32_t g = 0; g < n_groups; g++) { group_offset[g] = run; run += group_blocks[g]; }
-        group_offset[n_groups] = run;
+        chunk_items[c] = s_n[0] + s_n[1] + s_n[2] + s_n[3];
+        if (c == 0) counters[9] = cap;
+    }
+}
+
+__global__ __launch_bounds__(256) void items_fill_kernel(const uint32_t *__restrict__ tile_lo, const uint32_t *__restrict__ tile_hi,
+                                                         uint32_t n_row_tiles, uint32_t shard_index, uint32_t shard_count,
+                                                         uint32_t chunk_cols, const uint32_t *__restrict__ chunk_offset,
+                                                         const unsigned long long *__restrict__ counters, uint32_t n_items,
+                                                         SearchItem *__restrict__ items)
+{
+    __shared__ uint32_t s_scan[256];
+    const uint32_t c = blockIdx.x, tid = threadIdx.x;
+    const uint32_t cap = (uint32_t)counters[9];
+    uint32_t run = chunk_offset[c];
+    if (chunk_offset[c + 1] == run) return;
+    for (uint32_t t0 = shard_index; t0 < n_row_tiles; t0 += 256 * shard_count) {
+        const uint32_t t = t0 + tid * shard_count;
+        uint32_t lo = 0, hi = 0;
+        if (t < n_row_tiles) { lo = tile_lo[t]; hi = tile_hi[t]; }
+        const uint32_t n = items_in_chunk(lo, hi, chunk_cols, cap, c);
+        s_scan[tid] = n;
+        __syncthreads();
+        for (uint32_t o = 1; o < 256; o <<= 1) {
+            const uint32_t v = tid >= o ? s_scan[tid - o] : 0u;
+            __syncthreads();
+            s_scan[tid] += v;
+            __syncthreads();
+        }
+        const uint32_t at = run + s_scan[tid] - n;
+        for (uint32_t k = 0; k < n; k++)
+            if (at + k < n_items) items[at + k] = item_in_chunk(t, lo, hi, chunk_cols, cap, c, k);
+        run += s_scan[255];
+        __syncthreads();
     }
 }
 
@@ -437,19 +457,33 @@
     flush();
 }
 
+struct Mfma2Args {
+    const uint4 *row_exp;
+    const uint32_t *row_perm;
+    const uint4 *col_exp;
+    const uint32_t *row_lo, *row_hi;
+    const SearchItem *items;
+    uint32_t *ticket;
+    unsigned long long *counters;
+    uint32_t *overflow_row;
+    const float *row_pop3, *col_pop3;
+    CandEntry *cand;
+    unsigned long long *cand_head;
+    uint32_t n_rows, row_index_base, n_items, tol, row_pad, col_pad, cand_capacity;
+};
+
 template <int CHK, int WAVES>
-__global__ __launch_bounds__(64 * WAVES, 2) void hamming_mfma2_kernel(
-    const uint4 *__restrict__ row_exp, const uint32_t *__restrict__ row_perm, uint32_t n_rows,
-    uint32_t row_index_base, const uint4 *__restrict__ col_exp, const uint32_t *__restrict__ row_lo,
-    const uint32_t *__restrict__ row_hi, const uint32_t *__restrict__ tile_lo, const uint32_t *__restrict__ tile_hi,
-    const uint32_t *__restrict__ tile_first, const uint32_t *__restrict__ tile_count,
-    const uint32_t *__restrict__ group_offset, const uint32_t *__restrict__ group_cmin, uint32_t n_groups,
-    uint32_t group_size, uint32_t shard_index, uint32_t shard_count, uint32_t n_row_tiles, uint32_t chunk_cols,
-    uint32_t tol, const uint32_t *__restrict__ matched, int self_mode, vdf_hit *__restrict__ hits,
-    unsigned long long capacity, unsigned long long *__restrict__ counters, uint32_t *__restrict__ overflow_row,
-    uint32_t block_base, const float *__restrict__ row_pop3, uint32_t row_pad, const float *__restrict__ col_pop3,
-    uint32_t col_pad, CandEntry *__restrict__ cand, uint32_t cand_capacity, unsigned long long *__restrict__ cand_head)
-{
+__global__ __launch_bounds__(64 * WAVES, 2) void hamming_mfma2_kernel(const Mfma2Args A)
+{
+    const uint4 *__restrict__ col_exp = A.col_exp;
+    CandEntry *__restrict__ cand = A.cand;
+    unsigned long long *__restrict__ cand_head = A.cand_head;
+    const uint32_t cand_capacity = A.cand_capacity, tol = A.tol;
+    auto cold = [&]() __attribute__((always_inline)) {
+        const Mfma2Args *p = (const Mfma2Args *)__builtin_amdgcn_kernarg_segment_ptr();
+        asm volatile("" : "+s"(p));
+        return (const __attribute__((address_space(4))) Mfma2Args *)(uintptr_t)p;
+    };
     constexpr int K = CHK < 15 ? CHK + 1 : 16;
     constexpr bool kRowcLds = K > 13;
     constexpr uint32_t kSub = WAVES >= 8 ? 4 : 2;
@@ -463,43 +497,40 @@
     static_assert(kDmaEvery >= 2, "stage too short for its DMA pieces");
     constexpr int kTestAt = 2;
     static_assert(K >= kTestAt + 4, "block too short to hide the previous block's test");
-    const uint32_t bid = blockIdx.x + block_base;
     __shared__ __attribute__((aligned(16))) uint4 s_b0[kColStep * 32];
     __shared__ __attribute__((aligned(16))) uint4 s_b1[kColStep * 32];
     const uint32_t tid = threadIdx.x, lane = tid & 63, g = lane >> 5, c31 = lane & 31;
     const uint32_t wave = (uint32_t)__builtin_amdgcn_readfirstlane((int)(tid >> 6));
 
-    const_u32_ptr goff = (const_u32_ptr)(uintptr_t)group_offset;
-    uint32_t gl = 0, gh = n_groups;
-    while (gh - gl > 1) {
-        const uint32_t mid = (gl + gh) >> 1;
-        if (goff[mid] <= bid) gl = mid; else gh = mid;
-    }
-    const uint32_t idx = bid - goff[gl];
-    const uint32_t per_group = (group_size + shard_count - 1) / shard_count;
-    const uint32_t g0 = gl * group_size;
-    const uint32_t t0 = g0 + (shard_index + shard_count - g0 % shard_count) % shard_count;
-    const uint32_t t = t0 + (idx % per_group) * shard_count;
-    const uint32_t chunk = ((const_u32_ptr)(uintptr_t)group_cmin)[gl] + idx / per_group;
-    if (t >= n_row_tiles || t >= g0 + group_size) return;
+    __shared__ uint32_t s_next_item;
+    if (blockIdx.x >= A.n_items) return;
+    uint32_t t, c_begin, c_end;
     {
-        const uint32_t f = ((const_u32_ptr)(uintptr_t)tile_first)[t], cnt = ((const_u32_ptr)(uintptr_t)tile_count)[t];
-        if (chunk < f || chunk >= f + cnt) return;
-    }
-    const uint32_t t_lo = ((const_u32_ptr)(uintptr_t)tile_lo)[t];
-    const uint32_t t_hi = ((const_u32_ptr)(uintptr_t)tile_hi)[t];
-    const uint32_t c_begin = max(chunk * chunk_cols, t_lo);
-    const uint32_t c_end = min((chunk + 1) * chunk_cols, t_hi);
-    if (c_begin >= c_end) return;
+        const_u32_ptr w = (const_u32_ptr)(uintptr_t)A.items + 4 * (size_t)blockIdx.x;
+        t = w[0]; c_begin = w[1]; c_end = w[2];
+    }
+    uint32_t n_t = t, n_begin = c_begin, n_end = c_end;
+    bool have_next = false;
 
     const float tol_f = (float)min(tol, 1024u);
-    const float *row_popk = row_pop3 + row_pad;
-    const float *col_popkT = col_pop3 + 2 * (size_t)col_pad;
-    const uint32_t row0 = t * kTileRows + wave * 64;
+    const float *col_popkT = A.col_pop3 + 2 * (size_t)A.col_pad;
+    uint32_t row0 = t * kTileRows + wave * 64;
     v4i a[2][K];
-    const float4 *s_rc = nullptr;
+    float4 *s_rc = nullptr;
+    if constexpr (kRowcLds) {
+        __shared__ __attribute__((aligned(16))) float4 s_rowc[WAVES * 2 * 2 * 4];
+        s_rc = s_rowc + ((size_t)wave * 2 * 2 + g) * 4;
+    }
     v16f rowc[2];
     uint32_t live[2];
+    v16f acc[2] = {v16f{}, v16f{}};
+    auto load_targets = [&]() __attribute__((always_inline)) {
+    const auto ka = cold();
+    const uint4 *row_exp = ka->row_exp;
+    const uint32_t *row_perm = ka->row_perm, *row_lo = ka->row_lo, *row_hi = ka->row_hi;
+    const float *row_popk = ka->row_pop3 + ka->row_pad;
+    const uint32_t n_rows = ka->n_rows;
+    row0 = t * kTileRows + wave * 64;
 #pragma unroll
     for (int rt = 0; rt < 2; rt++) {
         live[rt] = 0;
@@ -512,27 +543,38 @@
             const uint4 v = rp[s];
             a[rt][s] = (v4i){(int)v.x, (int)v.y, (int)v.z, (int)v.w};
         }
-#pragma unroll
-        for (int r = 0; r < 16; r++) {
-            const uint32_t pr = row0 + 32 * rt + (r & 3) + 8 * (r >> 2) + 4 * g;
-            const uint32_t sr = (pr < n_rows && row_perm) ? row_perm[pr] : pr;
-            rowc[rt][r] = -0.5f * row_popk[sr];
-            if (row_hi[pr] > row_lo[pr]) live[rt] |= 1u << r;
+        if constexpr (!kRowcLds) {
+#pragma unroll
+            for (int r = 0; r < 16; r++) {
+                const uint32_t pr = row0 + 32 * rt + (r & 3) + 8 * (r >> 2) + 4 * g;
+                const uint32_t sr = (pr < n_rows && row_perm) ? row_perm[pr] : pr;
+                rowc[rt][r] = -0.5f * row_popk[sr];
+                if (row_hi[pr] > row_lo[pr]) live[rt] |= 1u << r;
+            }
         }
     }
     if constexpr (kRowcLds) {
-        __shared__ __attribute__((aligned(16))) float4 s_rowc[WAVES * 2 * 2 * 4];
-        float4 *mine = s_rowc + ((size_t)wave * 2 * 2 + g) * 4;
-        if (c31 == 0) {
-#pragma unroll
-            for (int rt = 0; rt < 2; rt++)
-#pragma unroll
-                for (int q = 0; q < 4; q++)
-                    mine[rt * 2 * 4 + q] = float4{rowc[rt][4 * q], rowc[rt][4 * q + 1], rowc[rt][4 * q + 2], rowc[rt][4 * q + 3]};
-        }
-        s_rc = mine;
-    }
-    const uint32_t cb0 = c_begin & ~(kColStep - 1);
+        const uint32_t rt = c31 >> 4, r = c31 & 15;
+        const uint32_t pr = row0 + 32 * rt + (r & 3) + 8 * (r >> 2) + 4 * g;
+        const uint32_t sr = (pr < n_rows && row_perm) ? row_perm[pr] : pr;
+        reinterpret_cast<float *>(s_rc)[rt * 32 + r] = -0.5f * row_popk[sr];
+        const unsigned long long lv = __builtin_amdgcn_ballot_w64(row_hi[pr] > row_lo[pr]);
+        const uint32_t mine = g ? (uint32_t)(lv >> 32) : (uint32_t)lv;
+        live[0] = mine & 0xFFFFu;
+        live[1] = mine >> 16;
+        __builtin_amdgcn_fence(__ATOMIC_ACQ_REL, "wavefront");
+        __builtin_amdgcn_wave_barrier();
+#pragma unroll
+        for (int q = 0; q < 4; q++) {
+            const float4 v = s_rc[q];
+            acc[0][4 * q + 0] = v.x; acc[0][4 * q + 1] = v.y; acc[0][4 * q + 2] = v.z; acc[0][4 * q + 3] = v.w;
+        }
+    }
+#pragma unroll
+    for (int rt = 0; rt < 2; rt++)
+#pragma unroll
+        for (int s = 0; s < K; s++) asm volatile("" ::"v"(a[rt][s]));
+    };
     constexpr uint32_t kColsPerRound = 2 * WAVES;
     constexpr int kOffsets = 32 / kColsPerRound;
     static_assert(kOffsets >= 1 && (kOffsets & (kOffsets - 1)) == 0, "piece addressing");
@@ -560,8 +602,6 @@
         }
     };
 
-    v16f acc[2] = {v16f{}, v16f{}};
-    if constexpr (kRowcLds) acc[0] = rowc[0];
     uint32_t n_early = 0;
     float thr[kSub], thr_next[kSub];
 
@@ -595,14 +635,16 @@
                 *reinterpret_cast<uint4 *>(&cand[slot]) = *reinterpret_cast<const uint4 *>(&ce);
             } else {
                 const uint32_t p = rows_first + 4 * g + (uint32_t)(__builtin_ctz(mask) & 3) + 8 * (uint32_t)(__builtin_ctz(mask) >> 2);
-                if (p < n_rows) atomicMin(overflow_row, row_index_base + (row_perm ? row_perm[p] : p));
+                const auto ka = cold();
+                const uint32_t *row_perm = ka->row_perm;
+                if (p < ka->n_rows) atomicMin(ka->overflow_row, ka->row_index_base + (row_perm ? row_perm[p] : p));
             }
         }
         q_next += need;
     };
 
     auto run_stage = [&](uint32_t cb, const uint4 *cur, uint4 *nxt) __attribute__((always_inline)) {
-        const uint32_t cb_next = cb + kColStep < c_end ? cb + kColStep : cb;
+        const uint32_t cb_next = cb + kColStep < c_end ? cb + kColStep : (n_begin & ~(kColStep - 1));
         const __amdgpu_buffer_rsrc_t rs_next = stage_rsrc(cb_next);
         load_thr(cb_next, thr_next);
         uint32_t flags = 0;
@@ -669,24 +711,51 @@
         for (uint32_t sub = 0; sub < kSub; sub++) thr[sub] = 0.5f * (thr_next[sub] - tol_f);
     };
 
-#pragma unroll
-    for (int i = 0; i < kDmaPerWave; i++) load_piece(stage_rsrc(cb0), s_b0, i);
-    load_thr(cb0, thr_next);
-#pragma unroll
-    for (int rt = 0; rt < 2; rt++)
-#pragma unroll
-        for (int s = 0; s < K; s++) asm volatile("" ::"v"(a[rt][s]));
-    asm volatile("s_waitcnt vmcnt(0)" ::: "memory");
-    __syncthreads();
+    auto begin_item = [&](bool reload) __attribute__((always_inline)) {
+        const auto ka = cold();
+        uint32_t drawn = 0;
+        if (tid == 0) drawn = gridDim.x + atomicAdd(ka->ticket, 1u);
+        if (reload) load_targets();
+        asm volatile("s_waitcnt vmcnt(0)" ::: "memory");
+        if (tid == 0) s_next_item = drawn;
+        __syncthreads();
+        const uint32_t next_item = (uint32_t)__builtin_amdgcn_readfirstlane((int)s_next_item);
+        have_next = next_item < ka->n_items;
+        if (have_next) {
+            const_u32_ptr w = (const_u32_ptr)(uintptr_t)ka->items + 4 * (size_t)next_item;
+            n_t = w[0]; n_begin = w[1]; n_end = w[2];
+        } else {
+            n_t = t; n_begin = c_begin; n_end = c_end;
+        }
+    };
+    unsigned long long cols_done = 0;
+    uint32_t cb = c_begin & ~(kColStep - 1);
+    auto advance = [&]() __attribute__((always_inline)) {
+        cb += kColStep;
+        if (cb < c_end) return true;
+        cols_done += c_end - c_begin;
+        if (!have_next) return false;
+        const bool reload = n_t != t;
+        t = n_t; c_begin = n_begin; c_end = n_end;
+        cb = c_begin & ~(kColStep - 1);
+        begin_item(reload);
+        return true;
+    };
+
+#pragma unroll
+    for (int i = 0; i < kDmaPerWave; i++) load_piece(stage_rsrc(cb), s_b0, i);
+    load_thr(cb, thr_next);
+    begin_item(true);
 #pragma unroll
     for (uint32_t sub = 0; sub < kSub; sub++) thr[sub] = 0.5f * (thr_next[sub] - tol_f);
-    for (uint32_t cb = cb0; cb < c_end; cb += 2 * kColStep) {
+    for (;;) {
         run_stage(cb, s_b0, s_b1);
-        if (cb + kColStep >= c_end) break;
-        run_stage(cb + kColStep, s_b1, s_b0);
-    }
-    if (tid == 0) atomicAdd(&counters[1], (unsigned long long)(c_end - c_begin) * kTileRows);
-    if (CHK < 15 && lane == 0 && n_early) atomicAdd(&counters[3], (unsigned long long)n_early * (32u * 32u));
+        if (!advance()) break;
+        run_stage(cb, s_b1, s_b0);
+        if (!advance()) break;
+    }
+    if (tid == 0) atomicAdd(&A.counters[1], cols_done * kTileRows);
+    if (CHK < 15 && lane == 0 && n_early) atomicAdd(&A.counters[3], (unsigned long long)n_early * (32u * 32u));
 }
 
 __global__ __launch_bounds__(256) void hits_mark_incoming_kernel(const vdf_hit *__restrict__ hits, unsigned long long n,
@@ -786,11 +855,13 @@
     hipLaunchKernelGGL(windows_tiles_kernel, dim3(L.n_row_tiles), dim3(256), 0, stream, mode, col_dur, n_cols, row_dur,
                        row_perm, n_rows, row_begin, row_end, shard_index, shard_count, (uint32_t)L.tile_rows,
                        L.chunk_cols, L.row_lo, L.row_hi, L.tile_lo, L.tile_hi, L.tile_first, L.tile_count, L.counters);
-    hipLaunchKernelGGL(scan_tiles_kernel, dim3(1), dim3(1024), 0, stream, L.tile_count, L.n_row_tiles, L.tile_offset);
-    if (L.n_groups) {
-        hipLaunchKernelGGL(group_tiles_kernel, dim3(L.n_groups), dim3(256), 0, stream, L.tile_first, L.tile_count,
-                           L.n_row_tiles, L.group_size, L.shard_count, L.group_cmin, L.group_blocks);
-        hipLaunchKernelGGL(group_scan_kernel, dim3(1), dim3(64), 0, stream, L.group_blocks, L.n_groups, L.group_offset);
+    if (L.n_chunks) {
+        if (L.n_chunks > kMaxBlocksPerLaunch) return hipErrorInvalidValue;
+        hipLaunchKernelGGL(items_count_kernel, dim3(L.n_chunks), dim3(256), 0, stream, L.tile_lo, L.tile_hi, L.n_row_tiles, L.shard_index,
+                           L.shard_count, L.chunk_cols, L.resident_wgs, L.items_per_wg, L.chunk_items, L.counters);
+        hipLaunchKernelGGL(scan_tiles_kernel, dim3(1), dim3(1024), 0, stream, L.chunk_items, L.n_chunks, L.chunk_offset);
+    } else {
+        hipLaunchKernelGGL(scan_tiles_kernel, dim3(1), dim3(1024), 0, stream, L.tile_count, L.n_row_tiles, L.tile_offset);
     }
     return hipGetLastError();
 }
@@ -884,39 +955,62 @@
     return hipGetLastError();
 }
 
-hipError_t launch_hamming_tiles_mfma2(const SearchLaunch &L, uint32_t total_tiles, hipStream_t stream)
-{
-    if (total_tiles == 0) return hipSuccess;
+#define VDF_MFMA2_STEPS(WV, DO)                                                                                     \
+    switch (prune_step) {                                                                                           \
+    case 0: case 1: case 2: case 3: case 4: case 5: case 6: DO(6, WV); break;                                        \
+    case 7: case 8: DO(8, WV); break;                                                                                \
+    case 9: case 10: DO(10, WV); break;                                                                              \
+    case 11: DO(11, WV); break;                                                                                      \
+    case 12: DO(12, WV); break;                                                                                      \
+    case 13: DO(13, WV); break;                                                                                      \
+    case 14: DO(14, WV); break;                                                                                      \
+    default: DO(16, WV); break;                                                                                      \
+    }
+
+hipError_t mfma2_resident_per_cu(uint32_t tile_rows, int prune_step, int *out)
+{
+    if (tile_rows != 512 && tile_rows != 256) return hipErrorInvalidValue;
+    int n = 0;
+    hipError_t e = hipSuccess;
+#define VDF_MFMA2_OCC(CK, WV) e = hipOccupancyMaxActiveBlocksPerMultiprocessor(&n, hamming_mfma2_kernel<CK, WV>, 64 * WV, 0)
+    if (tile_rows == 512) { VDF_MFMA2_STEPS(8, VDF_MFMA2_OCC) } else { VDF_MFMA2_STEPS(4, VDF_MFMA2_OCC) }
+#undef VDF_MFMA2_OCC
+    if (e != hipSuccess) return e;
+    if (n < 1) return hipErrorLaunchOutOfResources;
+    *out = n;
+    return hipSuccess;
+}
+
+hipError_t launch_search_items_fill(const SearchLaunch &L, hipStream_t stream)
+{
+    if (L.n_items == 0) return hipSuccess;
+    hipLaunchKernelGGL(items_fill_kernel, dim3(L.n_chunks), dim3(256), 0, stream, L.tile_lo, L.tile_hi, L.n_row_tiles, L.shard_index,
+                       L.shard_count, L.chunk_cols, L.chunk_offset, L.counters, L.n_items, L.items);
+    return hipGetLastError();
+}
+
+hipError_t launch_hamming_tiles_mfma2(const SearchLaunch &L, hipStream_t stream)
+{
+    if (L.n_items == 0) return hipSuccess;
     if (L.tile_rows != 512 && L.tile_rows != 256) return hipErrorInvalidValue;
-    for (uint32_t base = 0; base < total_tiles; base += kMaxBlocksPerLaunch) {
-        const uint32_t nb = std::min(kMaxBlocksPerLaunch, total_tiles - base);
+    if (L.resident_wgs == 0) return hipErrorInvalidValue;
+    uint32_t nb = std::min(L.resident_wgs, L.n_items);
+    if (L.max_wgs) nb = std::min(nb, L.max_wgs);
+    else if (L.span_cap >= kItemMaxSpan && L.n_items <= kMaxBlocksPerLaunch) nb = L.n_items;
+    const int prune_step = L.prune_step;
+    Mfma2Args A;
+    A.row_exp = reinterpret_cast<const uint4 *>(L.row_exp); A.row_perm = L.row_perm; A.col_exp = reinterpret_cast<const uint4 *>(L.col_exp);
+    A.row_lo = L.row_lo; A.row_hi = L.row_hi; A.items = L.items; A.ticket = L.ticket; A.counters = L.counters; A.overflow_row = L.overflow_row;
+    A.row_pop3 = L.row_pop3; A.col_pop3 = L.col_pop3; A.cand = reinterpret_cast<CandEntry *>(L.cand); A.cand_head = L.cand_head;
+    A.n_rows = L.n_rows; A.row_index_base = L.row_index_base; A.n_items = L.n_items; A.tol = L.tol; A.row_pad = L.row_pad; A.col_pad = L.col_pad;
+    A.cand_capacity = L.cand_capacity;
 #define VDF_MFMA2_LAUNCH(CK, WV)                                                                                    \
-    hipLaunchKernelGGL((hamming_mfma2_kernel<CK, WV>), dim3(nb), dim3(64 * WV), 0, stream,                           \
-                       reinterpret_cast<const uint4 *>(L.row_exp), L.row_perm, L.n_rows, L.row_index_base,           \
-                       reinterpret_cast<const uint4 *>(L.col_exp), L.row_lo, L.row_hi, L.tile_lo, L.tile_hi,         \
-                       L.tile_first, L.tile_count, L.group_offset, L.group_cmin, L.n_groups, L.group_size,           \
-                       L.shard_index, L.shard_count, L.n_row_tiles, L.chunk_cols, L.tol, L.matched, L.self_mode,     \
-                       L.hits, L.capacity, L.counters, L.overflow_row, base, L.row_pop3, L.row_pad, L.col_pop3, L.col_pad,                   \
-                       reinterpret_cast<CandEntry *>(L.cand), L.cand_capacity, L.cand_head)
-#define VDF_MFMA2_STEPS(WV)                                                                                         \
-    switch (L.prune_step) {                                    \
-    case 0: case 1: case 2: case 3: case 4: case 5: case 6: VDF_MFMA2_LAUNCH(6, WV); break;                          \
-    case 7: case 8: VDF_MFMA2_LAUNCH(8, WV); break;                                                                  \
-    case 9: case 10: VDF_MFMA2_LAUNCH(10, WV); break;                                                                \
-    case 11: VDF_MFMA2_LAUNCH(11, WV); break;                                                                        \
-    case 12: VDF_MFMA2_LAUNCH(12, WV); break;                                                                        \
-    case 13: VDF_MFMA2_LAUNCH(13, WV); break;                                                                        \
-    case 14: VDF_MFMA2_LAUNCH(14, WV); break;                                                                        \
-    default: VDF_MFMA2_LAUNCH(16, WV); break;                                                                        \
-    }
-        if (L.tile_rows == 512) { VDF_MFMA2_STEPS(8) } else { VDF_MFMA2_STEPS(4) }
+    hipLaunchKernelGGL((hamming_mfma2_kernel<CK, WV>), dim3(nb), dim3(64 * WV), 0, stream, A)
+    if (L.tile_rows == 512) { VDF_MFMA2_STEPS(8, VDF_MFMA2_LAUNCH) } else { VDF_MFMA2_STEPS(4, VDF_MFMA2_LAUNCH) }
+#undef VDF_MFMA2_LAUNCH
+    return hipGetLastError();
+}
 #undef VDF_MFMA2_STEPS
-#undef VDF_MFMA2_LAUNCH
-        hipError_t e = hipGetLastError();
-        if (e != hipSuccess) return e;
-    }
-    return hipSuccess;
-}
 
 hipError_t launch_resolve_candidates(const SearchLaunch &L, hipStream_t stream)
 {
diff --git a/vid_dup_finder_lib_amd/csrc/search_items.h b/vid_dup_finder_lib_amd/csrc/search_items.h
--- /dev/null
+++ b/vid_dup_finder_lib_amd/csrc/search_items.h
@@ -0,0 +1,92 @@
+#pragma once
+#include <cstdint>
+#if !defined(__HIP_DEVICE_COMPILE__)
+#include <vector>
+#endif
+
+#if defined(__HIPCC__)
+#define VDF_ITEMS_HD __host__ __device__
+#else
+#define VDF_ITEMS_HD
+#endif
+
+namespace vdf {
+
+struct SearchItem {
+    uint32_t tile, c_begin, c_end, pad;
+};
+
+constexpr uint32_t kItemStageCols = 128;
+constexpr uint32_t kItemMaxSpan = 65536;
+constexpr uint32_t kItemMinSpan = 1024;
+constexpr uint32_t kItemsPerWorkgroup = 8;
+
+VDF_ITEMS_HD inline uint32_t item_step(uint32_t cap) { return cap < 2 * kItemStageCols ? kItemStageCols : cap & ~(kItemStageCols - 1); }
+VDF_ITEMS_HD inline uint32_t item_first_chunk(uint32_t lo, uint32_t chunk_cols) { return lo / chunk_cols; }
+VDF_ITEMS_HD inline uint32_t item_end_chunk(uint32_t lo, uint32_t hi, uint32_t chunk_cols)
+{
+    return hi > lo ? (uint32_t)(((uint64_t)hi + chunk_cols - 1) / chunk_cols) : lo / chunk_cols;
+}
+VDF_ITEMS_HD inline void item_chunk_range(uint32_t lo, uint32_t hi, uint32_t chunk_cols, uint32_t chunk, uint32_t *b, uint32_t *e)
+{
+    const uint64_t cb = (uint64_t)chunk * chunk_cols, ce = cb + chunk_cols;
+    *b = cb > lo ? (uint32_t)(cb > 0xFFFFFFFFull ? 0xFFFFFFFFull : cb) : lo;
+    *e = ce < hi ? (uint32_t)ce : hi;
+}
+VDF_ITEMS_HD inline uint32_t items_in_chunk(uint32_t lo, uint32_t hi, uint32_t chunk_cols, uint32_t cap, uint32_t chunk)
+{
+    uint32_t b, e;
+    item_chunk_range(lo, hi, chunk_cols, chunk, &b, &e);
+    if (b >= e) return 0;
+    const uint32_t step = item_step(cap), base = b & ~(kItemStageCols - 1);
+    return (uint32_t)(((uint64_t)(e - base) + step - 1) / step);
+}
+VDF_ITEMS_HD inline SearchItem item_in_chunk(uint32_t tile, uint32_t lo, uint32_t hi, uint32_t chunk_cols, uint32_t cap, uint32_t chunk, uint32_t k)
+{
+    uint32_t b, e;
+    item_chunk_range(lo, hi, chunk_cols, chunk, &b, &e);
+    const uint32_t step = item_step(cap), base = b & ~(kItemStageCols - 1);
+    const uint64_t ib = (uint64_t)base + (uint64_t)k * step, ie = ib + step;
+    SearchItem it;
+    it.tile = tile;
+    it.c_begin = ib > b ? (uint32_t)ib : b;
+    it.c_end = ie < e ? (uint32_t)ie : e;
+    it.pad = 0;
+    return it;
+}
+VDF_ITEMS_HD inline uint64_t items_in_tile(uint32_t lo, uint32_t hi, uint32_t chunk_cols, uint32_t cap)
+{
+    uint64_t n = 0;
+    for (uint32_t c = item_first_chunk(lo, chunk_cols), c1 = item_end_chunk(lo, hi, chunk_cols); c < c1; c++) n += items_in_chunk(lo, hi, chunk_cols, cap, c);
+    return n;
+}
+
+VDF_ITEMS_HD inline uint32_t item_span_cap(uint64_t total_cols, uint32_t resident_wgs, uint32_t per_wg)
+{
+    const uint64_t want = (uint64_t)(resident_wgs ? resident_wgs : 1) * (per_wg ? per_wg : 1);
+    uint64_t cap = (total_cols + want - 1) / want;
+    cap = (cap + kItemStageCols - 1) / kItemStageCols * kItemStageCols;
+    if (cap < kItemMinSpan) cap = kItemMinSpan;
+    if (cap > kItemMaxSpan) cap = kItemMaxSpan;
+    return (uint32_t)cap;
+}
+
+VDF_ITEMS_HD inline bool item_tile_in_shard(uint32_t tile, uint32_t shard_index, uint32_t shard_count) { return tile % shard_count == shard_index; }
+
+#if !defined(__HIP_DEVICE_COMPILE__)
+inline std::vector<SearchItem> plan_search_items(const uint32_t *tile_lo, const uint32_t *tile_hi, uint32_t n_tiles, uint32_t n_cols, uint32_t chunk_cols,
+                                                 uint32_t cap, uint32_t shard_index, uint32_t shard_count)
+{
+    std::vector<SearchItem> out;
+    const uint32_t n_chunks = (uint32_t)(((uint64_t)n_cols + chunk_cols - 1) / chunk_cols);
+    for (uint32_t c = 0; c < n_chunks; c++)
+        for (uint32_t t = 0; t < n_tiles; t++) {
+            if (!item_tile_in_shard(t, shard_index, shard_count)) continue;
+            const uint32_t n = items_in_chunk(tile_lo[t], tile_hi[t], chunk_cols, cap, c);
+            for (uint32_t k = 0; k < n; k++) out.push_back(item_in_chunk(t, tile_lo[t], tile_hi[t], chunk_cols, cap, c, k));
+        }
+    return out;
+}
+#endif
+
+}
diff --git a/vid_dup_finder_lib_amd/csrc/vdf_ctx.h b/vid_dup_finder_lib_amd/csrc/vdf_ctx.h
--- a/vid_dup_finder_lib_amd/csrc/vdf_ctx.h
+++ b/vid_dup_finder_lib_amd/csrc/vdf_ctx.h
@@ -137,8 +137,6 @@
     const void *pinned_db = nullptr;
     size_t pinned_n = 0;
     ExpOwner exp_owner;
-    size_t refs_hint_cols = 0, refs_hint_rows = 0;
-    uint32_t refs_hint_chunk = 0;
     bool no_hit_filter = false;
     uint64_t hits_guess = 0;
     PinBuf pin_small;
@@ -151,9 +149,11 @@
     bool no_lb_fused = false;
     int hash_no_persistent = 0, hash_wgs_per_cu = 3;
     bool hash_wgs_per_cu_set = false;
-    uint32_t mfma_chunk_cols = 0, mfma_group = 8192;
-    DevBuf group_cmin, group_offset, group_blocks;
-    uint32_t mfma_min_wgs = 8192;
+    uint32_t mfma_chunk_cols = 0;
+    DevBuf chunk_items, chunk_offset, items;
+    uint32_t mfma_items_per_wg = vdf::kItemsPerWorkgroup;
+    uint32_t mfma_max_wgs = 0;
+    std::map<uint32_t, uint32_t> mfma_resident;
     uint64_t cand_scale = 1;
     uint32_t cand_capacity_override = 0;
     uint32_t mfma_self_rows = 512;
diff --git a/vid_dup_finder_lib_amd/csrc/vdf_internal.h b/vid_dup_finder_lib_amd/csrc/vdf_internal.h
--- a/vid_dup_finder_lib_amd/csrc/vdf_internal.h
+++ b/vid_dup_finder_lib_amd/csrc/vdf_internal.h
@@ -7,6 +7,7 @@
 #include "resize_dispatch.h"
 #include "windows_plan.h"
 #include "align_plan.h"
+#include "search_items.h"
 
 namespace vdf {
 
@@ -28,10 +29,16 @@
     unsigned long long *cand_head = nullptr;
     uint32_t *row_lo, *row_hi;
     uint32_t *tile_lo, *tile_hi, *tile_first, *tile_count, *tile_offset;
-    uint32_t *group_cmin, *group_offset, *group_blocks;
+    uint32_t *chunk_items = nullptr, *chunk_offset = nullptr;
+    SearchItem *items = nullptr;
+    uint32_t *ticket = nullptr;
+    uint32_t span_cap = 0;
+    uint32_t n_chunks = 0, n_items = 0;
+    uint32_t resident_wgs = 0;
+    uint32_t max_wgs = 0;
+    uint32_t items_per_wg = kItemsPerWorkgroup;
     int prune_step = 16;
     uint32_t shard_index = 0, shard_count = 1;
-    uint32_t n_groups, group_size;
     uint32_t n_row_tiles;
     uint32_t tile_rows;
     uint32_t chunk_cols;
@@ -52,7 +59,9 @@
 constexpr uint32_t kMfmaRowPad = 512, kMfmaColPad = 128;
 hipError_t launch_expand_fp4(const uint32_t *packed, uint32_t n, uint32_t n_pad, void *expanded, uint32_t k_steps,
                              float *pop3, hipStream_t stream);
-hipError_t launch_hamming_tiles_mfma2(const SearchLaunch &L, uint32_t total_tiles, hipStream_t stream);
+hipError_t mfma2_resident_per_cu(uint32_t tile_rows, int prune_step, int *out);
+hipError_t launch_search_items_fill(const SearchLaunch &L, hipStream_t stream);
+hipError_t launch_hamming_tiles_mfma2(const SearchLaunch &L, hipStream_t stream);
 hipError_t launch_resolve_candidates(const SearchLaunch &L, hipStream_t stream);
 hipError_t launch_filter_mark_incoming(const vdf_hit *hits, unsigned long long n_hits, uint32_t n_entries, uint32_t *bitmaps, hipStream_t stream);
 hipError_t launch_filter_mark_covered(const vdf_hit *hits, unsigned long long n_hits, uint32_t n_entries, uint32_t *bitmaps, hipStream_t stream);
```

Result: no change. 4669 billion (-0.9%).
